# marvinquiet/SpaDOT

Measured on AMD Instinct MI355X. Metric: training steps/sec + Sinkhorn iters/sec, 50k spots x 3k genes x 5 timepoints, higher is better.
Workload: dtype bf16; 1 GPU; cfg3: 5 time points x 10000 spots x 3000 genes, batch 512, k=30, 1200 inducing points; parallelism=1 GPU, n_sub=9980, E_sub=308893, m_inducing=236, params=16136032, hip_graphs=True, staged_graphs=True, bucketed_grad_exchange=False, units_in_schedule=80

## Files before the change

### include/spadot_model.h

```cpp
#ifndef SPADOT_MODEL_H
#define SPADOT_MODEL_H

#ifdef __cplusplus
extern "C" {
#endif

enum { SPADOT_DT_F32 = 0, SPADOT_DT_BF16 = 1, SPADOT_DT_F64 = 2 };
enum { SPADOT_KERNEL_GAUSSIAN = 0, SPADOT_KERNEL_CAUCHY = 1, SPADOT_KERNEL_QUADRATIC = 2 };

const char *spadot_model_version(void);

int spadot_gat_forward(const void *h, int dtype, const float *s_src, const float *s_dst,
                       const int *rowptr, const int *col, const float *bias, int n, int H, int C,
                       int concat, int act, void *out, float *alpha_out, void *stream);

int spadot_gat_backward_target(const void *g_out, const void *out, const void *h, int dtype,
                               const float *s_src, const float *s_dst, const float *alpha,
                               const int *rowptr, const int *col, int n, int H, int C, int concat,
                               int act, void *g_pre, float *dz, float *ds_dst, void *stream);

int spadot_gat_backward_source(const void *g_pre, int dtype, const float *alpha, const float *dz,
                               const int *rowptr_t, const int *col_t, const int *eid_t, int n, int H,
                               int C, void *dh, float *ds_src, const float *ds_dst, const float *att_src,
                               const float *att_dst, void *stream);
// ... 33 lines not shown
                          void *stream);
int spadot_bn_act_backward(const float *dy, const float *y, const void *x, int x_dtype, const float *lin_bias,
                           const float *gamma, const float *save_mean, const float *save_invstd, int b, int F,
                           double slope, void *dx, float *dgamma, float *dbeta, void *stream);
int spadot_ln_act_forward(const float *x, const float *gamma, const float *beta, int b, int F, double eps, double slope,
                          float *y, float *save_mean, float *save_invstd, void *stream);
int spadot_ln_act_backward(const float *dy, const float *y, const float *x, const float *gamma, const float *save_mean,
                           const float *save_invstd, int b, int F, double slope, float *dx, float *dgamma, float *dbeta,
                           void *stream);

int spadot_svgp_post_forward(const double *raw, const double *rd, const double *r, const double *Mr, const double *ld,
                             const double *sm, const double *mu, const double *var, const double *ktilde, int b, int L,
                             int m, double c, double kl_const, double b_over_N, double *p_m, double *mv, double *p_v,
                             double *tr, double *out4, float *skl32 , void *stream);
int spadot_svgp_post_backward(const float *g_skl, const double *out4, const double *G_pm, const double *G_pv,
                              const double *mu, const double *var, const double *mv, const double *tr, const double *p_m,
                              const double *p_v, const double *ktilde, const double *Mr, const double *M, int b, int L,
                              int m, double c, double b_over_N, double *g_mu, double *g_var, double *G1, double *G2T,
                              double *g_kl, double *gMr, double *gM, void *stream);
int spadot_svgp_q1t(const double *Ta, const double *Tb, const double *G2T, const double *m0, const double *g_kl, int L, int nh,
                    int b, double *q1, void *stream);
int spadot_svgp_post_pm_pv(const double *raw, const double *rd_a, const double *ktilde, int b, int L, double c, double *p_m,
                           double *p_v, void *stream);
int spadot_svgp_grad_tail(const double *q1, const double *q2, const double *Kdt, const double *p_v, const double *ktilde,
                          const double *p_m, const double *mu, const double *w, const double *g_kl, const double *g_mu,
                          const double *g_var, int b, int L, double c, double *dmu, double *dvar, float *dz,
                          void *stream);
int spadot_svgp_pre(const float *z, int b, int L, double *mu, double *var, double *w, double *muw, void *stream);
int spadot_svgp_pre2(const float *z, const double *Kn, int b, int L, int m, double *mu, double *var, double *w, double *muw,
                     double *A, void *stream);
int spadot_svgp_mid(const double *S, const double *t, const double *M, const double *X2, int L, int m, int rows2,
                    double *r, double *Mr, double *raw, double *sm, double *smpart, int smpart_doubles, void *stream);

int spadot_latent_head_forward(const float *zg, const double *p_m, const double *p_v, float *eps, int b, int Ls,
                               int Lg, float *latent, float *scal2, double *partials, unsigned *counter,
                               unsigned long long *rng_state, void *stream);
int spadot_latent_head_backward(const float *zg, const double *p_v, const float *eps, const float *latent,
                                const float *g_latent, const float *g_kl, const float *g_align, int b, int Ls, int Lg,
                                float *d_zg, double *d_pm, double *d_pv, void *stream);
int spadot_cluster_losses_forward(const float *z, const long long *labels_all, const long long *seed_ids,
                                  const float *centres, const float *prev_centres, const float *gamma,
                                  const long long *cluster_list, int b, int D, int K, int Kp, int Kl, int do_km,
                                  int do_ot, float *out2, float *work, void *stream);
int spadot_cluster_losses_backward(const float *z, const float *centres, const float *prev_centres, const float *gamma,
                                   const long long *cluster_list, const float *work, const float *g_km,
                                   const float *g_ot, int b, int D, int K, int Kp, int Kl, int do_km, int do_ot,
                                   float *dz, void *stream);
int spadot_cluster_losses_fb(const float *z, const long long *labels_all, const long long *seed_ids, const float *centres,
                             const float *prev_centres, const float *gamma, const long long *cluster_list, int b, int D, int K,
                             int Kp, int Kl, int do_km, int do_ot, const float *g_km, const float *g_ot, float *out2,
                             float *work, float *dz, void *stream);
int spadot_mix_losses_forward(const float *const *terms6, const float *w6, float *out7, void *stream);
int spadot_mix_losses_backward(const float *g_elbo, const float *w6, float *g6, void *stream);

int spadot_sqerr_forward(const void *y, const void *yhat, long long count, double inv_scale, int dtype,
                         double *scratch, void *out1, void *stream);
int spadot_sqerr_backward(const void *g1, const void *y, const void *yhat, long long count,
                          double inv_scale, int dtype, void *g_yhat, void *stream);

int spadot_kmeans_assign(const void *x, const void *centers, int n, int k, int d, int dtype, int *labels,
                         void *stream);

int spadot_sgemm_small(int mode, const float *A, int lda, const float *B, int ldb, float *C, int ldc, int M, int N, int K,
                       const float *bias, int batch, long long strideA, long long strideB, long long strideC, void *stream);

int spadot_enc_fused_supported(int b, int F1, int F2, int Q);
long long spadot_enc_fused_workspace(int b, int F1, int F2, int Q);
int spadot_enc_bn_map(const float *h1, const float *lin_bias, const float *gamma, const float *beta, float *running_mean,
                      float *running_var, long long *num_batches_tracked, int b, int F1, double momentum, double eps, double slope,
                      float *y1, float *save_mean, float *save_invstd, const float *W2, int F2, float *part, void *stream);
int spadot_enc_bn_fc(const float *part, int nparts, const float *lin_bias, const float *gamma, const float *beta, float *running_mean,
                     float *running_var, long long *num_batches_tracked, int b, int F2, double momentum, double eps, double slope,
                     float *h2, float *y2, float *save_mean, float *save_invstd, const float *Wfc, int Q, float *pz, void *stream);
int spadot_enc_sum_z(const float *pz, int nparts, const float *bias, int b, int Q, float *z, void *stream);
int spadot_svgp_pre2_partials(const float *pz, int nparts, const float *bias, const double *Kn, int b, int L, int m, float *z,
                              double *mu, double *var, double *w, double *muw, double *A, void *stream);

int spadot_recon_fb_supported(int b, int K, int G);
long long spadot_recon_fb_workspace(int b, int K, int G);
int spadot_recon_fb(const void *h_bf16, const void *W_bf16, const void *WT_bf16, int ldt, const float *bias, const float *y, int b, int K,
                    int G, double inv_scale, const float *grad_weight, void *g_bf16, float *workspace, double *loss_parts, float *dh,
                    void *stream);
int spadot_sum_parts(const double *part, int n, double scale, float *out, void *stream);

int spadot_stamp(unsigned long long *buf, int slot, void *stream);

int spadot_lloyd_step(const double *X, double *C, const int *xoff, const int *npts, int n_max, int R, const int *rgroup,
                      const int *Kr, int K_max, int D, const double *tol, double *part, int *done, double *inertia, int skip_done,
                      void *stream);
int spadot_kmeanspp_seed(const double *X, const int *xoff, const int *npts, int D, int P, const int *pset, const int *pK,
                         const int *pfirst, const int *puoff, const double *U, int K_max, int n_max, double *closest, int *idx,
                         double *centers, void *stream);

int spadot_knn(const double *x, int n, int d, int kk, int *out, void *stream);

int spadot_gat_mfma_supported(int dtype, int H, int C, int max_cols);

int spadot_gat_tail_supported(int dtype, int H, int K);
int spadot_gat_tail_wvec(const float *W, int ldw, const float *att_src, const float *att_dst, int H, int C, int K, float *part,
                         int slices, float *wv, void *whi, void *wlo, void *stream);
int spadot_gat_tail_logits(const void *x, int dtype, int ldx, const float *wv, const void *whi, const void *wlo, int n, int H, int K,
                           float *s, void *stream);
int spadot_gat_tail_aggregate(const void *x, int dtype, int ldx, const float *s, const int *rowptr, const int *col, int n_tgt, int H,
                              int K, void *A, float *alpha, void *stream);
int spadot_gat_tail_headmean(const void *O, int dtype, const float *bias, int n_tgt, int H, int C, void *out, void *stream);
int spadot_gat_tail_colsum_rows(const void *g, int dtype, int rows, int C, float *out, void *stream);
int spadot_gat_tail_scale_colsum(const void *g, int dtype, int rows, int C, double scale, void *gs, float *out, void *stream);
int spadot_gat_tail_edge_backward(const void *x, int dtype, int ldx, const void *dA, const float *s, const float *alpha, const int *rowptr,
                                  const int *col, int n_tgt, int H, int K, float *dz, float *ds_dst, void *stream);
int spadot_gat_tail_source_backward(const void *dA, int dtype, const float *alpha, const float *dz, const float *ds_dst, const float *wv,
                                    const int *rowptr_t, const int *col_t, const int *eid_t, int n, int n_tgt, int rows_out, int H, int K,
                                    void *dx, int lddx, float *ds_src, const void *act_out, int ldm, double slope, void *stream);
int spadot_gat_tail_dwvec_rows(int n);
int spadot_gat_tail_dwvec(const void *x, int dtype, int ldx, const float *ds_src, const float *ds_dst, int n, int n_tgt, int H, int K,
                          float *part, void *stream);
int spadot_gat_tail_wvec_backward(const float *W, int ldw, const float *att_src, const float *att_dst, const float *dwv, int H, int C, int K,
                                  float *dW, int lddw, int accumulate, float *datt_src, float *datt_dst, void *stream);
int spadot_gat_alpha(const float *s_src, const float *s_dst, const int *rowptr, const int *col, const int *cellq, int n_tgt,
                     int H, float *alpha, void *acell, const int *cellq_s, void *acell_s, void *stream);
int spadot_gat_aggregate(const void *x, int dtype, const void *acell, const int *plan_rows, const int *plan_sptr,
                         const int *plan_cols, int nb, int max_cols, int H, int C, int mode, const float *vec_a,
                         const float *vec_b, int act, const float *ds_src, const float *ds_dst, void *out,
                         const void *h_rows, float *att_part, int part_width, int pad_from, int pad_to, const float *dz,
                         const int *rowptr_t, const int *eid_t, float *ds_src_out, void *stream);
int spadot_gat_edge_dot(const void *g_out, const void *out, const void *h, int dtype, const int *plan_rows,
                        const int *plan_sptr, const int *plan_cols, const int *plan_cell, int nb, int max_cols, int H,
                        int C, int act, void *g_pre, float *dz, float *bias_part, int part_width, int part_col, void *stream);
int spadot_gat_softmax_backward(const float *alpha, const float *s_src, const float *s_dst, const int *rowptr,
                                const int *col, const int *cellq_s, int n_tgt, int n_all, int H, float *dz, float *ds_dst,
                                void *acell_s, void *stream);
int spadot_gat_ds_src(const float *dz, const int *rowptr_t, const int *eid_t, int n, int H, float *ds_src, void *stream);

int spadot_gemm_tn_bf16(const void *A, int lda, const void *B, int ldb, void *C, int ldc, int M, int N, int K, void *stream);
int spadot_gemm_nn_bf16(const void *A, int lda, const void *B, int ldb, void *C, int ldc, int M, int N, int K, void *stream);
int spadot_gemm_nn_bf16_masked(const void *A, int lda, const void *B, int ldb, void *C, int ldc, int M, int N, int K,
                               const void *act_out, int ldm, double slope, void *stream);
long long spadot_gemm_bf16_split_workspace(int M, int N, int tail_row_tiles, int slices);
int spadot_gemm_tn_bf16_split(const void *A, int lda, const void *B, int ldb, void *C, int ldc, int M, int N, int K,
                              int tail_row_tiles, int slices, float *workspace, void *stream);


long long spadot_gemm_wgrad_bf16_workspace(int M, int N, int K, int slices);
int spadot_gemm_wgrad_bf16(const void *G, int ldg, const void *X, int ldx, float *dW, int ldw, int M, int N, int K,
                           int slices, float *workspace, const void *zero_row, void *stream);
long long spadot_gemm_wgrad_bf16_workspace_tiled(int M, int N, int K, int slices, int tile_k);
int spadot_gemm_wgrad_bf16_tiled(const void *G, int ldg, const void *X, int ldx, float *dW, int ldw, int M, int N, int K,
                                 int slices, int tile_k, float *workspace, const void *zero_row, void *stream);

int spadot_mlp_chain_supported(int n_layers, const int *dims);
int spadot_mlp_chain_workspace(int b, int n_layers, const int *dims, int *n_rows, int *width);
int spadot_mlp_chain_forward(const float *x, int b, int n_layers, const int *dims, const float *const *W,
                             const float *const *bias, const float *const *gamma, const float *const *beta, const double *eps,
                             const double *slope, float *const *a, float *const *y, float *const *mean, float *const *invstd,
                             void *stream);
int spadot_mlp_chain_forward_bf16(const float *x, int b, int n_layers, const int *dims, const float *const *W,
                                  const float *const *bias, const float *const *gamma, const float *const *beta,
                                  const double *eps, const double *slope, float *const *a, float *const *y, float *const *mean,
                                  float *const *invstd, void *y_last_bf16, void *stream);
int spadot_mlp_chain_backward(const float *dy, const float *x, int b, int n_layers, const int *dims, const float *const *W,
                              const float *const *gamma, const double *slope, float *const *a, float *const *y,
                              float *const *mean, float *const *invstd, float *dx, float *workspace, float *grads, void *stream);
int spadot_mlp_chain_backward_add(const float *dy, const float *x, int b, int n_layers, const int *dims, const float *const *W,
                                  const float *const *gamma, const double *slope, float *const *a, float *const *y,
                                  float *const *mean, float *const *invstd, float *dx, const float *dx_add, float *workspace,
                                  float *grads, void *stream);

int spadot_bias_sqerr_forward(const float *o, const float *bias, const float *y, int b, int G, double inv_scale, double *scratch,
                              float *out, void *stream);
int spadot_bias_sqerr_backward(const float *g1, const float *o, const float *bias, const float *y, int b, int G,
                               double inv_scale, void *g_bf16, float *dbias, void *stream);

int spadot_headfc_backward(const float *g, const void *h_bf16, const float *W, int b, int K, int N, void *dh_bf16,
                           float *workspace , float *grads ,
                           void *stream);

int spadot_cast_rows_multi(const float *const *src, void *const *dst, const int *rows, const int *K, const int *Kp, int n,
                           void *stream);

int spadot_grad_sumsq(const float *grad, long long count, double *scratch, float *sumsq, void *stream);
int spadot_clip_adamw_dev(float *param, const float *grad, float *exp_avg, float *exp_avg_sq, long long count, double lr,
                          double beta1, double beta2, double eps, double weight_decay, double max_norm, double *scratch,
                          float *sumsq, int *step_dev, unsigned *counter, const float *grad_scale_dev, void *stream);
typedef struct spadot_weight_image {
    long long offset;
    int rows, K, Kp, reserved;
    void *image;
} spadot_weight_image;
typedef struct spadot_weight_images {
    int n, reserved;
    spadot_weight_image w[8];
} spadot_weight_images;
int spadot_clip_adamw_images_dev(float *param, const float *grad, float *exp_avg, float *exp_avg_sq, long long count, double lr,
                                 double beta1, double beta2, double eps, double weight_decay, double max_norm, double *scratch,
                                 float *sumsq, int *step_dev, const float *grad_scale_dev, const spadot_weight_images *images,
                                 void *stream);
int spadot_grad_norm_step_dev(const float *grad, long long count, double *scratch, float *sumsq, int *step_dev, void *stream);
int spadot_adamw_range_dev(float *param, const float *grad, float *exp_avg, float *exp_avg_sq, long long offset, long long count,
                           double lr, double beta1, double beta2, double eps, double weight_decay, double max_norm,
                           const float *sumsq, const int *step_dev, const float *grad_scale_dev, const spadot_weight_images *images,
                           void *stream);

int spadot_adamw_step(float *param, const float *grad, float *exp_avg, float *exp_avg_sq,
                      const float *sumsq, long long count, double lr, double beta1, double beta2,
                      double eps, double weight_decay, double max_norm, int step, void *stream);

int spadot_adamw_step_dev(float *param, const float *grad, float *exp_avg, float *exp_avg_sq,
                          const float *sumsq, long long count, double lr, double beta1, double beta2,
                          double eps, double weight_decay, double max_norm, int *step_dev, void *stream);

int spadot_pre_gene_detect(const long long *colptr, const int *ridx, const float *val, const int *tp_off, int T, int G,
                           double thr, int *cnt, double *colsum, void *stream);
int spadot_pre_row_total(const long long *indptr, const int *cidx, const float *val, const int *tp_off, int T, int G,
                         const unsigned char *mask, int nrows, double *total, void *stream);
int spadot_sparkx_moments(const long long *colptr, const int *ridx, const float *val, const int *tp_off, int P,
                          const int *pair_t, const int *pair_g, const int *rowmap, const double *xt, double *mom, void *stream);
int spadot_sparkx_pvals(const double *mom, int P, const int *pair_t, const int *nkeep, const double *inv, const double *lam,
                        int nodes, double *stat, double *pval, double *comb, void *stream);
int spadot_pre_lognorm_stats(const long long *colptr, const int *ridx, const float *val, const int *tp_off, int T, int S,
                             const int *cols, const double *total, double target, double *mean, double *stdv, void *stream);
int spadot_pre_scale_write(const long long *indptr, const int *cidx, const float *val, const int *tp_off, int T, int S,
                           const int *colpos, const double *total, double target, const double *mean, const double *stdv,
                           double clip, int nrows, float *out, void *stream);

int spadot_sct_gene_stats(const long long *colptr, const int *ridx, const float *val, const int *tp_off, int t, int Gk,
                          const int *genes, int N, double *out, void *stream);
int spadot_sct_fit(const long long *colptr, const int *ridx, const float *val, const int *tp_off, int t, int G1,
                   const int *genes, const double *lur, const double *lu, int N, double tol, int maxit, int limit, double eps,
                   double *out, void *stream);
int spadot_sct_resid_stats(const long long *colptr, const int *ridx, const float *val, const int *tp_off, int t, int Gk,
                           const int *genes, const double *lur, const double *lu, int N, const double *pars, double clip_hi,
                           double clip_lo, double *out, void *stream);
int spadot_sct_resid_write(const long long *colptr, const int *ridx, const float *val, const int *tp_off, int t, int S,
                           const int *genes, const double *lur, const double *lu, const int *krow, const int *rowmap, int N,
                           const double *pars, const double *center, double clip_lo, double *out, void *stream);
int spadot_sct_polygamma(const double *x, int n, double *psi, double *psi1, void *stream);

#ifdef __cplusplus
}
#endif
#endif
```

### spadot_amd/_lib.py

```python
import ctypes
import os

_CSRC = os.path.join(os.path.dirname(os.path.abspath(__file__)), "csrc")
_CACHE = {}


class NativeLibraryMissing(RuntimeError):
    pass


def _load(name):
    if name in _CACHE:
        return _CACHE[name]
    import torch

    path = os.path.join(_CSRC, name)
    if not os.path.exists(path):
        raise NativeLibraryMissing(
            f"{path} is missing: build the HIP extension with `python -m spadot_amd.csrc.build` "
            "(needs hipcc; cross-compiles for gfx950 without a GPU). There is no CPU fallback.")
    lib = ctypes.CDLL(path)
    _CACHE[name] = lib
    return lib

# ... 70 lines not shown
    lib.spadot_ot_destroy.restype = None
    lib.spadot_ot_ld.argtypes = [vp]
    lib.spadot_ot_ld.restype = ci
    lib.spadot_ot_fused_geometry.argtypes = [vp, ctypes.POINTER(ci)]
    lib.spadot_ot_fused_geometry.restype = None
    lib.spadot_ot_matrix_dev.argtypes = [vp, ci]
    lib.spadot_ot_matrix_dev.restype = vp
    lib.spadot_ot_vector_dev.argtypes = [vp, ci]
    lib.spadot_ot_vector_dev.restype = vp
    lib.spadot_ot_vector_host.argtypes = [vp, ci, vp]
    lib.spadot_ot_vector_host.restype = ci
    lib.spadot_ot_matrix_host.argtypes = [vp, ci, vp]
    lib.spadot_ot_matrix_host.restype = ci
    lib.spadot_ot_set_cost_dev.argtypes = [vp, vp, ci, ci]
    lib.spadot_ot_set_cost_dev.restype = ci
    lib.spadot_ot_set_cost_host.argtypes = [vp, vp]
    lib.spadot_ot_set_cost_host.restype = ci
    lib.spadot_ot_set_cost_from_latents_dev.argtypes = [vp, vp, vp, ci, ci]
    lib.spadot_ot_set_cost_from_latents_dev.restype = ci
    lib.spadot_ot_solve.argtypes = [vp, vp, ctypes.POINTER(OTConfig), ctypes.POINTER(OTInfo)]
    lib.spadot_ot_solve.restype = ci
    lib.spadot_ot_plan_dev.argtypes = [vp, vp, ci, ci]
    lib.spadot_ot_plan_dev.restype = ci
    lib.spadot_ot_plan_group_sums_dev.argtypes = [vp, vp, ci, vp]
    lib.spadot_ot_plan_group_sums_dev.restype = ci
    lib.spadot_ot_plan_apply_dev.argtypes = [vp, ci, vp, ci, vp]
    lib.spadot_ot_plan_apply_dev.restype = ci
    lib.spadot_ot_plan_host.argtypes = [vp, vp]
    lib.spadot_ot_plan_host.restype = ci
    lib.spadot_ot_plan_rowsums_host.argtypes = [vp, vp]
    lib.spadot_ot_plan_rowsums_host.restype = ci
    lib.spadot_ot_run_iterations.argtypes = [vp, ctypes.POINTER(OTConfig), cd, ci, ctypes.POINTER(ctypes.c_float)]
    lib.spadot_ot_run_iterations.restype = ci
    lib.spadot_ot_run_tau_flag.argtypes = [vp, ci]
    lib.spadot_ot_run_tau_flag.restype = ci
    lib.spadot_ot_run_checked.argtypes = [vp, ctypes.POINTER(OTConfig), cd, ci, ci, ctypes.POINTER(ci), ctypes.POINTER(ctypes.c_float)]
    lib.spadot_ot_run_checked.restype = ci
    lib.spadot_ot_time_kernels.argtypes = [vp, ctypes.POINTER(OTConfig), cd, ci, ctypes.POINTER(ctypes.c_float)]
    lib.spadot_ot_time_kernels.restype = ci
    lib.spadot_ot_small_max.argtypes = []
    lib.spadot_ot_small_max.restype = ci
    lib.spadot_ot_small_solve.argtypes = [ci, ctypes.POINTER(OTSmallProblem), ci, ci, ctypes.POINTER(OTConfig), vp, vp]
    lib.spadot_ot_small_solve.restype = ci
    _seal(lib)
    lib._spadot_ready = True
    return lib


def model_lib():
    lib = _load("libspadot_model.so")
    if getattr(lib, "_spadot_ready", False):
        return lib
    vp, ci, cd, ll = ctypes.c_void_p, ctypes.c_int, ctypes.c_double, ctypes.c_longlong
    lib.spadot_model_version.restype = ctypes.c_char_p
    sig = {
        "spadot_gat_forward": [vp, ci, vp, vp, vp, vp, vp, ci, ci, ci, ci, ci, vp, vp, vp],
        "spadot_gat_backward_target": [vp, vp, vp, ci, vp, vp, vp, vp, vp, ci, ci, ci, ci, ci, vp, vp, vp, vp],
        "spadot_gat_backward_source": [vp, ci, vp, vp, vp, vp, vp, ci, ci, ci, vp, vp, vp, vp, vp, vp],
        "spadot_gat_logits": [vp, ci, vp, vp, ci, ci, ci, vp, vp, vp],
        "spadot_gat_att_grad": [vp, ci, vp, vp, ci, ci, ci, vp, ci, vp, vp, vp, ci, vp],
        "spadot_gat_alpha": [vp, vp, vp, vp, vp, ci, ci, vp, vp, vp, vp, vp],
        "spadot_gat_softmax_backward": [vp, vp, vp, vp, vp, vp, ci, ci, ci, vp, vp, vp, vp],
        "spadot_gat_ds_src": [vp, vp, vp, ci, ci, vp, vp],
        "spadot_gat_mfma_supported": [ci, ci, ci, ci],
        "spadot_gat_tail_supported": [ci, ci, ci],
        "spadot_gat_tail_wvec": [vp, ci, vp, vp, ci, ci, ci, vp, ci, vp, vp, vp, vp],
        "spadot_gat_tail_logits": [vp, ci, ci, vp, vp, vp, ci, ci, ci, vp, vp],
        "spadot_gat_tail_aggregate": [vp, ci, ci, vp, vp, vp, ci, ci, ci, vp, vp, vp],
        "spadot_gat_tail_headmean": [vp, ci, vp, ci, ci, ci, vp, vp],
        "spadot_gat_tail_colsum_rows": [vp, ci, ci, ci, vp, vp],
        "spadot_gat_tail_scale_colsum": [vp, ci, ci, ci, cd, vp, vp, vp],
        "spadot_gat_tail_edge_backward": [vp, ci, ci, vp, vp, vp, vp, vp, ci, ci, ci, vp, vp, vp],
        "spadot_gat_tail_source_backward": [vp, ci, vp, vp, vp, vp, vp, vp, vp, ci, ci, ci, ci, ci, vp, ci, vp, vp, ci, cd, vp],
        "spadot_gat_tail_dwvec_rows": [ci],
        "spadot_gat_tail_dwvec": [vp, ci, ci, vp, vp, ci, ci, ci, ci, vp, vp],
        "spadot_gat_tail_wvec_backward": [vp, ci, vp, vp, vp, ci, ci, ci, vp, ci, ci, vp, vp, vp],
        "spadot_gat_aggregate": [vp, ci, vp, vp, vp, vp, ci, ci, ci, ci, ci, vp, vp, ci, vp, vp, vp, vp, vp, ci, ci, ci, vp, vp, vp, vp, vp],
        "spadot_gat_edge_dot": [vp, vp, vp, ci, vp, vp, vp, vp, ci, ci, ci, ci, ci, vp, vp, vp, ci, ci, vp],
        "spadot_gemm_tn_bf16": [vp, ci, vp, ci, vp, ci, ci, ci, ci, vp],
        "spadot_gemm_nn_bf16": [vp, ci, vp, ci, vp, ci, ci, ci, ci, vp],
        "spadot_enc_fused_supported": [ci, ci, ci, ci],
        "spadot_recon_fb_supported": [ci, ci, ci],
        "spadot_recon_fb": [vp, vp, vp, ci, vp, vp, ci, ci, ci, cd, vp, vp, vp, vp, vp, vp],
        "spadot_sum_parts": [vp, ci, cd, vp, vp],
        "spadot_enc_bn_map": [vp, vp, vp, vp, vp, vp, vp, ci, ci, cd, cd, cd, vp, vp, vp, vp, ci, vp, vp],
        "spadot_enc_bn_fc": [vp, ci, vp, vp, vp, vp, vp, vp, ci, ci, cd, cd, cd, vp, vp, vp, vp, vp, ci, vp, vp],
        "spadot_enc_sum_z": [vp, ci, vp, ci, ci, vp, vp],
        "spadot_svgp_pre2_partials": [vp, ci, vp, vp, ci, ci, ci, vp, vp, vp, vp, vp, vp, vp],
        "spadot_gemm_nn_bf16_masked": [vp, ci, vp, ci, vp, ci, ci, ci, ci, vp, ci, cd, vp],
        "spadot_gemm_tn_bf16_split": [vp, ci, vp, ci, vp, ci, ci, ci, ci, ci, ci, vp, vp],
        "spadot_gemm_wgrad_bf16": [vp, ci, vp, ci, vp, ci, ci, ci, ci, ci, vp, vp, vp],
        "spadot_gemm_wgrad_bf16_tiled": [vp, ci, vp, ci, vp, ci, ci, ci, ci, ci, ci, vp, vp, vp],
        "spadot_mlp_chain_supported": [ci, vp],
        "spadot_headfc_backward": [vp, vp, vp, ci, ci, ci, vp, vp, vp, vp],
        "spadot_bias_sqerr_forward": [vp, vp, vp, ci, ci, cd, vp, vp, vp],
        "spadot_bias_sqerr_backward": [vp, vp, vp, vp, ci, ci, cd, vp, vp, vp],
        "spadot_mlp_chain_workspace": [ci, ci, vp, vp, vp],
        "spadot_mlp_chain_forward": [vp, ci, ci, vp, vp, vp, vp, vp, vp, vp, vp, vp, vp, vp, vp],
        "spadot_mlp_chain_forward_bf16": [vp, ci, ci, vp, vp, vp, vp, vp, vp, vp, vp, vp, vp, vp, vp, vp],
        "spadot_mlp_chain_backward": [vp, vp, ci, ci, vp, vp, vp, vp, vp, vp, vp, vp, vp, vp, vp, vp],
        "spadot_mlp_chain_backward_add": [vp, vp, ci, ci, vp, vp, vp, vp, vp, vp, vp, vp, vp, vp, vp, vp, vp],
        "spadot_kernel_matrix": [vp, vp, ci, ci, ci, cd, ci, ci, vp, vp],
        "spadot_spd_inverse_logdet": [vp, ci, ci, vp, vp, vp],
        "spadot_rowdot_forward": [vp, vp, ci, ci, ci, ci, vp, vp],
        "spadot_rowdot_backward": [vp, vp, ci, ci, ci, ci, vp, vp],
        "spadot_elbo_forward": [vp, vp, vp, vp, vp, vp, vp, ci, ci, ci, vp, vp],
        "spadot_elbo_backward": [vp, vp, vp, vp, vp, vp, vp, vp, ci, ci, ci, vp, vp, vp, vp, vp, vp, vp],
        "spadot_bn_act_forward": [vp, ci, vp, vp, vp, vp, vp, vp, ci, ci, cd, cd, cd, vp, vp, vp, vp],
        "spadot_bn_act_backward": [vp, vp, vp, ci, vp, vp, vp, vp, ci, ci, cd, vp, vp, vp, vp],
        "spadot_ln_act_forward": [vp, vp, vp, ci, ci, cd, cd, vp, vp, vp, vp],
        "spadot_ln_act_backward": [vp, vp, vp, vp, vp, vp, ci, ci, cd, vp, vp, vp, vp],
        "spadot_svgp_post_forward": [vp] * 9 + [ci, ci, ci, cd, cd, cd] + [vp] * 7,
        "spadot_svgp_post_backward": [vp] * 13 + [ci, ci, ci, cd, cd] + [vp] * 8,
        "spadot_svgp_grad_tail": [vp] * 11 + [ci, ci, cd] + [vp] * 4,
        "spadot_svgp_q1t": [vp, vp, vp, vp, vp, ci, ci, ci, vp, vp],
        "spadot_svgp_post_pm_pv": [vp, vp, vp, ci, ci, cd, vp, vp, vp],
        "spadot_svgp_pre": [vp, ci, ci, vp, vp, vp, vp, vp],
        "spadot_svgp_pre2": [vp, vp, ci, ci, ci, vp, vp, vp, vp, vp, vp],
        "spadot_svgp_mid": [vp, vp, vp, vp, ci, ci, ci, vp, vp, vp, vp, vp, ci, vp],
        "spadot_spd_inverse_logdet2": [vp, ci, ci, ci, vp, vp, vp, vp, vp],
        "spadot_latent_head_forward": [vp, vp, vp, vp, ci, ci, ci, vp, vp, vp, vp, vp, vp],
        "spadot_latent_head_backward": [vp, vp, vp, vp, vp, vp, vp, ci, ci, ci, vp, vp, vp, vp],
        "spadot_cluster_losses_forward": [vp, vp, vp, vp, vp, vp, vp, ci, ci, ci, ci, ci, ci, ci, vp, vp, vp],
        "spadot_cluster_losses_backward": [vp, vp, vp, vp, vp, vp, vp, vp, ci, ci, ci, ci, ci, ci, ci, vp, vp],
        "spadot_cluster_losses_fb": [vp, vp, vp, vp, vp, vp, vp, ci, ci, ci, ci, ci, ci, ci, vp, vp, vp, vp, vp, vp],
        "spadot_mix_losses_forward": [vp, vp, vp, vp],
        "spadot_mix_losses_backward": [vp, vp, vp, vp],
        "spadot_sqerr_forward": [vp, vp, ll, cd, ci, vp, vp, vp],
        "spadot_sqerr_backward": [vp, vp, vp, ll, cd, ci, vp, vp],
        "spadot_kmeans_assign": [vp, vp, ci, ci, ci, ci, vp, vp],
        "spadot_sgemm_small": [ci, vp, ci, vp, ci, vp, ci, ci, ci, ci, vp, ci, ll, ll, ll, vp],
        "spadot_lloyd_step": [vp, vp, vp, vp, ci, ci, vp, vp, ci, ci, vp, vp, vp, vp, ci, vp],
        "spadot_kmeanspp_seed": [vp, vp, vp, ci, ci, vp, vp, vp, vp, vp, ci, ci, vp, vp, vp, vp],
        "spadot_colsum": [vp, ci, ci, vp, vp],
        "spadot_cast_rows_multi": [vp, vp, vp, vp, vp, ci, vp],
        "spadot_knn": [vp, ci, ci, ci, vp, vp],
        "spadot_stamp": [vp, ci, vp],
        "spadot_grad_sumsq": [vp, ll, vp, vp, vp],
        "spadot_clip_adamw_dev": [vp, vp, vp, vp, ll, cd, cd, cd, cd, cd, cd, vp, vp, vp, vp, vp, vp],
        "spadot_clip_adamw_images_dev": [vp, vp, vp, vp, ll, cd, cd, cd, cd, cd, cd, vp, vp, vp, vp, ctypes.POINTER(WeightImages), vp],
        "spadot_grad_norm_step_dev": [vp, ll, vp, vp, vp, vp],
        "spadot_adamw_range_dev": [vp, vp, vp, vp, ll, ll, cd, cd, cd, cd, cd, cd, vp, vp, vp, ctypes.POINTER(WeightImages), vp],
        "spadot_adamw_step": [vp, vp, vp, vp, vp, ll, cd, cd, cd, cd, cd, cd, ci, vp],
        "spadot_adamw_step_dev": [vp, vp, vp, vp, vp, ll, cd, cd, cd, cd, cd, cd, vp, vp],
        "spadot_pre_gene_detect": [vp, vp, vp, vp, ci, ci, cd, vp, vp, vp],
        "spadot_pre_row_total": [vp, vp, vp, vp, ci, ci, vp, ci, vp, vp],
        "spadot_sparkx_moments": [vp, vp, vp, vp, ci, vp, vp, vp, vp, vp, vp],
        "spadot_sparkx_pvals": [vp, ci, vp, vp, vp, vp, ci, vp, vp, vp, vp],
        "spadot_pre_lognorm_stats": [vp, vp, vp, vp, ci, ci, vp, vp, cd, vp, vp, vp],
        "spadot_pre_scale_write": [vp, vp, vp, vp, ci, ci, vp, vp, cd, vp, vp, cd, ci, vp, vp],
        "spadot_sct_gene_stats": [vp, vp, vp, vp, ci, ci, vp, ci, vp, vp],
        "spadot_sct_fit": [vp, vp, vp, vp, ci, ci, vp, vp, vp, ci, cd, ci, ci, cd, vp, vp],
        "spadot_sct_resid_stats": [vp, vp, vp, vp, ci, ci, vp, vp, vp, ci, vp, cd, cd, vp, vp],
        "spadot_sct_resid_write": [vp, vp, vp, vp, ci, ci, vp, vp, vp, vp, vp, ci, vp, vp, cd, vp, vp],
        "spadot_sct_polygamma": [vp, ci, vp, vp, vp],
    }
    for name, args in sig.items():
        fn = getattr(lib, name)
        fn.argtypes = args
        fn.restype = ci
    lib.spadot_recon_fb_workspace.argtypes = [ci, ci, ci]
    lib.spadot_recon_fb_workspace.restype = ll
    lib.spadot_enc_fused_workspace.argtypes = [ci, ci, ci, ci]
    lib.spadot_enc_fused_workspace.restype = ll
    lib.spadot_gemm_bf16_split_workspace.argtypes = [ci, ci, ci, ci]
    lib.spadot_gemm_bf16_split_workspace.restype = ll
    lib.spadot_gemm_wgrad_bf16_workspace.argtypes = [ci, ci, ci, ci]
    lib.spadot_gemm_wgrad_bf16_workspace.restype = ll
    lib.spadot_gemm_wgrad_bf16_workspace_tiled.argtypes = [ci, ci, ci, ci, ci]
    lib.spadot_gemm_wgrad_bf16_workspace_tiled.restype = ll
    _seal(lib)
    lib._spadot_ready = True
    return lib
```

### spadot_amd/csrc/gemm_wgrad_bf16.hip

```cpp
#include <hip/hip_runtime.h>
#include <cstdint>

#include "../../include/spadot_model.h"
#include "per_device.h"

namespace {

typedef __bf16 bf8 __attribute__((ext_vector_type(8)));
typedef short s4v __attribute__((ext_vector_type(4)));
typedef float f16v __attribute__((ext_vector_type(16)));

constexpr int TN = 256, TK = 256, CH = 64, NT = 512;
constexpr int ROWB = 512;
constexpr int OPB = CH * ROWB;
constexpr int STAGEB = 2 * OPB;
constexpr int LDS_BYTES = 2 * STAGEB;
constexpr int PIECES = 8;

template <int WGN, int WGK, int TI, int TJ>
__global__ __launch_bounds__(NT, 1) void k_gemm_wgrad_bf16(const __bf16 *__restrict__ G, int ldg, const __bf16 *__restrict__ X,
                                                          int ldx, float *__restrict__ dW, int ldw, int M, int N, int K,
                                                          int ktiles, int S, int chunks_per_slice,
                                                          const __bf16 *__restrict__ zrow, float *__restrict__ part) {
    extern __shared__ __attribute__((aligned(16))) unsigned char smem[];
// ... 92 lines not shown
#pragma unroll
            for (int j = 0; j < TJ; j++) {
#ifdef WGRAD_PROBE_NO_MFMA
                asm volatile("" ::"v"(af), "v"(bf[j]));
#else
                acc[i][j] = __builtin_amdgcn_mfma_f32_32x32x16_bf16(af, bf[j], acc[i][j], 0, 0, 0);
#endif
            }
        }
        __builtin_amdgcn_s_setprio(0);
    };
    auto frags_ready = [&]() __attribute__((always_inline)) {
#ifdef WGRAD_PROBE_NO_READS
        return;
#endif
        asm volatile("s_waitcnt lgkmcnt(%0)" ::"n"(RD) : "memory");
        __builtin_amdgcn_sched_barrier(0);
    };

    if (nk > 0) {
        request(0);
        if (1 < nk) {
            request(1);
            asm volatile("s_waitcnt vmcnt(%0)" ::"n"(PIECES) : "memory");
        } else {
            asm volatile("s_waitcnt vmcnt(0)" ::: "memory");
        }
        __builtin_amdgcn_s_barrier();
        s4v a0[TI][2], b0[TJ][2], a1[TI][2], b1[TJ][2];
        read_frags(0u, 0, a0, b0);
        for (int P = 0; P < nk; P++) {
            const unsigned so = (unsigned)(P & 1) * STAGEB;
            read_frags(so, 1, a1, b1);
            frags_ready();
            mma(a0, b0);
            read_frags(so, 2, a0, b0);
            frags_ready();
            mma(a1, b1);
            read_frags(so, 3, a1, b1);
            frags_ready();
            mma(a0, b0);
            if (P + 1 < nk) {
                asm volatile("s_waitcnt vmcnt(0)" ::: "memory");
                asm volatile("s_waitcnt lgkmcnt(0)" ::: "memory");
                __builtin_amdgcn_sched_barrier(0);
                __builtin_amdgcn_s_barrier();
                if (P + 2 < nk) request(P + 2);
                read_frags((unsigned)((P + 1) & 1) * STAGEB, 0, a0, b0);
                asm volatile("s_waitcnt lgkmcnt(%0)" ::"n"(RD) : "memory");
            } else {
                asm volatile("s_waitcnt lgkmcnt(0)" ::: "memory");
            }
            __builtin_amdgcn_sched_barrier(0);
            mma(a1, b1);
        }
    }

    const int lk = (wk * TJ) * 32 + (lane & 31);
    if (S == 1) {
#pragma unroll
        for (int i = 0; i < TI; i++)
#pragma unroll
            for (int j = 0; j < TJ; j++)
#pragma unroll
                for (int e = 0; e < 16; e++) {
                    const int n = n0 + (wn * TI + i) * 32 + (e & 3) + 8 * (e >> 2) + 4 * hh, k = k0 + lk + 32 * j;
                    if (n < N && k < K) dW[(size_t)n * ldw + k] = acc[i][j][e];
                }
        return;
    }
    float *mine = part + ((size_t)slice * gridDim.x / S + tile) * (size_t)(TN * TKE);
#pragma unroll
    for (int i = 0; i < TI; i++)
#pragma unroll
        for (int j = 0; j < TJ; j++)
#pragma unroll
            for (int e = 0; e < 16; e++) {
                const int ln = (wn * TI + i) * 32 + (e & 3) + 8 * (e >> 2) + 4 * hh;
                mine[(size_t)ln * TKE + lk + 32 * j] = acc[i][j][e];
            }
}

template <int TKE>
__global__ __launch_bounds__(256) void k_wgrad_reduce(const float *__restrict__ part, int S, int tiles, int ktiles,
                                                      float *__restrict__ dW, int ldw, int N, int K) {
    constexpr int RP = TKE / 4;
    constexpr int BPT = RP / 4;
    constexpr int Q = 64 * RP;
    typedef float f32x4 __attribute__((ext_vector_type(4)));
    const int tile = blockIdx.x / BPT;
    const int p0 = (blockIdx.x - tile * BPT) * 256 + threadIdx.x;
    const int tn = tile / ktiles, tk = tile - tn * ktiles;
    f32x4 v[8][4];
#pragma unroll
    for (int s_ = 0; s_ < 8; s_++)
        if (s_ < S) {
            const f32x4 *src = reinterpret_cast<const f32x4 *>(part + ((size_t)s_ * tiles + tile) * (size_t)(TN * TKE));
#pragma unroll
            for (int j = 0; j < 4; j++) v[s_][j] = src[p0 + j * Q];
        }
#pragma unroll
    for (int j = 0; j < 4; j++) {
        f32x4 sum = v[0][j];
#pragma unroll
        for (int s_ = 1; s_ < 8; s_++)
            if (s_ < S) sum += v[s_][j];
        const int idx4 = p0 + j * Q, ln = idx4 / RP, c4 = idx4 - ln * RP;
        const int n = tn * TN + ln, k = tk * TKE + 4 * c4;
        if (n < N && k + 3 < K) *reinterpret_cast<f32x4 *>(dW + (size_t)n * ldw + k) = sum;
        else if (n < N) {
            for (int e = 0; e < 4; e++)
                if (k + e < K) dW[(size_t)n * ldw + k + e] = sum[e];
        }
    }
}

static int effective_slices(int M, int slices, int *cps_out) {
    const int nchunk = (M + CH - 1) / CH;
    int S = slices > 0 ? slices : 1;
    if (S > nchunk) S = nchunk;
    if (S > 8) S = 8;
    const int cps = (nchunk + S - 1) / S;
    S = (nchunk + cps - 1) / cps;
    if (cps_out) *cps_out = cps;
    return S;
}

}

extern "C" long long spadot_gemm_wgrad_bf16_workspace_tiled(int M, int N, int K, int slices, int tile_k) {
    if (M <= 0 || N <= 0 || K <= 0 || N % TN != 0 || (tile_k != 256 && tile_k != 192)) return -22;
    const int S = effective_slices(M, slices, nullptr);
    const long long tiles = (long long)(N / TN) * ((K + tile_k - 1) / tile_k);
    return S > 1 ? (long long)S * tiles * TN * tile_k : 0;
}

extern "C" long long spadot_gemm_wgrad_bf16_workspace(int M, int N, int K, int slices) {
    return spadot_gemm_wgrad_bf16_workspace_tiled(M, N, K, slices, 256);
}

template <int WGN, int WGK, int TI, int TJ>
static int launch_wgrad(const void *G, int ldg, const void *X, int ldx, float *dW, int ldw, int M, int N, int K, int ktiles, int ntiles,
                        int S, int cps, float *workspace, const void *zero_row, hipStream_t stream) {
    constexpr int TKE = 32 * WGK * TJ;
    static PerDeviceFlag attr_set;     
    auto kern = k_gemm_wgrad_bf16<WGN, WGK, TI, TJ>;
    if (!attr_set) {
        if (hipFuncSetAttribute((const void *)kern, hipFuncAttributeMaxDynamicSharedMemorySize, LDS_BYTES) != hipSuccess) return -5;
        attr_set = true;
    }
    const int tiles = ntiles * ktiles;
    hipLaunchKernelGGL(kern, dim3((unsigned)(tiles * S)), dim3(NT), LDS_BYTES, stream, (const __bf16 *)G, ldg, (const __bf16 *)X, ldx, dW,
                       ldw, M, N, K, ktiles, S, cps, (const __bf16 *)zero_row, workspace);
    if (S > 1)
        hipLaunchKernelGGL(k_wgrad_reduce<TKE>, dim3((unsigned)tiles * (unsigned)(TKE / 16)), dim3(256), 0, stream, (const float *)workspace, S,
                           tiles, ktiles, dW, ldw, N, K);
    return hipGetLastError() == hipSuccess ? 0 : -5;
}

extern "C" int spadot_gemm_wgrad_bf16_tiled(const void *G, int ldg, const void *X, int ldx, float *dW, int ldw, int M, int N, int K,
                                            int slices, int tile_k, float *workspace, const void *zero_row, void *stream) {
    if (M <= 0 || N <= 0 || K <= 0 || N % TN != 0 || ldg < N || ldx < K || ldw < K || ldg % 8 || ldx % 8) return -22;
    if (tile_k != 256 && tile_k != 192) return -22;
    if (((uintptr_t)G & 15) || ((uintptr_t)X & 15) || ((uintptr_t)dW & 15) || (ldw % 4)) return -22;
    if (!zero_row || ((uintptr_t)zero_row & 15)) return -22;
    const int ktiles = (K + tile_k - 1) / tile_k, ntiles = N / TN;
    if (ldx < ktiles * tile_k) return -22;
    if ((size_t)M * ldg * 2 >= ((size_t)1 << 32) || (size_t)M * ldx * 2 >= ((size_t)1 << 32)) return -22;
    int cps = 0;
    const int S = effective_slices(M, slices, &cps);
    if (ntiles * ktiles > 4096) return -22;
    if (S > 1 && (!workspace || ((uintptr_t)workspace & 15))) return -22;
    if (tile_k == 256)
        return launch_wgrad<2, 4, 4, 2>(G, ldg, X, ldx, dW, ldw, M, N, K, ktiles, ntiles, S, cps, workspace, zero_row, (hipStream_t)stream);
    return launch_wgrad<4, 2, 2, 3>(G, ldg, X, ldx, dW, ldw, M, N, K, ktiles, ntiles, S, cps, workspace, zero_row, (hipStream_t)stream);
}

extern "C" int spadot_gemm_wgrad_bf16(const void *G, int ldg, const void *X, int ldx, float *dW, int ldw, int M, int N, int K,
                                      int slices, float *workspace, const void *zero_row, void *stream) {
    return spadot_gemm_wgrad_bf16_tiled(G, ldg, X, ldx, dW, ldw, M, N, K, slices, 256, workspace, zero_row, stream);
}
```

### spadot_amd/csrc/mlp_chain.hip

```cpp
#include <hip/hip_runtime.h>
#include <cstdint>

#include "../../include/spadot_model.h"
#include "per_device.h"

namespace {

constexpr int MAXL = 4, MAXD = 256, WAVE = 64;
constexpr int RBF = 4;
constexpr int RBB = 8;
constexpr int LDW = MAXD + 4;

typedef float f32x4 __attribute__((ext_vector_type(4)));

struct Stage {
    const float *W, *bias, *gamma, *beta;
    float *a, *y, *mean, *invstd;
    int din, dout;
    float eps, slope;
    int ws_off;
};
struct Chain {
    Stage s[MAXL];
    int n;
    __bf16 *ybf;
};

__device__ __forceinline__ float wave_sum(float x) {
#pragma unroll
    for (int off = 32; off > 0; off >>= 1) x += __shfl_xor(x, off, WAVE);
    return x;
}

__global__ __launch_bounds__(256) void k_mlp_chain_fwd(const float *__restrict__ x, int b, Chain ch) {
    __shared__ __attribute__((aligned(16))) float act[2][RBF][LDW];
    __shared__ float par[3][MAXD];
    const int t = threadIdx.x, lane = t & 63, wave = t >> 6;
    const int r0 = blockIdx.x * RBF;
    int cur = 0;
    {
        const int d0 = ch.s[0].din;
        for (int e = t; e < RBF * d0; e += 256) {
            const int r = e / d0, k = e - r * d0;
            act[0][r][k] = (r0 + r < b) ? x[(size_t)(r0 + r) * d0 + k] : 0.f;
        }
    }
    __syncthreads();
    for (int l = 0; l < ch.n; l++) {
        const Stage &s = ch.s[l];
        const int din = s.din, dout = s.dout;
        if (t < dout) { par[0][t] = s.bias[t]; par[1][t] = s.gamma[t]; par[2][t] = s.beta[t]; }
        for (int j = t; j < dout; j += 256) {
            float acc[RBF];
            const float bj = s.bias[j];
#pragma unroll
            for (int r = 0; r < RBF; r++) acc[r] = bj;
            const float4 *w4 = reinterpret_cast<const float4 *>(s.W + (size_t)j * din);
            for (int kb = 0; kb < din / 4; kb += 16) {
                float4 w[16];
#pragma unroll
                for (int u = 0; u < 16; u++) w[u] = kb + u < din / 4 ? w4[kb + u] : make_float4(0.f, 0.f, 0.f, 0.f);
#pragma unroll
                for (int u = 0; u < 16; u++) {
                    if (kb + u < din / 4) {
#pragma unroll
                        for (int r = 0; r < RBF; r++) {
                            const float4 xv = *reinterpret_cast<const float4 *>(&act[cur][r][4 * (kb + u)]);
                            acc[r] += w[u].x * xv.x + w[u].y * xv.y + w[u].z * xv.z + w[u].w * xv.w;
                        }
                    }
                }
            }
#pragma unroll
            for (int r = 0; r < RBF; r++) act[cur ^ 1][r][j] = acc[r];
        }
        __syncthreads();
        {
            const int r = wave, row = r0 + r;
            float *ar = act[cur ^ 1][r];
            float sm = 0.f;
            for (int j = lane; j < dout; j += WAVE) sm += ar[j];
            const float mean = wave_sum(sm) / (float)dout;
            float ss = 0.f;
            for (int j = lane; j < dout; j += WAVE) { const float d = ar[j] - mean; ss += d * d; }
            const float invstd = rsqrtf(wave_sum(ss) / (float)dout + s.eps);
            for (int j = lane; j < dout; j += WAVE) {
                const float av = ar[j];
                const float v = (av - mean) * invstd * par[1][j] + par[2][j];
                const float yv = v > 0.f ? v : s.slope * v;
                ar[j] = yv;
                if (row < b) {
                    s.a[(size_t)row * dout + j] = av; s.y[(size_t)row * dout + j] = yv;
                    if (ch.ybf && l == ch.n - 1) ch.ybf[(size_t)row * dout + j] = (__bf16)yv;
                }
            }
            if (lane == 0 && row < b) { s.mean[row] = mean; s.invstd[row] = invstd; }
        }
        __syncthreads();
        cur ^= 1;
    }
}

constexpr int WST = 16384;
constexpr int LPR = 256 / RBB;
constexpr int LDS_BWD_FLOATS = 4 * RBB * LDW + 2 * RBB + MAXD + WST;
__global__ __launch_bounds__(256, 1) void k_mlp_chain_bwd(const float *__restrict__ dy_last, const float *__restrict__ x, int b,
                                                       Chain ch, float *__restrict__ dx_out, float *__restrict__ ws,
                                                       int ws_width, const float *__restrict__ dx_add) {
    extern __shared__ __attribute__((aligned(16))) float lds_dyn[];
    float (*gz)[LDW] = reinterpret_cast<float (*)[LDW]>(lds_dyn);
    float (*da)[LDW] = reinterpret_cast<float (*)[LDW]>(lds_dyn + RBB * LDW);
    float (*xs)[LDW] = reinterpret_cast<float (*)[LDW]>(lds_dyn + 2 * RBB * LDW);
    float (*xh)[LDW] = reinterpret_cast<float (*)[LDW]>(lds_dyn + 3 * RBB * LDW);
    float *rmean = lds_dyn + 4 * RBB * LDW, *rinv = rmean + RBB;
    float *gam = rinv + RBB;
    float *wst = gam + MAXD;
    const int t = threadIdx.x;
    const int r0 = blockIdx.x * RBB;
    float *wrow = ws + (size_t)blockIdx.x * ws_width;
    {
        const int d = ch.s[ch.n - 1].dout;
        float v[RBB * MAXD / 256];
#pragma unroll
        for (int u = 0; u < RBB * MAXD / 256; u++) {
            const int e = min(t + u * 256, RBB * d - 1), r = e / d, j = e - r * d;
            v[u] = dy_last[(size_t)min(r0 + r, b - 1) * d + j];
        }
#pragma unroll
        for (int u = 0; u < RBB * MAXD / 256; u++) {
            const int e = t + u * 256;
            if (!(e < RBB * d && r0 + e / d < b)) v[u] = 0.f;
        }
#pragma unroll
        for (int u = 0; u < RBB * MAXD / 256; u++) {
            const int e = t + u * 256, r = e / d, j = e - r * d;
            if (e < RBB * d) gz[r][j] = v[u];
        }
    }
    for (int l = ch.n - 1; l >= 0; l--) {
        const Stage &s = ch.s[l];
        const int din = s.din, dout = s.dout;
        const float *xin = l == 0 ? x : ch.s[l - 1].y;
        const int tk = din / 4;
        const int jc = min(dout, WST / din);
        const bool need_dx = l > 0 || dx_out != nullptr;
        {
            constexpr int NE = RBB * MAXD / 256, NW = WST / 4 / 256;
            float vx[NE], vy[NE], va[NE];
            f32x4 vw[NW];
#pragma unroll
            for (int u = 0; u < NE; u++) {
                const int e = min(t + u * 256, RBB * din - 1), r = e / din, k = e - r * din;
                vx[u] = xin[(size_t)min(r0 + r, b - 1) * din + k];
                const int e2 = min(t + u * 256, RBB * dout - 1), r2 = e2 / dout, j = e2 - r2 * dout;
                const size_t o2 = (size_t)min(r0 + r2, b - 1) * dout + j;
                vy[u] = s.y[o2];
                va[u] = s.a[o2];
            }
            {
                const f32x4 *src = reinterpret_cast<const f32x4 *>(s.W);
#pragma unroll
                for (int u = 0; u < NW; u++) vw[u] = src[min(t + u * 256, jc * tk - 1)];
            }
            const int rr = min(r0 + (t & (RBB - 1)), b - 1);
            const float mean_t = s.mean[rr], inv_t = s.invstd[rr], gam_t = s.gamma[min(t, dout - 1)];
#pragma unroll
            for (int u = 0; u < NE; u++) {
                const int e = t + u * 256;
                if (!(e < RBB * din && r0 + e / din < b)) vx[u] = 0.f;
                if (!(e < RBB * dout && r0 + e / dout < b)) { vy[u] = 0.f; va[u] = 0.f; }
            }
            if (t < RBB) {
                const bool live = r0 + t < b;
                rmean[t] = live ? mean_t : 0.f;
                rinv[t] = live ? inv_t : 0.f;
            }
            if (t < dout) gam[t] = gam_t;
            __syncthreads();
#pragma unroll
            for (int u = 0; u < NE; u++) {
                const int e = t + u * 256;
                if (e < RBB * din) { const int r = e / din; xs[r][e - r * din] = vx[u]; }
                if (e < RBB * dout) {
                    const int r = e / dout, j = e - r * dout;
                    const bool live = r0 + r < b;
                    gz[r][j] = live ? gz[r][j] * (vy[u] > 0.f ? 1.f : s.slope) : 0.f;
                    xh[r][j] = live ? (va[u] - rmean[r]) * rinv[r] : 0.f;
                }
            }
            if (need_dx) {
                f32x4 *dst = reinterpret_cast<f32x4 *>(wst);
#pragma unroll
                for (int u = 0; u < NW; u++) {
                    const int e = t + u * 256;
                    if (e < jc * tk) dst[e] = vw[u];
                }
            }
        }
        __syncthreads();
        {
            const int r = t / LPR, sl = t % LPR;
            const float inv = rinv[r];
            float s1 = 0.f, s2 = 0.f;
// ... 235 lines not shown
            for (int r = 0; r < 8; r++) {
                const float gv = gs[r][j];
#pragma unroll
                for (int e = 0; e < 8; e++) { acc[r][e] += gv * wv[e]; pw[e] += gv * hf[r][e]; }
            }
            *reinterpret_cast<float4 *>(wrow + (size_t)j * K + k0) = make_float4(pw[0], pw[1], pw[2], pw[3]);
            *reinterpret_cast<float4 *>(wrow + (size_t)j * K + k0 + 4) = make_float4(pw[4], pw[5], pw[6], pw[7]);
        }
#pragma unroll
        for (int r = 0; r < 8; r++)
            if (r0 + r < b) {
                bf16x8 o;
#pragma unroll
                for (int e = 0; e < 8; e++) o[e] = (__bf16)acc[r][e];
                *reinterpret_cast<bf16x8 *>(dh + (size_t)(r0 + r) * K + k0) = o;
            }
    }
    if ((int)threadIdx.x < N) {
        float sb = 0.f;
#pragma unroll
        for (int r = 0; r < 8; r++) sb += gs[r][threadIdx.x];
        wrow[(size_t)N * K + threadIdx.x] = sb;
    }
}

bool fill_chain(Chain &ch, int n_layers, const int *dims, const float *const *W, const float *const *bias,
                const float *const *gamma, const float *const *beta, const double *eps, const double *slope, float *const *a,
                float *const *y, float *const *mean, float *const *invstd) {
    if (n_layers < 1 || n_layers > MAXL) return false;
    int off = 0;
    for (int l = 0; l < n_layers; l++) {
        const int din = dims[l], dout = dims[l + 1];
        if (din <= 0 || dout <= 0 || din > MAXD || dout > MAXD || din % 4 || dout % 8) return false;
        Stage &s = ch.s[l];
        s.W = W[l]; s.bias = bias ? bias[l] : nullptr; s.gamma = gamma[l]; s.beta = beta ? beta[l] : nullptr;
        s.a = a[l]; s.y = y[l]; s.mean = mean[l]; s.invstd = invstd[l];
        s.din = din; s.dout = dout; s.eps = eps ? (float)eps[l] : 0.f; s.slope = (float)slope[l];
        s.ws_off = off;
        off += dout * din + 3 * dout;
    }
    ch.n = n_layers;
    ch.ybf = nullptr;
    return true;
}

}

extern "C" {

int spadot_mlp_chain_supported(int n_layers, const int *dims) {
    if (n_layers < 1 || n_layers > MAXL) return 0;
    for (int l = 0; l < n_layers; l++)
        if (dims[l] <= 0 || dims[l + 1] <= 0 || dims[l] > MAXD || dims[l + 1] > MAXD || dims[l] % 4 || dims[l + 1] % 8) return 0;
    return 1;
}

int spadot_mlp_chain_workspace(int b, int n_layers, const int *dims, int *n_rows, int *width) {
    if (!spadot_mlp_chain_supported(n_layers, dims) || b <= 0) return -22;
    int w = 0;
    for (int l = 0; l < n_layers; l++) w += dims[l + 1] * dims[l] + 3 * dims[l + 1];
    *n_rows = (b + RBB - 1) / RBB;
    *width = w;
    return 0;
}

int spadot_mlp_chain_forward_bf16(const float *x, int b, int n_layers, const int *dims, const float *const *W,
                                  const float *const *bias, const float *const *gamma, const float *const *beta,
                                  const double *eps, const double *slope, float *const *a, float *const *y, float *const *mean,
                                  float *const *invstd, void *y_last_bf16, void *stream) {
    Chain ch;
    if (b <= 0 || !fill_chain(ch, n_layers, dims, W, bias, gamma, beta, eps, slope, a, y, mean, invstd)) return -22;
    ch.ybf = (__bf16 *)y_last_bf16;
    hipLaunchKernelGGL(k_mlp_chain_fwd, dim3((b + RBF - 1) / RBF), dim3(256), 0, (hipStream_t)stream, x, b, ch);
    return hipGetLastError() == hipSuccess ? 0 : -5;
}

int spadot_mlp_chain_forward(const float *x, int b, int n_layers, const int *dims, const float *const *W,
                             const float *const *bias, const float *const *gamma, const float *const *beta, const double *eps,
                             const double *slope, float *const *a, float *const *y, float *const *mean, float *const *invstd,
                             void *stream) {
    return spadot_mlp_chain_forward_bf16(x, b, n_layers, dims, W, bias, gamma, beta, eps, slope, a, y, mean, invstd, nullptr, stream);
}

int spadot_mlp_chain_backward_add(const float *dy, const float *x, int b, int n_layers, const int *dims, const float *const *W,
                                  const float *const *gamma, const double *slope, float *const *a, float *const *y,
                                  float *const *mean, float *const *invstd, float *dx, const float *dx_add, float *workspace,
                                  float *grads, void *stream) {
    Chain ch;
    if (b <= 0 || !fill_chain(ch, n_layers, dims, W, nullptr, gamma, nullptr, nullptr, slope, a, y, mean, invstd)) return -22;
    if (dx_add && !dx) return -22;
    int rows, width;
    if (spadot_mlp_chain_workspace(b, n_layers, dims, &rows, &width)) return -22;
    constexpr int LDS_BWD = LDS_BWD_FLOATS * (int)sizeof(float);
    static PerDeviceFlag attr_set;     
    if (!attr_set) {
        if (hipFuncSetAttribute((const void *)k_mlp_chain_bwd, hipFuncAttributeMaxDynamicSharedMemorySize, LDS_BWD) != hipSuccess) return -5;
        attr_set = true;
    }
    hipLaunchKernelGGL(k_mlp_chain_bwd, dim3(rows), dim3(256), LDS_BWD, (hipStream_t)stream, dy, x, b, ch, dx, workspace, width, dx_add);
    if (hipGetLastError() != hipSuccess) return -5;
    if (!grads) return 0;
    return spadot_colsum(workspace, rows, width, grads, stream);
}

int spadot_mlp_chain_backward(const float *dy, const float *x, int b, int n_layers, const int *dims, const float *const *W,
                              const float *const *gamma, const double *slope, float *const *a, float *const *y,
                              float *const *mean, float *const *invstd, float *dx, float *workspace, float *grads, void *stream) {
    return spadot_mlp_chain_backward_add(dy, x, b, n_layers, dims, W, gamma, slope, a, y, mean, invstd, dx, nullptr, workspace, grads,
                                         stream);
}

int spadot_bias_sqerr_forward(const float *o, const float *bias, const float *y, int b, int G, double inv_scale, double *scratch,
                              float *out, void *stream) {
    const int nb = (b + SQ_ROWS - 1) / SQ_ROWS;
    if (b <= 0 || G <= 0 || !scratch || nb > 4096) return -22;
    hipLaunchKernelGGL(k_bias_sqerr_part, dim3(nb), dim3(256), 0, (hipStream_t)stream, o, bias, y, b, G, scratch);
    hipLaunchKernelGGL(k_sum_parts, dim3(1), dim3(1024), 0, (hipStream_t)stream, scratch, nb, inv_scale, out);
    return hipGetLastError() == hipSuccess ? 0 : -5;
}

int spadot_bias_sqerr_backward(const float *g1, const float *o, const float *bias, const float *y, int b, int G,
                               double inv_scale, void *g_bf16, float *dbias, void *stream) {
    if (b <= 0 || G <= 0) return -22;
    hipLaunchKernelGGL(k_bias_sqerr_bwd, dim3((G + SB_COLS - 1) / SB_COLS), dim3(SB_COLS * SB_GY), 0, (hipStream_t)stream, g1, o,
                       bias, y, b, G, inv_scale, (__bf16 *)g_bf16, dbias);
    return hipGetLastError() == hipSuccess ? 0 : -5;
}

int spadot_headfc_backward(const float *g, const void *h_bf16, const float *W, int b, int K, int N, void *dh_bf16,
                           float *workspace, float *grads, void *stream) {
    if (b <= 0 || K <= 0 || K % 8 || N <= 0 || N > FC_MAXN || !workspace) return -22;
    const int blocks = (b + 7) / 8;
    hipLaunchKernelGGL(k_headfc_bwd, dim3(blocks), dim3(256), 0, (hipStream_t)stream, g, (const __bf16 *)h_bf16, W, b, K, N,
                       (__bf16 *)dh_bf16, workspace);
    if (hipGetLastError() != hipSuccess) return -5;
    if (!grads) return 0;
    return spadot_colsum(workspace, blocks, N * K + N, grads, stream);
}

}
```

### spadot_amd/csrc/model_kernels.hip

```cpp
#include <hip/hip_runtime.h>
#include <cmath>
#include <climits>
#include <cstdint>
#include <cstdio>
#include <cstdlib>

#include "../../include/spadot_model.h"
#include "per_device.h"

namespace {

constexpr int WAVE = 64;
constexpr float ATT_SLOPE = 0.2f;
constexpr float ACT_SLOPE = 0.01f;

template <typename T> __device__ __forceinline__ float ld(const T *p);
template <> __device__ __forceinline__ float ld<float>(const float *p) { return *p; }
template <> __device__ __forceinline__ float ld<__bf16>(const __bf16 *p) { return (float)*p; }
template <typename T> __device__ __forceinline__ void st(T *p, float v);
template <> __device__ __forceinline__ void st<float>(float *p, float v) { *p = v; }
template <> __device__ __forceinline__ void st<__bf16>(__bf16 *p, float v) { *p = (__bf16)v; }

__device__ __forceinline__ unsigned bf16_pack2(float lo, float hi) {
    const unsigned short a = __builtin_bit_cast(unsigned short, (__bf16)lo), b = __builtin_bit_cast(unsigned short, (__bf16)hi);
// ... 1224 lines not shown
        }
        int best = 0;
        double bpot = 0.0;
#pragma unroll
        for (int j = 0; j < KPP_MAXTR; j++) {
            if (j < trials) {
                const double pj = block_sum_d(lp[j], s_red);
                if (j == 0 || pj < bpot) { bpot = pj; best = j; }
            }
        }
        pot = bpot;
        const double *cb = s_c + best * D;
        const double csqb = s_csq[best];
        for (int i = t; i < n; i += KPP_T) cl[i] = fmin(cl[i], kpp_d2(Xg + (size_t)i * D, cb, csqb, D));
        for (int e = t; e < D; e += KPP_T) cp[(size_t)c * D + e] = cb[e];
        if (t == 0) ip[c] = min(s_cand[best], n - 1);
        __syncthreads();
    }
}

__global__ __launch_bounds__(256) void k_sumsq_part(const float *__restrict__ g, long long count,
                                                    double *__restrict__ part) {
    __shared__ double sh[16];
    double acc = 0.0;
    const long long n4 = count / 4;
    const float4 *g4 = reinterpret_cast<const float4 *>(g);
    for (long long k = (long long)blockIdx.x * 256 + threadIdx.x; k < n4; k += (long long)gridDim.x * 256) {
        const float4 v = g4[k];
        acc += (double)v.x * v.x + (double)v.y * v.y + (double)v.z * v.z + (double)v.w * v.w;
    }
    if (blockIdx.x == 0)
        for (long long k = n4 * 4 + threadIdx.x; k < count; k += 256) acc += (double)g[k] * g[k];
    acc = block_sum_d(acc, sh);
    if (threadIdx.x == 0) part[blockIdx.x] = acc;
}

template <int U>
__global__ __launch_bounds__(256) void k_sumsq_last(const float *__restrict__ g, long long count, double *__restrict__ part,
                                                    float *__restrict__ sumsq, int *__restrict__ step_dev,
                                                    unsigned *__restrict__ counter) {
    __shared__ double sh[16];
    __shared__ bool last;
    double acc = 0.0;
    const long long n4 = count / 4;
    const float4 *g4 = reinterpret_cast<const float4 *>(g);
    const long long stride = (long long)gridDim.x * 256;
    for (long long k = (long long)blockIdx.x * 256 + threadIdx.x; k < n4; k += U * stride) {
        float4 v[U];
#pragma unroll
        for (int u = 0; u < U; u++)
            v[u] = (k + u * stride < n4) ? g4[k + u * stride] : make_float4(0.f, 0.f, 0.f, 0.f);
#pragma unroll
        for (int u = 0; u < U; u++)
            acc += ((double)v[u].x * v[u].x + (double)v[u].y * v[u].y) + ((double)v[u].z * v[u].z + (double)v[u].w * v[u].w);
    }
    if (blockIdx.x == 0)
        for (long long k = n4 * 4 + threadIdx.x; k < count; k += 256) acc += (double)g[k] * g[k];
    acc = block_sum_d(acc, sh);
    if (threadIdx.x == 0) {
        part[blockIdx.x] = acc;
        __threadfence();
        last = atomicAdd(counter, 1u) == gridDim.x - 1;
    }
    __syncthreads();
    if (!last) return;
    __threadfence();
    double t = 0.0;
    {
        double q[8];
#pragma unroll
        for (int u = 0; u < 8; u++) {
            const int b = threadIdx.x + u * 256;
            q[u] = b < (int)gridDim.x ? __builtin_nontemporal_load(part + b) : 0.0;
        }
        t = ((q[0] + q[1]) + (q[2] + q[3])) + ((q[4] + q[5]) + (q[6] + q[7]));
    }
    t = block_sum_d(t, sh);
    if (threadIdx.x == 0) { sumsq[0] = (float)t; if (step_dev) step_dev[0] += 1; *counter = 0u; }
}

__global__ void k_step_inc(int *step) { step[0] += 1; }

template <int U>
__global__ __launch_bounds__(256) void k_sumsq_part_u(const float *__restrict__ g, long long count, double *__restrict__ part) {
    __shared__ double sh[16];
    double acc = 0.0;
    const long long n4 = count / 4;
    const float4 *g4 = reinterpret_cast<const float4 *>(g);
    const long long stride = (long long)gridDim.x * 256;
    for (long long k = (long long)blockIdx.x * 256 + threadIdx.x; k < n4; k += U * stride) {
        float4 v[U];
#pragma unroll
        for (int u = 0; u < U; u++)
            v[u] = (k + u * stride < n4) ? g4[k + u * stride] : make_float4(0.f, 0.f, 0.f, 0.f);
#pragma unroll
        for (int u = 0; u < U; u++)
            acc += ((double)v[u].x * v[u].x + (double)v[u].y * v[u].y) + ((double)v[u].z * v[u].z + (double)v[u].w * v[u].w);
    }
    if (blockIdx.x == 0)
        for (long long k = n4 * 4 + threadIdx.x; k < count; k += 256) acc += (double)g[k] * g[k];
    acc = block_sum_d(acc, sh);
    if (threadIdx.x == 0) part[blockIdx.x] = acc;
}
__global__ __launch_bounds__(1024) void k_final_sum_step(const double *__restrict__ part, int nparts, float *__restrict__ out,
                                                         int *__restrict__ step_dev) {
    __shared__ double sh[16];
    double acc = 0.0;
    for (int k = threadIdx.x; k < nparts; k += 1024) acc += part[k];
    acc = block_sum_d(acc, sh);
    if (threadIdx.x == 0) { out[0] = (float)acc; if (step_dev) step_dev[0] += 1; }
}

__device__ __forceinline__ void adamw_element(float g_, float &pp, float &mm, float &vv, float coef, float lr, float wd,
                                              float b1, float b2, float eps, float bc1, float bc2_sqrt) {
#pragma clang fp contract(off)
    const float gg = g_ * coef;
    float pn = pp * (1.f - lr * wd);
    const float mn = mm + (gg - mm) * (1.f - b1);
    const float vn = vv * b2 + gg * gg * (1.f - b2);
    const float denom = sqrtf(vn) / bc2_sqrt + eps;
    pn -= (lr / bc1) * (mn / denom);
    pp = pn; mm = mn; vv = vn;
}

__device__ __forceinline__ float adamw_clip_coef(float sumsq, float gs, float max_norm) {
#pragma clang fp contract(off)
    const float total = sqrtf(sumsq) * gs;
    return fminf(1.f, max_norm / (total + 1e-6f)) * gs;
}

__global__ __launch_bounds__(256) void k_adamw(float *__restrict__ p, const float *__restrict__ g,
                                               float *__restrict__ m, float *__restrict__ v,
                                               const float *__restrict__ sumsq, long long count, float lr,
                                               float b1, float b2, float eps, float wd, float max_norm,
                                               float bc1, float bc2_sqrt, const int *__restrict__ step_dev,
                                               const float *__restrict__ grad_scale) {
    if (step_dev) {
        const double t = (double)step_dev[0];
        bc1 = (float)(1.0 - pow((double)b1, t));
        bc2_sqrt = (float)sqrt(1.0 - pow((double)b2, t));
    }
    const float gs = grad_scale ? grad_scale[0] : 1.f;
    const float coef = adamw_clip_coef(sumsq[0], gs, max_norm);
    for (long long k = (long long)blockIdx.x * 256 + threadIdx.x; k < count; k += (long long)gridDim.x * 256) {
        float pp = p[k], mm = m[k], vv = v[k];
        adamw_element(g[k], pp, mm, vv, coef, lr, wd, b1, b2, eps, bc1, bc2_sqrt);
        p[k] = pp; m[k] = mm; v[k] = vv;
    }
}

__global__ __launch_bounds__(256) void k_adamw_img(float *__restrict__ p, const float *__restrict__ g,
                                                   float *__restrict__ m, float *__restrict__ v,
                                                   const float *__restrict__ sumsq, long long count, float lr,
                                                   float b1, float b2, float eps, float wd, float max_norm,
                                                   const int *__restrict__ step_dev, const float *__restrict__ grad_scale,
                                                   spadot_weight_images imgs, long long base) {
    const double t = (double)step_dev[0];
    const float bc1 = (float)(1.0 - pow((double)b1, t));
    const float bc2_sqrt = (float)sqrt(1.0 - pow((double)b2, t));
    const float gs = grad_scale ? grad_scale[0] : 1.f;
    const float coef = adamw_clip_coef(sumsq[0], gs, max_norm);
    const long long n4 = count >> 2;
    for (long long q = (long long)blockIdx.x * 256 + threadIdx.x; q < n4; q += (long long)gridDim.x * 256) {
        const long long k = q << 2;
        const float4 g4 = *reinterpret_cast<const float4 *>(g + k);
        const float4 p4 = *reinterpret_cast<const float4 *>(p + k);
        const float4 m4 = *reinterpret_cast<const float4 *>(m + k);
        const float4 v4 = *reinterpret_cast<const float4 *>(v + k);
        const float gi[4] = {g4.x, g4.y, g4.z, g4.w}, pi[4] = {p4.x, p4.y, p4.z, p4.w};
        const float mi[4] = {m4.x, m4.y, m4.z, m4.w}, vi[4] = {v4.x, v4.y, v4.z, v4.w};
        float po[4], mo[4], vo[4];
#pragma unroll
        for (int e = 0; e < 4; e++) {
            po[e] = pi[e]; mo[e] = mi[e]; vo[e] = vi[e];
            adamw_element(gi[e], po[e], mo[e], vo[e], coef, lr, wd, b1, b2, eps, bc1, bc2_sqrt);
        }
        *reinterpret_cast<float4 *>(p + k) = make_float4(po[0], po[1], po[2], po[3]);
        *reinterpret_cast<float4 *>(m + k) = make_float4(mo[0], mo[1], mo[2], mo[3]);
        *reinterpret_cast<float4 *>(v + k) = make_float4(vo[0], vo[1], vo[2], vo[3]);
#pragma unroll
        for (int s_ = 0; s_ < 8; s_++) {
            if (s_ >= imgs.n) break;
            const spadot_weight_image W = imgs.w[s_];
            const unsigned long long d = (unsigned long long)(k + base - W.offset);
            if (d < (unsigned long long)W.rows * (unsigned long long)W.K) {
                const unsigned row = (unsigned)d / (unsigned)W.K;
                const unsigned col = (unsigned)d - row * (unsigned)W.K;
                __bf16 *dst = reinterpret_cast<__bf16 *>(W.image) + (size_t)row * W.Kp + col;
                const unsigned lo = (unsigned)__builtin_bit_cast(unsigned short, (__bf16)po[0]) |
                                    ((unsigned)__builtin_bit_cast(unsigned short, (__bf16)po[1]) << 16);
                const unsigned hi = (unsigned)__builtin_bit_cast(unsigned short, (__bf16)po[2]) |
                                    ((unsigned)__builtin_bit_cast(unsigned short, (__bf16)po[3]) << 16);
                *reinterpret_cast<uint2 *>(dst) = make_uint2(lo, hi);
                break;
            }
        }
    }
}

#ifndef BN_RG_DEF
#define BN_RG_DEF 16
#endif
constexpr int BN_RPT = 512 / BN_RG_DEF;
#ifndef BN_COLS_DEF
#define BN_COLS_DEF 16
#endif
constexpr int BN_COLS = BN_COLS_DEF, BN_RG = BN_RG_DEF, BN_NT = BN_COLS * BN_RG;
constexpr int LN_RG = 64, LN_NT = BN_COLS * LN_RG;

template <int RG = BN_RG>
__device__ __forceinline__ float bn_col_sum(float v, float (*sh)[BN_COLS + 1], int cl, int rg) {
    __syncthreads();
    sh[rg][cl] = v;
    __syncthreads();
    float t = 0.f;
#pragma unroll 8
    for (int g = 0; g < RG; g++) t += sh[g][cl];
    return t;
}

template <typename TX>
__global__ __launch_bounds__(BN_NT) void k_bn_act_fwd(const TX *__restrict__ x, const float *__restrict__ lb,
                                                    const float *__restrict__ gamma, const float *__restrict__ beta,
                                                    float *__restrict__ run_mean, float *__restrict__ run_var,
                                                    long long *__restrict__ nbt, int b, int F, float momentum, float eps,
                                                    float slope, float *__restrict__ y, float *__restrict__ save_mean,
                                                    float *__restrict__ save_invstd) {
    __shared__ float sh[BN_RG][BN_COLS + 1];
    const int cl = threadIdx.x & (BN_COLS - 1), rg = threadIdx.x / BN_COLS;
    const int c = blockIdx.x * BN_COLS + cl;
    const bool on = c < F;
    const int c1 = min(c, F - 1);
    const float add_r = (lb ? lb : gamma)[c1];
    const float add = (on && lb) ? add_r : 0.f;
    if (b <= BN_RG * BN_RPT) {
        float v[BN_RPT];
        const int cc = min(c, F - 1);
#pragma unroll
        for (int r = 0; r < BN_RPT; r++) v[r] = ld<TX>(x + (size_t)min(rg + r * BN_RG, b - 1) * F + cc);
        const float gam_r = gamma[cc], bet_r = beta[cc], rm_r = run_mean[cc], rv_r = run_var[cc];
#pragma unroll
        for (int r = 0; r < BN_RPT; r++) v[r] = (on && rg + r * BN_RG < b) ? v[r] + add : 0.f;
        float s = 0.f;
#pragma unroll
        for (int r = 0; r < BN_RPT; r++)
            if (rg + r * BN_RG < b) s += v[r];
        const float mean = bn_col_sum(s, sh, cl, rg) / (float)b;
        float ss = 0.f;
#pragma unroll
        for (int r = 0; r < BN_RPT; r++)
            if (rg + r * BN_RG < b) { const float d = v[r] - mean; ss += d * d; }
        const float var = bn_col_sum(ss, sh, cl, rg) / (float)b;
        const float invstd = rsqrtf(var + eps);
        if (on) {
            const float g = gam_r * invstd, o = bet_r;
#pragma unroll
            for (int r = 0; r < BN_RPT; r++) {
                const int i = rg + r * BN_RG;
                if (i < b) {
                    const float u = (v[r] - mean) * g + o;
                    y[(size_t)i * F + c] = u > 0.f ? u : slope * u;
                }
            }
            if (rg == 0) {
                save_mean[c] = mean; save_invstd[c] = invstd;
                run_mean[c] = (1.f - momentum) * rm_r + momentum * mean;
                run_var[c] = (1.f - momentum) * rv_r + momentum * var * ((float)b / (float)(b > 1 ? b - 1 : 1));
            }
        }
        if (nbt && blockIdx.x == 0 && threadIdx.x == 0) nbt[0] += 1;
        return;
    }
    float s = 0.f;
    if (on)
#pragma unroll 4
        for (int i = rg; i < b; i += BN_RG) s += ld<TX>(x + (size_t)i * F + c) + add;
    const float mean = bn_col_sum(s, sh, cl, rg) / (float)b;
    float ss = 0.f;
    if (on)
#pragma unroll 4
// ... 1041 lines not shown
    if (mode == 0) hipLaunchKernelGGL(k_sgemm_small<0>, grid, dim3(256), 0, st_, A, lda, B, ldb, C, ldc, M, N, K, bias, strideA, strideB, strideC);
    else if (mode == 1) hipLaunchKernelGGL(k_sgemm_small<1>, grid, dim3(256), 0, st_, A, lda, B, ldb, C, ldc, M, N, K, bias, strideA, strideB, strideC);
    else hipLaunchKernelGGL(k_sgemm_small<2>, grid, dim3(256), 0, st_, A, lda, B, ldb, C, ldc, M, N, K, bias, strideA, strideB, strideC);
    return hipGetLastError() == hipSuccess ? 0 : -5;
}

int spadot_stamp(unsigned long long *buf, int slot, void *stream) {
    if (!buf || slot < 0) return -22;
    hipLaunchKernelGGL(k_stamp, dim3(1), dim3(64), 0, (hipStream_t)stream, buf, slot);
    return hipGetLastError() == hipSuccess ? 0 : -5;
}

int spadot_knn(const double *x, int n, int d, int kk, int *out, void *stream) {
    if (n <= 0 || d <= 0 || d > KNN_MAXD || kk <= 0 || kk > n || kk > 128) return -22;
    const size_t lds = sizeof(double) * KNN_T * KNN_MAXD + (sizeof(double) + sizeof(int)) * (size_t)kk * KNN_T;
    static PerDeviceFlag attr_set;     
    if (!attr_set) { (void)hipFuncSetAttribute((const void *)k_knn, hipFuncAttributeMaxDynamicSharedMemorySize, 160 * 1024); attr_set = true; }
    hipLaunchKernelGGL(k_knn, dim3((n + KNN_T - 1) / KNN_T), dim3(KNN_T), lds, (hipStream_t)stream, x, n, d, kk, out);
    return hipGetLastError() == hipSuccess ? 0 : -5;
}

int spadot_lloyd_step(const double *X, double *C, const int *xoff, const int *npts, int n_max, int R, const int *rgroup,
                      const int *Kr, int K_max, int D, const double *tol, double *part, int *done, double *inertia, int skip_done,
                      void *stream) {
    if (n_max <= 0 || R <= 0 || R > 65535 || D <= 0 || D > LL_MAXD || K_max <= 0 || K_max > LL_MAXK) return -22;
    if (!X || !C || !xoff || !npts || !rgroup || !Kr || !tol || !part || !done || !inertia) return -22;
    if ((size_t)K_max * D + (size_t)LL_PTS * D > 7936) return -22;
    hipStream_t st_ = (hipStream_t)stream;
    const int nchunk = (n_max + LL_PTS - 1) / LL_PTS;
    const size_t lds = sizeof(double) * ((size_t)K_max * D + (size_t)LL_PTS * D);
    hipLaunchKernelGGL(k_lloyd_assign, dim3(nchunk, R), dim3(LL_PTS), lds, st_, X, (const double *)C, D, K_max, part, xoff, npts,
                       skip_done ? (const int *)done : (const int *)nullptr, Kr, rgroup);
    hipLaunchKernelGGL(k_lloyd_update, dim3(R), dim3(256), 0, st_, (const double *)part, nchunk, D, K_max, C, done, inertia, npts,
                       tol, skip_done, Kr, rgroup);
    return hipGetLastError() == hipSuccess ? 0 : -5;
}

int spadot_kmeanspp_seed(const double *X, const int *xoff, const int *npts, int D, int P, const int *pset, const int *pK,
                         const int *pfirst, const int *puoff, const double *U, int K_max, int n_max, double *closest, int *idx,
                         double *centers, void *stream) {
    if (P <= 0 || D <= 0 || D > LL_MAXD || K_max <= 0 || K_max > LL_MAXK || n_max <= 0) return -22;
    if (!X || !xoff || !npts || !pset || !pK || !pfirst || !puoff || !U || !closest || !idx || !centers) return -22;
    hipLaunchKernelGGL(k_kmeanspp_seed, dim3(P), dim3(KPP_T), 0, (hipStream_t)stream, X, xoff, npts, D, pset, pK, pfirst, puoff,
                       U, K_max, n_max, closest, idx, centers);
    return hipGetLastError() == hipSuccess ? 0 : -5;
}

int spadot_grad_sumsq(const float *grad, long long count, double *scratch, float *sumsq, void *stream) {
    if (count <= 0 || !scratch) return -22;
    if (((uintptr_t)grad & 15) != 0) return -22;
    hipStream_t st_ = (hipStream_t)stream;
    const long long want = (count / 4 + 255) / 256;
    const int nb = (int)(want < 1 ? 1 : (want < 2048 ? want : 2048));
    hipLaunchKernelGGL(k_sumsq_part, dim3(nb), dim3(256), 0, st_, grad, count, scratch);
    hipLaunchKernelGGL(k_final_sum<float>, dim3(1), dim3(1024), 0, st_, scratch, nb, 1.0, sumsq);
    return hipGetLastError() == hipSuccess ? 0 : -5;
}

int spadot_adamw_step_dev(float *param, const float *grad, float *exp_avg, float *exp_avg_sq, const float *sumsq,
                          long long count, double lr, double beta1, double beta2, double eps, double weight_decay,
                          double max_norm, int *step_dev, void *stream) {
    if (count <= 0 || !step_dev) return -22;
    hipStream_t st_ = (hipStream_t)stream;
    const long long want = (count + 255) / 256;
    const int nb = (int)(want < 4096 ? want : 4096);
    hipLaunchKernelGGL(k_step_inc, dim3(1), dim3(1), 0, st_, step_dev);
    hipLaunchKernelGGL(k_adamw, dim3(nb), dim3(256), 0, st_, param, grad, exp_avg, exp_avg_sq, sumsq, count,
                       (float)lr, (float)beta1, (float)beta2, (float)eps, (float)weight_decay, (float)max_norm,
                       1.f, 1.f, (const int *)step_dev, (const float *)nullptr);
    return hipGetLastError() == hipSuccess ? 0 : -5;
}

int spadot_clip_adamw_dev(float *param, const float *grad, float *exp_avg, float *exp_avg_sq, long long count, double lr,
                          double beta1, double beta2, double eps, double weight_decay, double max_norm, double *scratch,
                          float *sumsq, int *step_dev, unsigned *counter, const float *grad_scale_dev, void *stream) {
    if (count <= 0 || !step_dev || !scratch || !sumsq || !counter) return -22;
    if (((uintptr_t)grad & 15) != 0) return -22;
    hipStream_t st_ = (hipStream_t)stream;
    const long long want4 = (count / 4 + 255) / 256;
    const int nbs = (int)(want4 < 1 ? 1 : (want4 < 512 ? want4 : 512));
    constexpr int split = 2048;
    if (split > 0) {
        const int nb2 = (int)(want4 < 1 ? 1 : (want4 < split ? want4 : split));
        hipLaunchKernelGGL(k_sumsq_part_u<4>, dim3(nb2), dim3(256), 0, st_, grad, count, scratch);
        hipLaunchKernelGGL(k_final_sum_step, dim3(1), dim3(1024), 0, st_, (const double *)scratch, nb2, sumsq, step_dev);
    } else
        hipLaunchKernelGGL(k_sumsq_last<4>, dim3(nbs), dim3(256), 0, st_, grad, count, scratch, sumsq, step_dev, counter);
    const long long want = (count + 255) / 256;
    const int nb = (int)(want < 4096 ? want : 4096);
    hipLaunchKernelGGL(k_adamw, dim3(nb), dim3(256), 0, st_, param, grad, exp_avg, exp_avg_sq, (const float *)sumsq, count,
                       (float)lr, (float)beta1, (float)beta2, (float)eps, (float)weight_decay, (float)max_norm,
                       1.f, 1.f, (const int *)step_dev, grad_scale_dev);
    return hipGetLastError() == hipSuccess ? 0 : -5;
}

int spadot_clip_adamw_images_dev(float *param, const float *grad, float *exp_avg, float *exp_avg_sq, long long count, double lr,
                                 double beta1, double beta2, double eps, double weight_decay, double max_norm, double *scratch,
                                 float *sumsq, int *step_dev, const float *grad_scale_dev, const spadot_weight_images *images,
                                 void *stream) {
    if (count <= 0 || (count & 3) || !step_dev || !scratch || !sumsq || !images) return -22;
    if (((uintptr_t)grad & 15) || ((uintptr_t)param & 15) || ((uintptr_t)exp_avg & 15) || ((uintptr_t)exp_avg_sq & 15)) return -22;
    if (images->n < 0 || images->n > 8) return -22;
    for (int s_ = 0; s_ < images->n; s_++) {
        const spadot_weight_image &W = images->w[s_];
        if (!W.image || ((uintptr_t)W.image & 7) || W.rows <= 0 || W.K <= 0 || (W.K & 3) || W.Kp < W.K || (W.Kp & 3) || (W.offset & 3) ||
            W.offset < 0 || W.offset + (long long)W.rows * W.K > count || (long long)W.rows * W.K >= (1ll << 31))
            return -22;
    }
    hipStream_t st_ = (hipStream_t)stream;
    const long long want4 = (count / 4 + 255) / 256;
    const int nb2 = (int)(want4 < 1 ? 1 : (want4 < 2048 ? want4 : 2048));
    hipLaunchKernelGGL(k_sumsq_part_u<4>, dim3(nb2), dim3(256), 0, st_, grad, count, scratch);
    hipLaunchKernelGGL(k_final_sum_step, dim3(1), dim3(1024), 0, st_, (const double *)scratch, nb2, sumsq, step_dev);
    const int nb = (int)(want4 < 4096 ? want4 : 4096);
    hipLaunchKernelGGL(k_adamw_img, dim3(nb), dim3(256), 0, st_, param, grad, exp_avg, exp_avg_sq, (const float *)sumsq, count,
                       (float)lr, (float)beta1, (float)beta2, (float)eps, (float)weight_decay, (float)max_norm,
                       (const int *)step_dev, grad_scale_dev, *images, 0ll);
    return hipGetLastError() == hipSuccess ? 0 : -5;
}

int spadot_grad_norm_step_dev(const float *grad, long long count, double *scratch, float *sumsq, int *step_dev, void *stream) {
    if (count <= 0 || !scratch || !sumsq || !step_dev || ((uintptr_t)grad & 15)) return -22;
    hipStream_t st_ = (hipStream_t)stream;
    const long long want4 = (count / 4 + 255) / 256;
    const int nb2 = (int)(want4 < 1 ? 1 : (want4 < 2048 ? want4 : 2048));
    hipLaunchKernelGGL(k_sumsq_part_u<4>, dim3(nb2), dim3(256), 0, st_, grad, count, scratch);
    hipLaunchKernelGGL(k_final_sum_step, dim3(1), dim3(1024), 0, st_, (const double *)scratch, nb2, sumsq, step_dev);
    return hipGetLastError() == hipSuccess ? 0 : -5;
}

int spadot_adamw_range_dev(float *param, const float *grad, float *exp_avg, float *exp_avg_sq, long long offset, long long count,
                           double lr, double beta1, double beta2, double eps, double weight_decay, double max_norm,
                           const float *sumsq, const int *step_dev, const float *grad_scale_dev, const spadot_weight_images *images,
                           void *stream) {
    if (offset < 0 || count <= 0 || (offset & 3) || (count & 3) || !step_dev || !sumsq) return -22;
    if (((uintptr_t)grad & 15) || ((uintptr_t)param & 15) || ((uintptr_t)exp_avg & 15) || ((uintptr_t)exp_avg_sq & 15)) return -22;
    spadot_weight_images none;
    none.n = 0;
    const spadot_weight_images *tab = images ? images : &none;
    if (tab->n < 0 || tab->n > 8) return -22;
    for (int s_ = 0; s_ < tab->n; s_++) {
        const spadot_weight_image &W = tab->w[s_];
        if (!W.image || ((uintptr_t)W.image & 7) || W.rows <= 0 || W.K <= 0 || (W.K & 3) || W.Kp < W.K || (W.Kp & 3) || (W.offset & 3) ||
            W.offset < 0 || (long long)W.rows * W.K >= (1ll << 31))
            return -22;
    }
    hipStream_t st_ = (hipStream_t)stream;
    constexpr long long max_wgs = 512;
    const long long want4 = (count / 4 + 255) / 256;
    const int nb = (int)(want4 < max_wgs ? want4 : max_wgs);
    hipLaunchKernelGGL(k_adamw_img, dim3(nb), dim3(256), 0, st_, param + offset, grad + offset, exp_avg + offset, exp_avg_sq + offset,
                       sumsq, count, (float)lr, (float)beta1, (float)beta2, (float)eps, (float)weight_decay, (float)max_norm,
                       step_dev, grad_scale_dev, *tab, offset);
    return hipGetLastError() == hipSuccess ? 0 : -5;
}

int spadot_adamw_step(float *param, const float *grad, float *exp_avg, float *exp_avg_sq, const float *sumsq,
                      long long count, double lr, double beta1, double beta2, double eps, double weight_decay,
                      double max_norm, int step, void *stream) {
    if (count <= 0 || step < 1) return -22;
    hipStream_t st_ = (hipStream_t)stream;
    const long long want = (count + 255) / 256;
    const int nb = (int)(want < 4096 ? want : 4096);
    const double bc1 = 1.0 - pow(beta1, (double)step);
    const double bc2 = 1.0 - pow(beta2, (double)step);
    hipLaunchKernelGGL(k_adamw, dim3(nb), dim3(256), 0, st_, param, grad, exp_avg, exp_avg_sq, sumsq, count,
                       (float)lr, (float)beta1, (float)beta2, (float)eps, (float)weight_decay, (float)max_norm,
                       (float)bc1, (float)sqrt(bc2), (const int *)nullptr, (const float *)nullptr);
    return hipGetLastError() == hipSuccess ? 0 : -5;
}

}
```

### spadot_amd/csrc/recon_fb.hip

```cpp
#include <hip/hip_runtime.h>
#include <cmath>
#include <cstdint>

#include "../../include/spadot_model.h"

namespace {

constexpr int K = 256;
constexpr int BR = 64, BG = 128;
constexpr int NT = 256;
constexpr int DROW = 2 * BG + 16;
constexpr int LDS_D = BR * DROW;

typedef __bf16 bf8 __attribute__((ext_vector_type(8)));
typedef float f16v __attribute__((ext_vector_type(16)));

__device__ __forceinline__ unsigned short bf16_bits(float x) { return __builtin_bit_cast(unsigned short, (__bf16)x); }
__device__ __forceinline__ unsigned pack2(float lo, float hi) { return (unsigned)bf16_bits(lo) | ((unsigned)bf16_bits(hi) << 16); }

__global__ __launch_bounds__(NT, 1) void k_recon_fb(const __bf16 *__restrict__ hb, const __bf16 *__restrict__ W,
                                                    const __bf16 *__restrict__ WT, int ldt,
                                                    const float *__restrict__ bias, const float *__restrict__ y, int b, int G,
                                                    double inv_scale, const float *__restrict__ gw, __bf16 *__restrict__ gc,
                                                    float *__restrict__ dbp, double *__restrict__ lossp, float *__restrict__ dxp) {
// ... 64 lines not shown
                v[e] = (float)(coef * d);
            }
            *reinterpret_cast<uint2 *>(dl + (32 * rt + l31) * DROW + gl * 2) = make_uint2(pack2(v[0], v[1]), pack2(v[2], v[3]));
#pragma unroll
            for (int e = 0; e < 4; e++) {
                float s = v[e];
#pragma unroll
                for (int off = 16; off > 0; off >>= 1) s += __shfl_xor(s, off, 64);
                if (l31 == 0) dbl[rt * BG + gl + e] = s;
            }
        }
    }
#pragma unroll
    for (int off = 32; off > 0; off >>= 1) loss += __shfl_xor(loss, off, 64);
    if (lane == 0) lsh[wave] = loss;
    __syncthreads();
    if (tid == 0) lossp[rb * gridDim.x + gb] = ((lsh[0] + lsh[1]) + lsh[2]) + lsh[3];
    if (tid < BG && g0 + tid < G) dbp[(size_t)rb * G + g0 + tid] = dbl[tid] + dbl[BG + tid];
    {
        const int row = tid >> 2, quarter = tid & 3;
        if (r0 + row < b) {
#pragma unroll
            for (int p = 0; p < 4; p++) {
                const int gl = quarter * 32 + p * 8;
                if (g0 + gl < G)
                    *reinterpret_cast<uint4 *>(gc + (size_t)(r0 + row) * G + g0 + gl) = *reinterpret_cast<const uint4 *>(dl + row * DROW + gl * 2);
            }
        }
    }

    f16v acc2[4];
#pragma unroll
    for (int ct = 0; ct < 4; ct++)
#pragma unroll
        for (int i = 0; i < 16; i++) acc2[ct][i] = 0.f;
    const unsigned char *drow = dl + (32 * rt + l31) * DROW + 16 * hh;
#pragma unroll
    for (int gs = 0; gs < BG / 16; gs++) {
        const bf8 gf = *reinterpret_cast<const bf8 *>(drow + gs * 32);
#pragma unroll
        for (int ct = 0; ct < 4; ct++) acc2[ct] = __builtin_amdgcn_mfma_f32_32x32x16_bf16(w2[ct][gs], gf, acc2[ct], 0, 0, 0);
    }
    if (row_on) {
        float *dst = dxp + ((size_t)gb * b + r) * K + 128 * gh;
#pragma unroll
        for (int ct = 0; ct < 4; ct++)
#pragma unroll
            for (int q = 0; q < 4; q++)
                *reinterpret_cast<float4 *>(dst + 32 * ct + 8 * q + 4 * hh) =
                    make_float4(acc2[ct][4 * q], acc2[ct][4 * q + 1], acc2[ct][4 * q + 2], acc2[ct][4 * q + 3]);
    }
}

__global__ __launch_bounds__(256) void k_recon_fb_reduce(const float *__restrict__ dxp, int nblk, long long n4, float *__restrict__ dh) {
    const long long e = (long long)blockIdx.x * 256 + threadIdx.x;
    if (e >= n4) return;
    typedef float f32x4 __attribute__((ext_vector_type(4)));
    f32x4 acc = {0.f, 0.f, 0.f, 0.f};
    const f32x4 *src = reinterpret_cast<const f32x4 *>(dxp) + e;
    for (int k = 0; k < nblk; k += 8) {
        f32x4 v[8];
#pragma unroll
        for (int u = 0; u < 8; u++) v[u] = src[(long long)min(k + u, nblk - 1) * n4];
#pragma unroll
        for (int u = 0; u < 8; u++)
            if (k + u < nblk) acc += v[u];
    }
    reinterpret_cast<f32x4 *>(dh)[e] = acc;
}

}

extern "C" {

int spadot_recon_fb_supported(int b, int Kin, int G) {
    return b > 0 && b <= 4096 && Kin == K && G >= BG && G % 8 == 0;
}

long long spadot_recon_fb_workspace(int b, int Kin, int G) {
    if (!spadot_recon_fb_supported(b, Kin, G)) return -22;
    return (long long)((G + BG - 1) / BG) * b * K + (long long)((b + BR - 1) / BR) * G;
}

int spadot_recon_fb(const void *h_bf16, const void *W_bf16, const void *WT_bf16, int ldt, const float *bias, const float *y, int b, int Kin,
                    int G, double inv_scale, const float *grad_weight, void *g_bf16, float *workspace, double *loss_parts, float *dh,
                    void *stream) {
    if (!spadot_recon_fb_supported(b, Kin, G) || !h_bf16 || !W_bf16 || !WT_bf16 || !bias || !y || !grad_weight || !g_bf16 || !workspace ||
        !loss_parts || !dh || ldt < (G + BG - 1) / BG * BG || ldt % 8 || ((uintptr_t)WT_bf16 & 15))
        return -22;
    if (((uintptr_t)h_bf16 & 15) || ((uintptr_t)W_bf16 & 15) || ((uintptr_t)bias & 15) || ((uintptr_t)y & 15) || ((uintptr_t)g_bf16 & 15) ||
        ((uintptr_t)workspace & 15) || ((uintptr_t)dh & 15))
        return -22;
    const int GB = (G + BG - 1) / BG, RB = (b + BR - 1) / BR;
    float *dxp = workspace, *dbp = workspace + (size_t)GB * b * K;
    hipStream_t st = (hipStream_t)stream;
    hipLaunchKernelGGL(k_recon_fb, dim3(GB, RB), dim3(NT), 0, st, (const __bf16 *)h_bf16, (const __bf16 *)W_bf16, (const __bf16 *)WT_bf16, ldt,
                       bias, y, b, G,
                       inv_scale, grad_weight, (__bf16 *)g_bf16, dbp, loss_parts, dxp);
    const long long n4 = (long long)b * K / 4;
    hipLaunchKernelGGL(k_recon_fb_reduce, dim3((unsigned)((n4 + 255) / 256)), dim3(256), 0, st, (const float *)dxp, GB, n4, dh);
    return hipGetLastError() == hipSuccess ? 0 : -5;
}

}

namespace {
__global__ __launch_bounds__(256) void k_sum_parts_d(const double *__restrict__ part, int n, double scale, float *__restrict__ out) {
    __shared__ double sh[4];
    double acc = 0.0;
    for (int k = threadIdx.x; k < n; k += 256) acc += part[k];
#pragma unroll
    for (int off = 32; off > 0; off >>= 1) acc += __shfl_xor(acc, off, 64);
    if ((threadIdx.x & 63) == 0) sh[threadIdx.x >> 6] = acc;
    __syncthreads();
    if (threadIdx.x == 0) out[0] = (float)((((sh[0] + sh[1]) + sh[2]) + sh[3]) * scale);
}
}

extern "C" int spadot_sum_parts(const double *part, int n, double scale, float *out, void *stream) {
    if (!part || !out || n < 1) return -22;
    hipLaunchKernelGGL(k_sum_parts_d, dim3(1), dim3(256), 0, (hipStream_t)stream, part, n, scale, out);
    return hipGetLastError() == hipSuccess ? 0 : -5;
}
```

### spadot_amd/model/decoder.py

```python
import torch
import torch.nn as nn
import torch.nn.functional as F

from ..ops import (grad_bias, linear_bias, ln_act, mlp_chain, mlp_chain_ok, recon_fb_ok, recon_sqerr, recon_sqerr_fb, recon_sqerr_ok,
                   sqerr_sum, weight_image)


def _hidden_stage(fan_in, fan_out):
    dense = nn.Linear(fan_in, fan_out)
    nn.init.xavier_uniform_(dense.weight)
    return dense, nn.LayerNorm(fan_out), nn.LeakyReLU()


class Decoder(nn.Module):
    def __init__(self, input_dim, z_dim, decoder_layers, compute_dtype=torch.float32):
        super().__init__()
        self.compute_dtype = compute_dtype
        widths = [z_dim, *decoder_layers]
        stages = []
        for fan_in, fan_out in zip(widths[:-1], widths[1:]):
            stages.extend(_hidden_stage(fan_in, fan_out))
        stages.append(nn.Linear(widths[-1], input_dim))
        self.decoder_net = nn.Sequential(*stages)

    def forward(self, latent_sample):
        h, last, _ = self._hidden(latent_sample)
        return linear_bias(h, last.weight, last.bias, self.compute_dtype)

    def recon_loss(self, latent_sample, y, inv_scale, dz_extra=None, grad_weight=None):
        bf = self.compute_dtype == torch.bfloat16
        nocast = bf
        h, last, hb = self._hidden(latent_sample, bf16_out=nocast, dx_add=dz_extra)
        if bf and grad_weight is not None:
            wim = self._output_image(last.weight)
            wimT = self._output_image_T(wim) if wim is not None else None
            if recon_fb_ok(h, last.weight, last.bias, y, hb, wim, wimT, grad_weight):
                return recon_sqerr_fb(h, last.weight, last.bias, y, inv_scale, hb, wim, wimT, grad_weight)
        if bf and recon_sqerr_ok(h, last.weight, last.bias, y):
            return recon_sqerr(h, last.weight, last.bias, y, inv_scale, hb, self._output_image(last.weight) if nocast else None)
        return sqerr_sum(y, linear_bias(h, last.weight, last.bias, self.compute_dtype), inv_scale)

    def _output_image(self, W):
        opt = getattr(self, "_image_optimizer", None)
        if opt is None or not self.training or not W.is_cuda:
            return None
        if not opt.owns(W):
            object.__setattr__(self, "_image_optimizer", None)
            return None
        im = weight_image(W, W.shape[1], torch.bfloat16, self, tag="_wout")
        if not opt.maintain_image(W, im):
            return None
        opt.sync_images()
        return im

    def _output_image_T(self, wim, refresh=None):
        G, K = wim.shape
        Gp = (G + 127) // 128 * 128
        t = getattr(self, "_wout_T", None)
        if t is None or t.shape != (K, Gp) or t.device != wim.device:
            t = torch.zeros((K, Gp), dtype=torch.bfloat16, device=wim.device)
            object.__setattr__(self, "_wout_T", t)
            object.__setattr__(self, "_wout_T_fresh", False)
        if refresh is True or (refresh is None and not getattr(self, "_wout_T_fresh", False)):
            with torch.no_grad():
                t[:, :G].copy_(wim.t())
        object.__setattr__(self, "_wout_T_fresh", bool(refresh))
        return t

    def step_begin(self):
        if self.compute_dtype != torch.bfloat16 or not self.training:
            return
        wim = self._output_image(list(self.decoder_net)[-1].weight)
        if wim is not None:
            self._output_image_T(wim, refresh=True)

    def _hidden(self, latent_sample, bf16_out=False, dx_add=None):
        stages = list(self.decoder_net)
        h, hb = latent_sample, None
        hidden = [(stages[i], stages[i + 1], stages[i + 2].negative_slope) for i in range(0, len(stages) - 1, 3)]
        if hidden and mlp_chain_ok(h, hidden):
            if bf16_out:
                h, hb = mlp_chain(h, hidden, bf16_out=True, dx_add=dx_add)
            else:
                h = mlp_chain(h, hidden, dx_add=dx_add)
        else:
            if dx_add is not None:
                h = grad_bias(h, dx_add)
            for dense, norm, slope in hidden:
                h = ln_act(linear_bias(h, dense.weight, dense.bias), norm, slope)
        return h, stages[-1], hb
```

### spadot_amd/ops.py

```python
import ctypes

import torch

from ._lib import model_lib

DT_F32, DT_BF16, DT_F64 = 0, 1, 2
_DT = {torch.float32: DT_F32, torch.bfloat16: DT_BF16, torch.float64: DT_F64}
KERNEL_KINDS = {"Gaussian": 0, "Cauchy": 1, "Quadratic": 2}


def _p(t):
    return ctypes.c_void_p(t.data_ptr()) if t is not None else None


def _stream():
    return ctypes.c_void_p(torch.cuda.current_stream().cuda_stream)


def _need_cuda(*ts):
    for t in ts:
        if t is not None and not t.is_cuda:
            raise RuntimeError("spadot_amd ops run on the MI355X only (got a CPU tensor); there is no CPU path")


# ... 54 lines not shown
        return None
    return pt, ps


class _GATEdgeMFMA(torch.autograd.Function):

    @staticmethod
    def forward(ctx, h, att_src, att_dst, bias, graph, H, C, act, plans, defer=False, act_cell=None):
        _need_cuda(h, att_src, att_dst, bias)
        lib = model_lib()
        pt, ps = plans
        h = h.contiguous()
        a_s = att_src.reshape(H, C).contiguous().float()
        a_d = att_dst.reshape(H, C).contiguous().float()
        bias_f = bias.contiguous().float()
        n, nt = graph.n, graph.n_tgt
        assert h.shape[0] >= n and h.shape[1] == H * C, (h.shape, n, H, C)
        dev = h.device
        s_src = torch.empty((n, H), dtype=torch.float32, device=dev)
        s_dst = torch.empty((n, H), dtype=torch.float32, device=dev)
        _check(lib.spadot_gat_logits(_p(h), DT_BF16, _p(a_s), _p(a_d), n, H, C, _p(s_src), _p(s_dst), _stream()), "spadot_gat_logits")
        alpha = torch.empty((graph.E, H), dtype=torch.float32, device=dev)
        img = pt.weight_image(H)
        ctx.owner = att_src.data_ptr()
        img_s = ps.weight_image(H, owner=ctx.owner) if any(ctx.needs_input_grad[:4]) else None
        _check(lib.spadot_gat_alpha(_p(s_src), _p(s_dst), _p(graph.rowptr), _p(graph.col), _p(pt.cellq), nt, H, _p(alpha), _p(img),
                                    _p(ps.cellq) if img_s is not None else None, _p(img_s), _stream()), "spadot_gat_alpha")
        ctx.img_s = img_s
        out_rows = h.shape[0] if (nt == n and h.shape[0] - n <= 4096) else nt
        out = torch.empty((out_rows, H * C), dtype=h.dtype, device=dev)
        _check(lib.spadot_gat_aggregate(_p(h), DT_BF16, _p(img), _p(pt.rows), _p(pt.sptr), _p(pt.cols), pt.nb, pt.max_cols, H, C, 0,
                                        _p(bias_f), None, int(act), None, None, _p(out), None, None, 0, nt, out_rows,
                                        None, None, None, None, _stream()), "spadot_gat_aggregate")
        ctx.save_for_backward(h, s_src, s_dst, out, alpha, a_s, a_d)
        ctx.graph, ctx.H, ctx.C, ctx.act, ctx.plans = graph, H, C, act, plans
        ctx.bias_dtype, ctx.att_shape, ctx.att_dtype = bias.dtype, att_src.shape, att_src.dtype
        ctx.flat3, ctx.defer = _adjacent_flat_grads((att_src, att_dst, bias), H * C), bool(defer)
        ctx.cell = act_cell if (act and act_cell is not None) else None
        if ctx.cell is not None:
            ctx.cell["armed"], ctx.cell["rows"], ctx.cell["slope"] = True, out_rows, ACT_SLOPE
        return out

    @staticmethod
    def backward(ctx, g_out):
        lib = model_lib()
        h, s_src, s_dst, out, alpha, a_s, a_d = ctx.saved_tensors
        graph, H, C = ctx.graph, ctx.H, ctx.C
        pt, ps = ctx.plans
        n, nt = graph.n, graph.n_tgt
        dev = h.device
        g_out = g_out.contiguous().to(h.dtype)
        premasked = ctx.cell is not None and bool(ctx.cell.pop("premasked", False))
        act_here = 0 if premasked else int(ctx.act)
        g_pre = g_out if premasked else torch.empty((nt, H * C), dtype=h.dtype, device=dev)
        dz = torch.empty((graph.E, H), dtype=torch.float32, device=dev)
        ds_dst = torch.empty((n, H), dtype=torch.float32, device=dev)
        W3 = 3 * H * C
        R = max(pt.nb, ps.nb)
        bufs = graph.__dict__.setdefault("_bwd_bufs", {})
        part = bufs.get(("attpart", H, C, ctx.owner))
        if part is None or part.device != dev or part.shape != (R, W3):
            part = bufs[("attpart", H, C, ctx.owner)] = torch.zeros((R, W3), dtype=torch.float32, device=dev)
        _check(lib.spadot_gat_edge_dot(_p(g_out), _p(out), _p(h), DT_BF16, _p(pt.rows), _p(pt.sptr), _p(pt.cols), _p(pt.cell),
                                       pt.nb, pt.max_cols, H, C, act_here, None if premasked else _p(g_pre), _p(dz), _p(part), W3,
                                       2 * H * C, _stream()), "spadot_gat_edge_dot")
        img = ctx.img_s
        _check(lib.spadot_gat_softmax_backward(_p(alpha), _p(s_src), _p(s_dst), _p(graph.rowptr), _p(graph.col), None, nt, n,
                                               H, _p(dz), _p(ds_dst), None, _stream()), "spadot_gat_softmax_backward")
        dh = torch.empty_like(h)
        pad_ok = h.shape[0] - n <= 4096
        if not pad_ok:
            dh[n:].zero_()
        _check(lib.spadot_gat_aggregate(_p(g_pre), DT_BF16, _p(img), _p(ps.rows), _p(ps.sptr), _p(ps.cols), ps.nb, ps.max_cols, H, C, 1,
                                        _p(a_s), _p(a_d), 0, None, _p(ds_dst), _p(dh), _p(h), _p(part), W3, n,
                                        h.shape[0] if pad_ok else n, _p(dz), _p(graph.rowptr_t), _p(graph.eid_t), None, _stream()),
               "spadot_gat_aggregate")
        if ctx.flat3 is not None and _DIRECT_GRAD[0]:
            fa, fd, fb_ = ctx.flat3
            nrow = part.shape[0]
            job = lambda: _check(lib.spadot_colsum(_p(part), nrow, W3, _p(fa), _stream()), "spadot_colsum")
            if ctx.defer and _deferring():
                DEFERRED[0].append(job)
            elif POST_CHAIN[0] is not None:
                POST_CHAIN[0].append(job)
            else:
                job()
            return dh, fa, fd, fb_, None, None, None, None, None, None, None
        datt = torch.empty((3, H * C), dtype=torch.float32, device=dev)
        _check(lib.spadot_colsum(_p(part), part.shape[0], W3, _p(datt), _stream()), "spadot_colsum")
        return (dh, datt[0].view(ctx.att_shape).to(ctx.att_dtype), datt[1].view(ctx.att_shape).to(ctx.att_dtype),
                datt[2].to(ctx.bias_dtype), None, None, None, None, None, None, None)


ACT_SLOPE = 0.01


def _adjacent_flat_grads(params, width):
    gs = [getattr(p, "grad", None) for p in params]
    if any(g is None or g.dtype != torch.float32 or not g.is_contiguous() or g.numel() != width or g.shape != p.shape
           for g, p in zip(gs, params)):
        return None
    base = gs[0].data_ptr()
    if any(g.data_ptr() != base + 4 * width * k for k, g in enumerate(gs)):
        return None
    return tuple(gs)


class _GATEdge(torch.autograd.Function):

    @staticmethod
    def forward(ctx, h, att_src, att_dst, bias, graph, H, C, concat, act):
        _need_cuda(h, att_src, att_dst, bias)
        lib = model_lib()
        h = h.contiguous()
        a_s = att_src.reshape(H, C).contiguous().float()
        a_d = att_dst.reshape(H, C).contiguous().float()
        bias_f = bias.contiguous().float()
        n, nt = graph.n, graph.n_tgt
        assert h.shape[0] >= n and h.shape[1] == H * C, (h.shape, n, H, C)
        s_src = torch.empty((n, H), dtype=torch.float32, device=h.device)
        s_dst = torch.empty((n, H), dtype=torch.float32, device=h.device)
        _check(lib.spadot_gat_logits(_p(h), _DT[h.dtype], _p(a_s), _p(a_d), n, H, C, _p(s_src), _p(s_dst), _stream()),
               "spadot_gat_logits")
        out = torch.empty((nt, H * C if concat else C), dtype=h.dtype, device=h.device)
        alpha = torch.empty((graph.E, H), dtype=torch.float32, device=h.device)
        _check(lib.spadot_gat_forward(_p(h), _DT[h.dtype], _p(s_src), _p(s_dst), _p(graph.rowptr), _p(graph.col),
                                      _p(bias_f), nt, H, C, int(concat), int(act), _p(out), _p(alpha), _stream()),
               "spadot_gat_forward")
        ctx.save_for_backward(h, s_src, s_dst, out, alpha, a_s, a_d)
        ctx.graph, ctx.H, ctx.C, ctx.concat, ctx.act = graph, H, C, concat, act
        ctx.bias_dtype, ctx.att_shape, ctx.att_dtype = bias.dtype, att_src.shape, att_src.dtype
        return out

    @staticmethod
    def backward(ctx, g_out):
        lib = model_lib()
        h, s_src, s_dst, out, alpha, a_s, a_d = ctx.saved_tensors
        graph, H, C = ctx.graph, ctx.H, ctx.C
        n, nt = graph.n, graph.n_tgt
        g_out = g_out.contiguous().to(h.dtype)
        g_pre = torch.empty((nt, H * C), dtype=h.dtype, device=h.device)
        dz = torch.empty((graph.E, H), dtype=torch.float32, device=h.device)
        if nt == n:
            ds_dst = torch.empty((n, H), dtype=torch.float32, device=h.device)
        else:
            key = ("ds_dst", H)
            bufs = graph.__dict__.setdefault("_bwd_bufs", {})
            ds_dst = bufs.get(key)
            if ds_dst is None or ds_dst.device != h.device:
                ds_dst = bufs[key] = torch.zeros((n, H), dtype=torch.float32, device=h.device)
        _check(lib.spadot_gat_backward_target(_p(g_out), _p(out), _p(h), _DT[h.dtype], _p(s_src), _p(s_dst), _p(alpha),
                                              _p(graph.rowptr), _p(graph.col), nt, H, C, int(ctx.concat), int(ctx.act),
                                              _p(g_pre), _p(dz), _p(ds_dst), _stream()), "spadot_gat_backward_target")
        dh = torch.empty_like(h)
        if h.shape[0] > n:
            dh[n:].zero_()
        ds_src = torch.empty((n, H), dtype=torch.float32, device=h.device)
        _check(lib.spadot_gat_backward_source(_p(g_pre), _DT[h.dtype], _p(alpha), _p(dz), _p(graph.rowptr_t),
                                              _p(graph.col_t), _p(graph.eid_t), n, H, C, _p(dh), _p(ds_src),
                                              _p(ds_dst), _p(a_s), _p(a_d), _stream()), "spadot_gat_backward_source")
        datt = torch.empty((3, H * C), dtype=torch.float32, device=h.device)
        floats = 3 * H * C * max(1, min((n + 15) // 16, 1024))
        scratch = _gat_att_scratch(h.device, floats)
        _check(lib.spadot_gat_att_grad(_p(h), _DT[h.dtype], _p(ds_src), _p(ds_dst), n, H, C, _p(scratch), floats,
                                       _p(datt), ctypes.c_void_p(datt.data_ptr() + 4 * H * C), _p(g_pre), nt, _stream()),
               "spadot_gat_att_grad")
        dbias = datt[2] if ctx.concat else datt[2].view(H, C).sum(dim=0)
# ... 181 lines not shown
        K = (ctypes.c_int * n)(*(s_.shape[1] for s_, _ in grp))
        Kp = (ctypes.c_int * n)(*(d_.shape[1] for _, d_ in grp))
        _check(lib.spadot_cast_rows_multi(src, dst, rows, K, Kp, n, _stream()), "spadot_cast_rows_multi")


GEMM_DGRAD_MIN_WGS = 240
GEMM_MAX_WGS = 256
GEMM_OWN = [True]
GEMM_BUSY_CUS = 40
GEMM_FWD_SHAPES = ((2048, 9000),)


def _own_forward(M, Kp):
    return any(t[0] == Kp and M >= t[1] for t in GEMM_FWD_SHAPES)


def gemm_tn(x, w):
    M, K = x.shape
    N = w.shape[0]
    if (GEMM_OWN[0] and x.is_cuda and x.dtype == torch.bfloat16 and w.dtype == torch.bfloat16 and x.is_contiguous()
            and w.is_contiguous() and N % 256 == 0 and K % 64 == 0 and w.shape[1] == K and M >= 2560 and N >= 1024
            and ((M + 319) // 320) * (N // 256) <= GEMM_MAX_WGS):
        out = torch.empty((M, N), dtype=torch.bfloat16, device=x.device)
        lib = model_lib()
        mt, nt_ = (M + 319) // 320, N // 256
        tail = mt - (256 - GEMM_BUSY_CUS) // nt_ if GEMM_BUSY_CUS > 0 else 0
        if 0 < tail < mt and mt * nt_ > 256 - GEMM_BUSY_CUS and K >= 4 * 64:
            need = int(lib.spadot_gemm_bf16_split_workspace(M, N, tail, 4))
            if need > 0:
                ws = torch.empty(need, dtype=torch.float32, device=x.device)
                rc = lib.spadot_gemm_tn_bf16_split(x.data_ptr(), K, w.data_ptr(), K, out.data_ptr(), N, M, N, K, tail, 4,
                                                   ws.data_ptr(), _stream())
                if rc == 0:
                    return out
                if rc != -22:
                    _check(rc, "spadot_gemm_tn_bf16_split")
        rc = lib.spadot_gemm_tn_bf16(x.data_ptr(), K, w.data_ptr(), K, out.data_ptr(), N, M, N, K, _stream())
        if rc == 0:
            return out
        if rc != -22:
            _check(rc, "spadot_gemm_tn_bf16")
    return torch.nn.functional.linear(x, w)


WGRAD_MIN_WGS = 200


_ZERO_ROWS = {}


def _zero_row(device):
    key = (device.type, device.index)
    z = _ZERO_ROWS.get(key)
    if z is None:
        z = torch.zeros(256, dtype=torch.bfloat16, device=device)
        if not torch.cuda.is_current_stream_capturing():
            _ZERO_ROWS[key] = z
    return z




def wgrad_plan(N, K, Kp):
    best = None
    for tk in (256, 192):
        kt = (K + tk - 1) // tk
        if Kp < kt * tk:
            continue
        tiles = (N // 256) * kt
        if tiles == 0 or tiles > 256:
            wgs, slices = tiles, 1
        else:
            slices = min(8, max(1, 256 // tiles))
            wgs = tiles * slices
        fill = wgs / (256.0 * ((wgs + 255) // 256)) if wgs else 0.0
        score = fill * (1.0 if tk == 256 else 0.85)
        if best is None or score > best[0]:
            best = (score, tk, slices, wgs)
    if best is None or best[3] < WGRAD_MIN_WGS:
        return None
    return best[1], best[2], best[3]


def wgrad_bf16(g, x, K, out=None):
    M, N = g.shape
    Kp = x.shape[1]
    if (g.is_cuda and g.dtype == torch.bfloat16 and x.dtype == torch.bfloat16 and g.is_contiguous()
            and x.is_contiguous() and N % 256 == 0 and Kp % 8 == 0 and M >= 1024 and N >= 1024 and K >= 1024):
        if out is None:
            out = torch.empty((N, K), dtype=torch.float32, device=g.device)
        plan = wgrad_plan(N, K, Kp) if (out.is_contiguous() and out.dtype == torch.float32 and out.shape == (N, K)) else None
        if plan is not None:
            tile_k, slices, _ = plan
            lib = model_lib()
            need = int(lib.spadot_gemm_wgrad_bf16_workspace_tiled(M, N, K, slices, tile_k))
            ws = torch.empty(max(need, 4), dtype=torch.float32, device=g.device) if need >= 0 else None
            rc = -22 if ws is None else lib.spadot_gemm_wgrad_bf16_tiled(g.data_ptr(), N, x.data_ptr(), Kp, out.data_ptr(), K, M, N, K,
                                                                        slices, tile_k, ws.data_ptr(), _zero_row(g.device).data_ptr(),
                                                                        _stream())
            if rc == 0:
                return out
            if rc != -22:
                _check(rc, "spadot_gemm_wgrad_bf16_tiled")
    if out is not None:
        return torch.mm(g.t(), x[:, :K], out_dtype=torch.float32, out=out)
    return torch.mm(g.t(), x[:, :K], out_dtype=torch.float32)


class _DenseCD(torch.autograd.Function):

    @staticmethod
    def forward(ctx, x, W, wbuf, fresh, defer=False, in_cell=None):
        N, K = W.shape
        Kp = x.shape[1]
        ctx.defer = bool(defer)
        ctx.in_cell = in_cell if (in_cell is not None and in_cell.get("armed") and in_cell.get("rows") == x.shape[0]
                                  and x.dtype == torch.bfloat16 and x.is_contiguous()) else None
        assert Kp >= K and wbuf.shape == (N, Kp) and wbuf.dtype == x.dtype
        if not fresh:
            wbuf[:, :K].copy_(W)
        ctx.save_for_backward(x, wbuf)
        ctx.K = K
        g = W.grad
        ctx.wgrad = g if (g is not None and g.dtype == torch.float32 and g.is_contiguous() and g.shape == W.shape) else None
        return gemm_tn(x, wbuf) if _own_forward(x.shape[0], Kp) else torch.nn.functional.linear(x, wbuf)

    @staticmethod
    def backward(ctx, g):
        x, wbuf = ctx.saved_tensors
        g_final = g.is_contiguous() and g.dtype == x.dtype
        g = g.contiguous()
        dx = None
        if ctx.needs_input_grad[0]:
            dx = None
            M_, Kp_ = g.shape[0], wbuf.shape[1]
            if (GEMM_OWN[0] and g.is_cuda and g.dtype == torch.bfloat16 and M_ >= 2560 and Kp_ % 256 == 0
                    and wbuf.shape[0] % 64 == 0 and wbuf.is_contiguous() and ((M_ + 319) // 320) * (Kp_ // 256) >= GEMM_DGRAD_MIN_WGS):
                dx = torch.empty((M_, Kp_), dtype=torch.bfloat16, device=g.device)
                if ctx.in_cell is not None and x.shape == (M_, Kp_):
                    rc = model_lib().spadot_gemm_nn_bf16_masked(g.data_ptr(), g.shape[1], wbuf.data_ptr(), Kp_, dx.data_ptr(), Kp_, M_,
                                                                Kp_, g.shape[1], x.data_ptr(), Kp_, float(ctx.in_cell["slope"]), _stream())
                    if rc == 0:
                        ctx.in_cell["premasked"] = True
                else:
                    rc = model_lib().spadot_gemm_nn_bf16(g.data_ptr(), g.shape[1], wbuf.data_ptr(), Kp_, dx.data_ptr(), Kp_, M_, Kp_,
                                                         g.shape[1], _stream())
                if rc == -22:
                    dx = None
                elif rc != 0:
                    _check(rc, "spadot_gemm_nn_bf16")
            if dx is None:
                dx = g @ wbuf
        dW = None
        if ctx.needs_input_grad[1]:
            if ctx.defer and ctx.wgrad is not None and _deferring() and g_final:
                DEFERRED[0].append(lambda g=g, x=x, K=ctx.K, out=ctx.wgrad: wgrad_bf16(g, x, K, out))
                dW = ctx.wgrad
            else:
                dW = wgrad_bf16(g, x, ctx.K, ctx.wgrad if (ctx.wgrad is not None and _DIRECT_GRAD[0]) else None)
        return dx, dW, None, None, None, None


class _FirstMapSeeds(torch.autograd.Function):

    @staticmethod
    def forward(ctx, x32, W, xbf):
        K = W.shape[1]
        ctx.save_for_backward(x32, xbf)
        ctx.K = K
        g = W.grad
        ctx.wgrad = g if (g is not None and g.dtype == torch.float32 and g.is_contiguous() and g.shape == W.shape) else None
        return torch.nn.functional.linear(x32[:, :K], W)

    @staticmethod
    def backward(ctx, g):
        x32, xbf = ctx.saved_tensors
        K = ctx.K
        M, N = g.shape
        lib = model_lib()
        gb = g.contiguous().to(torch.bfloat16)
        out = ctx.wgrad if (ctx.wgrad is not None and _DIRECT_GRAD[0]) else torch.empty((N, K), dtype=torch.float32, device=g.device)
        S_ = 1
        need = int(lib.spadot_gemm_wgrad_bf16_workspace(M, N, K, S_))
        rc = -22
        if need >= 0:
            ws = torch.empty(max(need, 4), dtype=torch.float32, device=g.device)
            rc = lib.spadot_gemm_wgrad_bf16(gb.data_ptr(), N, xbf.data_ptr(), xbf.shape[1], out.data_ptr(), K, M, N, K, S_,
                                            ws.data_ptr(), _zero_row(g.device).data_ptr(), _stream())
        if rc == -22:
            return None, torch.mm(g.t(), x32[:, :K]), None
        _check(rc, "spadot_gemm_wgrad_bf16")
        return None, out, None


def first_map_seeds_ok(x32, W, xbf):
    if xbf is None or not (x32.is_cuda and x32.dtype == torch.float32 and xbf.dtype == torch.bfloat16 and xbf.is_contiguous()):
        return False
    N, K = W.shape
    return (N % 256 == 0 and K % 4 == 0 and xbf.shape[0] == x32.shape[0] and xbf.shape[1] >= (K + 255) // 256 * 256
            and xbf.shape[1] % 8 == 0 and xbf.data_ptr() % 16 == 0 and x32.shape[0] >= 64 and not x32.requires_grad)


def first_map_seeds(x32, W, xbf):
    return _FirstMapSeeds.apply(x32, W, xbf)


def _small_weight_grad(g, x):
    M, N = g.shape
    K = x.shape[1]
    if M >= 256 and M % 8 == 0 and min(N, K) >= 64 and N * K <= 65536:
        return torch.bmm(g.view(8, M // 8, N).transpose(1, 2), x.view(8, M // 8, K)).sum(0)
    return g.t() @ x


def sgemm_small_ok(*ts):
    return all(t.is_cuda and t.dtype == torch.float32 and t.dim() == 2 and t.is_contiguous() for t in ts)


def sgemm_small(mode, A, B, bias=None):
    _need_cuda(A, B, bias)
    if mode == 0:
        (M, K), N = A.shape, B.shape[1]
    elif mode == 1:
        (M, K), N = A.shape, B.shape[0]
    else:
        (K, M), N = A.shape, B.shape[1]
    C = torch.empty((M, N), dtype=torch.float32, device=A.device)
    _check(model_lib().spadot_sgemm_small(mode, _p(A), A.shape[1], _p(B), B.shape[1], _p(C), N, M, N, K,
                                          _p(bias) if bias is not None else None, 1, 0, 0, 0, _stream()), "spadot_sgemm_small")
    return C


def wgrad_small(g, x, slices=8):
    _need_cuda(g, x)
    M, N = g.shape
    K = x.shape[1]
    S = slices if (M % slices == 0 and M // slices >= 32) else 1
    Ms = M // S
    part = torch.empty((S, N, K), dtype=torch.float32, device=g.device)
    _check(model_lib().spadot_sgemm_small(2, _p(g), N, _p(x), K, _p(part), K, N, K, Ms, None, S, Ms * N, Ms * K, N * K, _stream()),
           "spadot_sgemm_small")
    return part.sum(0) if S > 1 else part[0]
# ... 181 lines not shown
        np1, np2 = F1 // 16, F2 // 4
        ws = torch.empty(int(lib.spadot_enc_fused_workspace(b, F1, F2, Q)), dtype=torch.float32, device=dev)
        part, pz = ws[:np1 * b * F2], ws[np1 * b * F2:]
        y1 = torch.empty((b, F1), dtype=torch.float32, device=dev)
        h2 = torch.empty((b, F2), dtype=torch.float32, device=dev)
        y2 = torch.empty((b, F2), dtype=torch.float32, device=dev)
        st = torch.empty(2 * F1 + 2 * F2, dtype=torch.float32, device=dev)
        sm1, si1, sm2, si2 = st[:F1], st[F1:2 * F1], st[2 * F1:2 * F1 + F2], st[2 * F1 + F2:]
        mom = lambda bn: 0.1 if bn.momentum is None else float(bn.momentum)
        _check(lib.spadot_enc_bn_map(_p(h1), _p(b1), _p(g1), _p(be1), _p(bn1.running_mean), _p(bn1.running_var),
                                     _p(bn1.num_batches_tracked), b, F1, mom(bn1), float(bn1.eps), float(slope1), _p(y1), _p(sm1), _p(si1),
                                     _p(W2), F2, _p(part), _stream()), "spadot_enc_bn_map")
        _check(lib.spadot_enc_bn_fc(_p(part), np1, _p(b2), _p(g2), _p(be2), _p(bn2.running_mean), _p(bn2.running_var),
                                    _p(bn2.num_batches_tracked), b, F2, mom(bn2), float(bn2.eps), float(slope2), _p(h2), _p(y2), _p(sm2),
                                    _p(si2), _p(Wfc), Q, _p(pz), _stream()), "spadot_enc_bn_fc")
        z = torch.empty((b, Q), dtype=torch.float32, device=dev)
        if fill:
            _check(lib.spadot_enc_sum_z(_p(pz), np2, _p(bfc), b, Q, _p(z), _stream()), "spadot_enc_sum_z")
        ctx.save_for_backward(h1, b1, g1, y1, sm1, si1, W2, b2, g2, h2, y2, sm2, si2, Wfc)
        ctx.slopes = (float(slope1), float(slope2))
        ctx.mark_non_differentiable(pz)
        return z, pz

    @staticmethod
    def backward(ctx, dz, _unused):
        h1, b1, g1, y1, sm1, si1, W2, b2, g2, h2, y2, sm2, si2, Wfc = ctx.saved_tensors
        lib = model_lib()
        b, F1 = h1.shape
        F2, Q = W2.shape[0], Wfc.shape[0]
        dev = h1.device
        dz = dz.contiguous().float()
        dbfc = torch.empty(Q, dtype=torch.float32, device=dev)
        _check(lib.spadot_colsum(_p(dz), b, Q, _p(dbfc), _stream()), "spadot_colsum")
        dy2 = dz @ Wfc
        dWfc = _small_weight_grad(dz, y2)
        dh2 = torch.empty_like(h2)
        dg2 = torch.empty(F2, dtype=torch.float32, device=dev)
        dbe2 = torch.empty(F2, dtype=torch.float32, device=dev)
        _check(lib.spadot_bn_act_backward(_p(dy2), _p(y2), _p(h2), DT_F32, None if b2 is None else _p(b2), _p(g2), _p(sm2), _p(si2), b, F2,
                                          ctx.slopes[1], _p(dh2), _p(dg2), _p(dbe2), _stream()), "spadot_bn_act_backward")
        small = sgemm_small_ok(dh2, W2) and b * F2 * F1 <= _SMALL_WORK
        dy1 = sgemm_small(0, dh2, W2) if small else dh2 @ W2
        small = sgemm_small_ok(dh2, y1) and b * F2 * F1 <= _SMALL_WORK
        dW2 = wgrad_small(dh2, y1) if small else dh2.t() @ y1
        dh1 = torch.empty_like(h1)
        dg1 = torch.empty(F1, dtype=torch.float32, device=dev)
        dbe1 = torch.empty(F1, dtype=torch.float32, device=dev)
        _check(lib.spadot_bn_act_backward(_p(dy1.contiguous()), _p(y1), _p(h1), DT_F32, None if b1 is None else _p(b1), _p(g1), _p(sm1),
                                          _p(si1), b, F1, ctx.slopes[0], _p(dh1), _p(dg1), _p(dbe1), _stream()), "spadot_bn_act_backward")
        return (dh1, None if b1 is None else _const_zeros(b1), dg1, dbe1, None, None, dW2, None if b2 is None else _const_zeros(b2),
                dg2, dbe2, None, None, dWfc, dbfc, None)


def encoder_mid(h1, lin1_bias, bn1, slope1, W2, lin2_bias, bn2, slope2, Wfc, bfc, fill=True):
    assert bn1.training and bn2.training and bn1.track_running_stats and bn2.track_running_stats and bn1.affine and bn2.affine
    z, pz = _EncoderMid.apply(h1, lin1_bias, bn1.weight, bn1.bias, bn1, slope1, W2, lin2_bias, bn2.weight, bn2.bias, bn2, slope2,
                               Wfc, bfc, fill)
    return z, pz, W2.shape[0] // 4



MLP_CHAIN = [True]


def _ptr_array(tensors):
    return (ctypes.c_void_p * len(tensors))(*(t_.data_ptr() for t_ in tensors))


def _contiguous_grad_block(params):
    gs_ = [p.grad for p in params]
    if any(g is None or g.dtype != torch.float32 or not g.is_contiguous() for g in gs_):
        return None
    st0, off = gs_[0].untyped_storage(), gs_[0].storage_offset()
    pos = off
    for g in gs_:
        if g.untyped_storage().data_ptr() != st0.data_ptr() or g.storage_offset() != pos:
            return None
        pos += g.numel()
    return torch.empty(0, dtype=torch.float32, device=gs_[0].device).set_(st0, off, (pos - off,))


CHAIN_BF16_OUT = [False]
CHAIN_DX_ADD = [None]
_LAST_CHAIN_BF16 = []


class _MLPChain(torch.autograd.Function):

    @staticmethod
    def forward(ctx, x, eps, slope, *params):
        n = len(params) // 4
        Ws, bs, gs, betas = params[0::4], params[1::4], params[2::4], params[3::4]
        b = x.shape[0]
        dims = [x.shape[1]] + [W.shape[0] for W in Ws]
        dev = x.device
        a = [torch.empty((b, d), dtype=torch.float32, device=dev) for d in dims[1:]]
        y = [torch.empty((b, d), dtype=torch.float32, device=dev) for d in dims[1:]]
        stats = torch.empty((2 * n, b), dtype=torch.float32, device=dev)
        mean, inv = [stats[2 * l] for l in range(n)], [stats[2 * l + 1] for l in range(n)]
        cd = (ctypes.c_int * (n + 1))(*dims)
        ce = (ctypes.c_double * n)(*[float(e) for e in eps])
        cs = (ctypes.c_double * n)(*[float(v) for v in slope])
        ybf = torch.empty((b, dims[-1]), dtype=torch.bfloat16, device=dev) if CHAIN_BF16_OUT[0] else None
        _check(model_lib().spadot_mlp_chain_forward_bf16(_p(x), b, n, cd, _ptr_array(Ws), _ptr_array(bs), _ptr_array(gs),
                                                         _ptr_array(betas), ce, cs, _ptr_array(a), _ptr_array(y), _ptr_array(mean),
                                                         _ptr_array(inv), None if ybf is None else _p(ybf), _stream()),
               "spadot_mlp_chain_forward_bf16")
        if ybf is not None:
            _LAST_CHAIN_BF16.append(ybf)
        ctx.dx_add = CHAIN_DX_ADD[0]
        ctx.save_for_backward(x, stats, *Ws, *gs, *a, *y)
        ctx.n, ctx.dims, ctx.slope = n, dims, [float(v) for v in slope]
        ctx.flat_out = _contiguous_grad_block(params)
        return y[-1]

    @staticmethod
    def backward(ctx, dy):
        n, dims = ctx.n, ctx.dims
        sv = ctx.saved_tensors
        x, stats = sv[0], sv[1]
        Ws, gs, a, y = sv[2:2 + n], sv[2 + n:2 + 2 * n], sv[2 + 2 * n:2 + 3 * n], sv[2 + 3 * n:2 + 4 * n]
        b = x.shape[0]
        dev = x.device
        cd = (ctypes.c_int * (n + 1))(*dims)
        rows, width = ctypes.c_int(0), ctypes.c_int(0)
        lib = model_lib()
        _check(lib.spadot_mlp_chain_workspace(b, n, cd, ctypes.byref(rows), ctypes.byref(width)), "spadot_mlp_chain_workspace")
        ws = torch.empty((rows.value, width.value), dtype=torch.float32, device=dev)
        direct = ctx.flat_out is not None and _DIRECT_GRAD[0] and ctx.flat_out.numel() == width.value
        grads = ctx.flat_out if direct else torch.empty(width.value, dtype=torch.float32, device=dev)
        dx = torch.empty_like(x) if ctx.needs_input_grad[0] else None
        mean, inv = [stats[2 * l] for l in range(n)], [stats[2 * l + 1] for l in range(n)]
        cs = (ctypes.c_double * n)(*ctx.slope)
        late = direct and _deferring()
        add = ctx.dx_add
        assert add is None or (dx is not None and add.shape == x.shape and add.dtype == torch.float32 and add.is_contiguous())
        _check(lib.spadot_mlp_chain_backward_add(_p(dy.contiguous().float()), _p(x), b, n, cd, _ptr_array(Ws), _ptr_array(gs), cs,
                                                 _ptr_array(a), _ptr_array(y), _ptr_array(mean), _ptr_array(inv),
                                                 None if dx is None else _p(dx), None if add is None else _p(add), _p(ws),
                                                 None if late else _p(grads), _stream()),
               "spadot_mlp_chain_backward_add")
        if late:
            DEFERRED[0].append(lambda ws=ws, grads=grads: _check(
                lib.spadot_colsum(_p(ws), ws.shape[0], ws.shape[1], _p(grads), _stream()), "spadot_colsum"))
        out = []
        off = 0
        for l in range(n):
            din, dout = dims[l], dims[l + 1]
            out += [grads[off:off + dout * din].view(dout, din), grads[off + dout * din:off + dout * din + dout],
                    grads[off + dout * din + dout:off + dout * din + 2 * dout],
                    grads[off + dout * din + 2 * dout:off + dout * din + 3 * dout]]
            off += dout * din + 3 * dout
        return (dx, None, None, *out)


def mlp_chain_ok(x, stages):
    if not (MLP_CHAIN[0] and x.is_cuda and x.dtype == torch.float32 and x.dim() == 2 and 1 <= len(stages) <= 4):
        return False
    dims = [x.shape[1]] + [lin.out_features for lin, _, _ in stages]
    if any(lin.in_features != d for (lin, _, _), d in zip(stages, dims[:-1])):
        return False
    ts = [t_ for lin, ln, _ in stages for t_ in (lin.weight, lin.bias, ln.weight, ln.bias)]
    if any(t_ is None or t_.dtype != torch.float32 or not t_.is_contiguous() or t_.data_ptr() % 16 for t_ in ts):
        return False
    return bool(model_lib().spadot_mlp_chain_supported(len(stages), (ctypes.c_int * len(dims))(*dims)))


def mlp_chain(x, stages, bf16_out=False, dx_add=None):
    params = [t_ for lin, ln, _ in stages for t_ in (lin.weight, lin.bias, ln.weight, ln.bias)]
    CHAIN_BF16_OUT[0], CHAIN_DX_ADD[0] = bool(bf16_out), dx_add
    try:
        out = _MLPChain.apply(x.contiguous(), [ln.eps for _, ln, _ in stages], [sl for _, _, sl in stages], *params)
    finally:
        CHAIN_BF16_OUT[0], CHAIN_DX_ADD[0] = False, None
    return (out, _LAST_CHAIN_BF16.pop()) if bf16_out else out


class _GradBias(torch.autograd.Function):

    @staticmethod
    def forward(ctx, x, extra):
        ctx.extra = extra
        return x.view_as(x)

    @staticmethod
    def backward(ctx, g):
        return (ctx.extra if g is None else g + ctx.extra), None


def grad_bias(x, extra):
    return _GradBias.apply(x, extra)




class _HeadFC(torch.autograd.Function):

    @staticmethod
    def forward(ctx, h, W, bias):
        b, K = h.shape
        N = W.shape[0]
        out = torch.addmm(bias, h.float(), W.t())
        ctx.save_for_backward(h, W)
        ctx.flat_out = _contiguous_grad_block((W, bias))
        return out

    @staticmethod
    def backward(ctx, g):
        h, W = ctx.saved_tensors
        b, K = h.shape
        N = W.shape[0]
        dev = h.device
        dh = torch.empty_like(h)
        ws = torch.empty(((b + 7) // 8, N * K + N), dtype=torch.float32, device=dev)
        direct = ctx.flat_out is not None and _DIRECT_GRAD[0] and ctx.flat_out.numel() == N * K + N
        grads = ctx.flat_out if direct else torch.empty(N * K + N, dtype=torch.float32, device=dev)
        late = direct and _deferring()
        _check(model_lib().spadot_headfc_backward(_p(g.contiguous().float()), _p(h), _p(W), b, K, N, _p(dh), _p(ws),
                                                  None if late else _p(grads), _stream()), "spadot_headfc_backward")
        if late:
            DEFERRED[0].append(lambda ws=ws, grads=grads: _check(
                model_lib().spadot_colsum(_p(ws), ws.shape[0], ws.shape[1], _p(grads), _stream()), "spadot_colsum"))
        return dh, grads[:N * K].view(N, K), grads[N * K:]


def head_fc_ok(h, W, bias):
    return bool(h.is_cuda and h.dtype == torch.bfloat16 and h.dim() == 2 and h.is_contiguous()
                and W.dtype == torch.float32 and W.is_contiguous() and bias is not None and W.shape[0] <= 32
                and h.shape[1] % 8 == 0 and W.shape[1] == h.shape[1] and W.data_ptr() % 16 == 0 and h.data_ptr() % 16 == 0
                and W.numel() * 4 <= 65536)


def head_fc(h, W, bias):
    return _HeadFC.apply(h, W, bias)



_counters = {}


def _zero_counter(device):
    key = str(device)
    if key not in _counters:
        _counters[key] = torch.zeros(1, dtype=torch.int32, device=device)
    return _counters[key]


class _LatentHead(torch.autograd.Function):
    @staticmethod
    def forward(ctx, zg, p_m, p_v, eps, Ls, Lg, rng_state=None):
        _need_cuda(zg, p_m, p_v)
        zg = zg.contiguous().float()
        p_m, p_v = p_m.contiguous().double(), p_v.contiguous().double()
        b = zg.shape[0]
        if eps is None:
            assert rng_state is not None and rng_state.dtype == torch.int64 and rng_state.numel() == 2
            eps = torch.empty((b, Ls + Lg), dtype=torch.float32, device=zg.device)
# ... 304 lines not shown
        _need_cuda(y, yhat)
        y, yhat = y.contiguous(), yhat.contiguous()
        assert y.shape == yhat.shape and y.dtype == yhat.dtype
        out = torch.empty(1, dtype=y.dtype, device=y.device)
        _check(model_lib().spadot_sqerr_forward(_p(y), _p(yhat), y.numel(), float(inv_scale), _DT[y.dtype],
                                                _p(_get_scratch(y.device)), _p(out), _stream()), "spadot_sqerr_forward")
        ctx.save_for_backward(y, yhat)
        ctx.inv_scale = float(inv_scale)
        return out[0]

    @staticmethod
    def backward(ctx, g):
        y, yhat = ctx.saved_tensors
        g1 = g.reshape(1).contiguous().to(y.dtype)
        gy = torch.empty_like(yhat)
        _check(model_lib().spadot_sqerr_backward(_p(g1), _p(y), _p(yhat), y.numel(), ctx.inv_scale, _DT[y.dtype],
                                                 _p(gy), _stream()), "spadot_sqerr_backward")
        return None, gy, None


def sqerr_sum(y, yhat, inv_scale):
    return _SqErr.apply(y, yhat, inv_scale)




class _LinearSqErr(torch.autograd.Function):

    @staticmethod
    def forward(ctx, h, W, bias, y, inv_scale, hc=None, Wc=None):
        b, G = y.shape
        pairs = []
        if hc is None:
            hc = torch.empty(h.shape, dtype=torch.bfloat16, device=h.device)
            pairs.append((h, hc))
        if Wc is None:
            Wc = torch.empty(W.shape, dtype=torch.bfloat16, device=W.device)
            pairs.append((W.detach().contiguous(), Wc))
        if pairs:
            cast_rows(pairs)
        o = torch.mm(hc, Wc.t(), out_dtype=torch.float32)
        out = torch.empty(1, dtype=torch.float32, device=h.device)

        scratch = _get_scratch(h.device) if DEFERRED[0] is None else torch.empty_like(_get_scratch(h.device))

        def value(o=o, bias=bias, y=y, out=out, scratch=scratch):
            _check(model_lib().spadot_bias_sqerr_forward(_p(o), _p(bias), _p(y), b, G, float(inv_scale), _p(scratch), _p(out), _stream()),
                   "spadot_bias_sqerr_forward")

        if DEFERRED[0] is not None:
            DEFERRED[0].append(value)
        else:
            value()
        ctx.save_for_backward(hc, Wc, o, bias, y)
        ctx.inv_scale = float(inv_scale)
        ok = lambda g_, p_: g_ if (g_ is not None and g_.dtype == torch.float32 and g_.is_contiguous() and g_.shape == p_.shape) else None
        ctx.wgrad, ctx.bgrad = ok(W.grad, W), ok(bias.grad, bias)
        return out[0]

    @staticmethod
    def backward(ctx, g):
        hc, Wc, o, bias, y = ctx.saved_tensors
        b, G = y.shape
        g1 = g.reshape(1).contiguous().float()
        gc = torch.empty((b, G), dtype=torch.bfloat16, device=y.device)
        direct = _DIRECT_GRAD[0]
        db = ctx.bgrad if (direct and ctx.bgrad is not None) else torch.empty(G, dtype=torch.float32, device=y.device)
        _check(model_lib().spadot_bias_sqerr_backward(_p(g1), _p(o), _p(bias), _p(y), b, G, ctx.inv_scale, _p(gc), _p(db),
                                                      _stream()), "spadot_bias_sqerr_backward")
        dh = torch.mm(gc, Wc, out_dtype=torch.float32) if ctx.needs_input_grad[0] else None
        if direct and ctx.wgrad is not None and _deferring():
            DEFERRED[0].append(lambda gc=gc, hc=hc, out=ctx.wgrad: torch.mm(gc.t(), hc, out_dtype=torch.float32, out=out))
            dW = ctx.wgrad
        elif direct and ctx.wgrad is not None:
            dW = torch.mm(gc.t(), hc, out_dtype=torch.float32, out=ctx.wgrad)
        else:
            dW = torch.mm(gc.t(), hc, out_dtype=torch.float32)
        return dh, dW, db, None, None, None, None


class _ReconFB(torch.autograd.Function):

    @staticmethod
    def forward(ctx, h, W, bias, y, inv_scale, hc, Wc, WcT, gw):
        lib = model_lib()
        b, K = h.shape
        G = W.shape[0]
        dev = h.device
        nfl = int(lib.spadot_recon_fb_workspace(b, K, G))
        GB, RB = (G + 127) // 128, (b + 63) // 64
        ws = torch.empty(nfl, dtype=torch.float32, device=dev)
        lossp = torch.empty(GB * RB, dtype=torch.float64, device=dev)
        gc = torch.empty((b, G), dtype=torch.bfloat16, device=dev)
        dh = torch.empty((b, K), dtype=torch.float32, device=dev)
        _check(lib.spadot_recon_fb(_p(hc), _p(Wc), _p(WcT), WcT.shape[1], _p(bias), _p(y), b, K, G, float(inv_scale), _p(gw), _p(gc), _p(ws),
                                   _p(lossp), _p(dh), _stream()), "spadot_recon_fb")
        out = torch.empty(1, dtype=torch.float32, device=dev)

        def value(lossp=lossp, out=out):
            _check(lib.spadot_sum_parts(_p(lossp), GB * RB, float(inv_scale), _p(out), _stream()), "spadot_sum_parts")

        if DEFERRED[0] is not None:
            DEFERRED[0].append(value)
        else:
            value()
        ctx.save_for_backward(hc, gc, dh)
        ctx.dbp = ws[GB * b * K:].view(RB, G)
        ctx.seed = gw.data_ptr()
        ok = lambda g_, p_: g_ if (g_ is not None and g_.dtype == torch.float32 and g_.is_contiguous() and g_.shape == p_.shape) else None
        ctx.wgrad, ctx.bgrad = ok(W.grad, W), ok(bias.grad, bias)
        return out[0]

    @staticmethod
    def backward(ctx, g):
        if g is None or g.data_ptr() != ctx.seed:
            raise RuntimeError("recon_sqerr_fb: backward seeded with something other than the weight its gradient was formed for "
                               "(the forward launch already holds d loss / d h for THAT seed)")
        hc, gc, dh = ctx.saved_tensors
        lib = model_lib()
        dbp = ctx.dbp
        direct = _DIRECT_GRAD[0]
        db = ctx.bgrad if (direct and ctx.bgrad is not None) else torch.empty(dbp.shape[1], dtype=torch.float32, device=dh.device)
        dW = ctx.wgrad if (direct and ctx.wgrad is not None) else torch.empty((gc.shape[1], hc.shape[1]), dtype=torch.float32, device=dh.device)

        def rest(dbp=dbp, db=db, dW=dW, gc=gc, hc=hc):
            _check(lib.spadot_colsum(_p(dbp), dbp.shape[0], dbp.shape[1], _p(db), _stream()), "spadot_colsum")
            torch.mm(gc.t(), hc, out_dtype=torch.float32, out=dW)

        if direct and ctx.wgrad is not None and ctx.bgrad is not None and _deferring():
            DEFERRED[0].append(rest)
        else:
            with torch.no_grad():
                rest()
        return dh, dW, db, None, None, None, None, None, None


def recon_fb_ok(h, W, bias, y, hc, Wc, WcT, gw):
    ok = lambda t_, like: (t_ is not None and t_.dtype == torch.bfloat16 and t_.is_contiguous() and t_.shape == like.shape)
    okT = (WcT is not None and WcT.dtype == torch.bfloat16 and WcT.is_contiguous() and WcT.dim() == 2 and WcT.shape[0] == W.shape[1]
           and WcT.shape[1] >= (W.shape[0] + 127) // 128 * 128 and WcT.shape[1] % 8 == 0 and WcT.data_ptr() % 16 == 0)
    return bool(okT and gw is not None and gw.is_cuda and gw.dtype == torch.float32 and h.is_cuda and h.dtype == torch.float32 and h.dim() == 2
                and y.dtype == torch.float32 and y.is_contiguous() and y.shape == (h.shape[0], W.shape[0]) and bias is not None
                and bias.dtype == torch.float32 and bias.is_contiguous() and bias.data_ptr() % 16 == 0 and y.data_ptr() % 16 == 0
                and ok(hc, h) and ok(Wc, W) and model_lib().spadot_recon_fb_supported(h.shape[0], h.shape[1], W.shape[0]))


def recon_sqerr_fb(h, W, bias, y, inv_scale, h_bf16, W_image, W_image_T, grad_weight):
    return _ReconFB.apply(h, W, bias, y, inv_scale, h_bf16, W_image, W_image_T, grad_weight)


def recon_sqerr_ok(h, W, bias, y):
    return bool(h.is_cuda and h.dtype == torch.float32 and y.dtype == torch.float32 and h.dim() == 2
                and y.dim() == 2 and h.shape[1] % 4 == 0 and W.shape[1] % 4 == 0 and y.shape == (h.shape[0], W.shape[0])
                and h.shape[0] <= 4096
                and bias is not None)


def recon_sqerr(h, W, bias, y, inv_scale, h_bf16=None, W_image=None):
    ok = lambda t_, like: (t_ is not None and t_.dtype == torch.bfloat16 and t_.is_contiguous() and t_.shape == like.shape)
    return _LinearSqErr.apply(h.contiguous(), W, bias, y.contiguous(), inv_scale, h_bf16 if ok(h_bf16, h) else None,
                              W_image if ok(W_image, W) else None)


def kmeans_assign(x, centers):
    _need_cuda(x, centers)
    x = x.contiguous()
    centers = centers.contiguous().to(x.dtype)
    labels = torch.empty(x.shape[0], dtype=torch.int32, device=x.device)
    _check(model_lib().spadot_kmeans_assign(_p(x), _p(centers), x.shape[0], centers.shape[0], x.shape[1],
                                            _DT[x.dtype], _p(labels), _stream()), "spadot_kmeans_assign")
    return labels



def lloyd_steps(X, C, xoff, npts, n_max, rgroup, Kr, tol, done, inertia, part, steps, skip_done=False):
    D = X.shape[1]
    R, K_max = C.shape[0], C.shape[1]
    lib = model_lib()
    for _ in range(steps):
        _check(lib.spadot_lloyd_step(_p(X), _p(C), _p(xoff), _p(npts), int(n_max), R, _p(rgroup), _p(Kr), K_max, D, _p(tol),
                                     _p(part), _p(done), _p(inertia), 1 if skip_done else 0, _stream()), "spadot_lloyd_step")


def kmeanspp_seed(X, xoff, npts, n_max, pset, pK, pfirst, puoff, U, K_max, out=None):
    _need_cuda(X)
    P, D = int(pset.shape[0]), int(X.shape[1])
    dev = X.device
    idx, centers, closest = out if out is not None else (
        torch.empty((P, K_max), dtype=torch.int32, device=dev), torch.empty((P, K_max, D), dtype=torch.float64, device=dev),
        torch.empty((P, int(n_max)), dtype=torch.float64, device=dev))
    _check(model_lib().spadot_kmeanspp_seed(_p(X), _p(xoff), _p(npts), D, P, _p(pset), _p(pK), _p(pfirst), _p(puoff), _p(U),
                                            int(K_max), int(n_max), _p(closest), _p(idx), _p(centers), _stream()),
           "spadot_kmeanspp_seed")
    return idx, centers


def knn(coords, kk):
    _need_cuda(coords)
    x = coords.contiguous().double()
    n, d = x.shape
    out = torch.empty((n, kk), dtype=torch.int32, device=x.device)
    _check(model_lib().spadot_knn(_p(x), n, d, int(kk), _p(out), _stream()), "spadot_knn")
    return out


STAMP_BUF = [None]


def stamp_if(slot):
    if STAMP_BUF[0] is not None:
        stamp(STAMP_BUF[0], slot)


def stamp(buf, slot):
    _check(model_lib().spadot_stamp(_p(buf), int(slot), _stream()), "spadot_stamp")


class FlatAdamW:

    def __init__(self, params, lr=3e-4, betas=(0.9, 0.999), eps=1e-8, weight_decay=1e-2, max_norm=0.3, last=None, first=None):
        params = [p for p in params if p.requires_grad]
        tail_ids = {id(p) for p in (last or [])}
        head_ids = {id(p) for p in (first or [])} - tail_ids
        params = ([p for p in params if id(p) in head_ids] + [p for p in params if id(p) not in tail_ids and id(p) not in head_ids]
                  + [p for p in params if id(p) in tail_ids])
        n_tail = sum(1 for p in params if id(p) in tail_ids)
        n_head = sum(1 for p in params if id(p) in head_ids)
        assert params and all(p.is_cuda and p.dtype == torch.float32 for p in params), \
            "FlatAdamW needs fp32 parameters on the MI355X"
        dev = params[0].device
        sizes = [p.numel() for p in params]
# ... 10 lines not shown
        for p, o, s in zip(params, offs, sizes):
            self.flat_param[o:o + s].copy_(p.data.reshape(-1))
            p.data = self.flat_param[o:o + s].view_as(p.data)
            p.grad = self.flat_grad[o:o + s].view_as(p.data)
        self.params, self.count = params, tot
        self.tail_offset = offs[len(params) - n_tail] if n_tail else None
        self.tail_params = params[len(params) - n_tail:] if n_tail else []
        self.head_count = (offs[n_head] if n_head < len(params) else tot) if n_head else 0
        self.lr, self.betas, self.eps, self.weight_decay, self.max_norm = lr, betas, eps, weight_decay, max_norm
        self.t = 0
        self.step_dev = torch.zeros(1, dtype=torch.int32, device=dev)
        self.grad_scale = torch.ones(1, dtype=torch.float32, device=dev)
        self._counter = torch.zeros(1, dtype=torch.int32, device=dev)
        self._images, self._image_table, self.images_version = [], None, 0
        self._image_stamps = {}

    def owns(self, param):
        lo = self.flat_param.data_ptr()
        return param.is_cuda and lo <= param.data_ptr() < lo + 4 * self.count

    def _stamp(self, param):
        return (self.flat_param._version, param._version)

    def maintain_image(self, param, image):
        if not self.owns(param):
            return False
        if any(im.data_ptr() == image.data_ptr() and p is param for p, im in self._images):
            return True
        idx = next((i for i, p in enumerate(self.params) if p is param), None)
        rows, K = (int(param.shape[0]), int(param.shape[1])) if param.dim() == 2 else (0, 0)
        ok = (idx is not None and param.dim() == 2 and image.dtype == torch.bfloat16 and image.is_contiguous()
              and image.dim() == 2 and image.shape[0] == rows and image.shape[1] >= K and K % 4 == 0 and image.shape[1] % 4 == 0
              and rows * K < 2 ** 31 and image.data_ptr() % 8 == 0 and len(self._images) < 8 and self.count % 4 == 0
              and not any(im.data_ptr() == image.data_ptr() for _, im in self._images))
        if not ok:
            return False
        self._images.append((param, image))
        self._image_table = None
        self.images_version += 1
        self.refresh_images([image])
        return True

    def maintains(self, image):
        return any(im.data_ptr() == image.data_ptr() for _, im in self._images)

    def refresh_images(self, only=None):
        pairs = [(p.detach(), im) for p, im in self._images if only is None or any(im is o for o in only)]
        if pairs:
            with torch.no_grad():
                cast_rows(pairs)
        for p, im in self._images:
            if only is None or any(im is o for o in only):
                self._image_stamps[im.data_ptr()] = self._stamp(p)

    def sync_images(self):
        stale = [im for p, im in self._images if self._image_stamps.get(im.data_ptr()) != self._stamp(p)]
        if stale:
            self.refresh_images(stale)
        return len(stale)

    def _images_struct(self):
        if self._image_table is None:
            from ._lib import WeightImages
            tab = WeightImages()
            tab.n = len(self._images)
            for k, (p, im) in enumerate(self._images):
                off = (p.data_ptr() - self.flat_param.data_ptr()) // 4
                tab.w[k].offset, tab.w[k].rows, tab.w[k].K, tab.w[k].Kp = off, p.shape[0], p.shape[1], im.shape[1]
                tab.w[k].image = im.data_ptr()
            self._image_table = tab
        return self._image_table

    def zero_grad(self):
        self.flat_grad.zero_()

    def backward(self, loss):
        _DIRECT_GRAD[0] = True
        post = POST_CHAIN[0] = []
        try:
            grads = torch.autograd.grad(loss, self.params, allow_unused=True)
        finally:
            _DIRECT_GRAD[0] = False
            POST_CHAIN[0] = None
        with torch.no_grad():
            for job in post:
                job()
        pairs = [(p.grad, g) for p, g in zip(self.params, grads) if g is not None and g.data_ptr() != p.grad.data_ptr()]
        dst = [d for d, _ in pairs]
        src = [s for _, s in pairs]
        self._zero_unreached(self.params, grads)
        torch._foreach_copy_(dst, src)

    def backward_partial(self, outputs, grad_outputs, params, extra_inputs=()):
        ins = list(params) + list(extra_inputs)
        if grad_outputs is None and torch.is_tensor(outputs) and outputs.dim() == 0 and outputs.dtype == torch.float32:
            grad_outputs = unit_seed(outputs.device)
        _DIRECT_GRAD[0] = True
        post = POST_CHAIN[0] = []
        try:
            grads = torch.autograd.grad(outputs, ins, grad_outputs=grad_outputs, allow_unused=True)
        finally:
            _DIRECT_GRAD[0] = False
            POST_CHAIN[0] = None
        with torch.no_grad():
            for job in post:
                job()
        pg = grads[:len(params)]
        pairs = [(p.grad, g) for p, g in zip(params, pg) if g is not None and g.data_ptr() != p.grad.data_ptr()]
        self._zero_unreached(params, pg)
        if pairs:
            try:
                torch._foreach_copy_([d for d, _ in pairs], [s for _, s in pairs])
            except RuntimeError as ex:
                bad = [(tuple(d.shape), d.requires_grad, d.is_leaf, d.data_ptr() - self.flat_grad.data_ptr()) for d, _ in pairs
                       if d.requires_grad or not (0 <= d.data_ptr() - self.flat_grad.data_ptr() < 4 * self.count)]
                raise RuntimeError(f"{ex}; offending gradient slots (shape, requires_grad, is_leaf, byte offset in flat_grad): {bad}") from ex
        return grads[len(params):]

    def _zero_unreached(self, params, grads):
        for p, g in zip(params, grads):
            if g is None:
                p.grad.zero_()

    def grad_norm_sq(self):
        _check(model_lib().spadot_grad_sumsq(_p(self.flat_grad), self.count, _p(self.scratch), _p(self.sumsq),
                                             _stream()), "spadot_grad_sumsq")
        return self.sumsq

    def step(self):
        self.t += 1
        if self._images:
            _check(model_lib().spadot_clip_adamw_images_dev(_p(self.flat_param), _p(self.flat_grad), _p(self.exp_avg),
                                                            _p(self.exp_avg_sq), self.count, self.lr, self.betas[0], self.betas[1],
                                                            self.eps, self.weight_decay, self.max_norm, _p(self.scratch),
                                                            _p(self.sumsq), _p(self.step_dev), _p(self.grad_scale),
                                                            ctypes.byref(self._images_struct()), _stream()),
                   "spadot_clip_adamw_images_dev")
            return
        _check(model_lib().spadot_clip_adamw_dev(_p(self.flat_param), _p(self.flat_grad), _p(self.exp_avg),
                                                 _p(self.exp_avg_sq), self.count, self.lr, self.betas[0], self.betas[1],
                                                 self.eps, self.weight_decay, self.max_norm, _p(self.scratch), _p(self.sumsq),
                                                 _p(self.step_dev), _p(self._counter), _p(self.grad_scale), _stream()),
               "spadot_clip_adamw_dev")

    def _update_range(self, lo, hi):
        tab = ctypes.byref(self._images_struct()) if self._images else None
        _check(model_lib().spadot_adamw_range_dev(_p(self.flat_param), _p(self.flat_grad), _p(self.exp_avg), _p(self.exp_avg_sq),
                                                  lo, hi - lo, self.lr, self.betas[0], self.betas[1], self.eps, self.weight_decay,
                                                  self.max_norm, _p(self.sumsq), _p(self.step_dev), _p(self.grad_scale), tab,
                                                  _stream()), "spadot_adamw_range_dev")

    def step_sharded(self, group=None):
        from . import parallel as _par
        assert self.count % 4 == 0
        self.t += 1

        def local_sumsq(lo, hi):
            if hi <= lo:
                self.sumsq.zero_()
                self.step_dev += 1
                return self.sumsq
            _check(model_lib().spadot_grad_norm_step_dev(self.flat_grad[lo:hi].data_ptr(), hi - lo, _p(self.scratch), _p(self.sumsq),
                                                         _p(self.step_dev), _stream()), "spadot_grad_norm_step_dev")
            return self.sumsq

        def update_range(lo, hi, sumsq):
            if sumsq.data_ptr() != self.sumsq.data_ptr():
                self.sumsq.copy_(sumsq)
            self._update_range(lo, hi)

        _par.sharded_update(self.flat_grad, self.flat_param, local_sumsq, update_range, group=group)
        if self._images:
            self.refresh_images()

    def step_head(self):
        assert self.head_count > 0 and self.count % 4 == 0
        self.t += 1
        _check(model_lib().spadot_grad_norm_step_dev(_p(self.flat_grad), self.count, _p(self.scratch), _p(self.sumsq),
                                                     _p(self.step_dev), _stream()), "spadot_grad_norm_step_dev")
        self._update_range(0, self.head_count)

    def step_rest(self):
        if self.head_count < self.count:
            self._update_range(self.head_count, self.count)
```

Before: 672.0 training steps/s.

## Fold recon dh slab reduction, bias colsum, and grad-norm into downstream kernels

The recon forward/backward now leaves per-slab partial dh instead of reducing it, and the MLP-chain backward sums those slabs while loading its input gradient. A bias column-sum is folded into the wgrad reduce kernel as extra blocks, and the grad-norm computation is fused with the head AdamW update. The aim is fewer kernel launches and fewer intermediate passes over memory in the backward and optimizer steps. The cost is more complex cross-function state through slab cells, and the chain backward now reads every slab.

Result: no change. 671.2 training steps/s (-0.1%).

```diff
diff --git a/include/spadot_model.h b/include/spadot_model.h
--- a/include/spadot_model.h
+++ b/include/spadot_model.h
@@ -139,6 +139,9 @@
                     int G, double inv_scale, const float *grad_weight, void *g_bf16, float *workspace, double *loss_parts, float *dh,
                     void *stream);
 int spadot_sum_parts(const double *part, int n, double scale, float *out, void *stream);
+int spadot_recon_fb_slabs(const void *h_bf16, const void *W_bf16, const void *WT_bf16, int ldt, const float *bias, const float *y, int b,
+                          int K, int G, double inv_scale, const float *grad_weight, void *g_bf16, float *workspace, double *loss_parts,
+                          void *stream);
 
 int spadot_stamp(unsigned long long *buf, int slot, void *stream);
 
@@ -203,6 +206,9 @@
 long long spadot_gemm_wgrad_bf16_workspace_tiled(int M, int N, int K, int slices, int tile_k);
 int spadot_gemm_wgrad_bf16_tiled(const void *G, int ldg, const void *X, int ldx, float *dW, int ldw, int M, int N, int K,
                                  int slices, int tile_k, float *workspace, const void *zero_row, void *stream);
+int spadot_gemm_wgrad_bf16_tiled_colsum(const void *G, int ldg, const void *X, int ldx, float *dW, int ldw, int M, int N, int K,
+                                        int slices, int tile_k, float *workspace, const void *zero_row, const float *cs_part,
+                                        int cs_nslab, int cs_width, float *cs_out, void *stream);
 
 int spadot_mlp_chain_supported(int n_layers, const int *dims);
 int spadot_mlp_chain_workspace(int b, int n_layers, const int *dims, int *n_rows, int *width);
@@ -221,6 +227,10 @@
                                   const float *const *gamma, const double *slope, float *const *a, float *const *y,
                                   float *const *mean, float *const *invstd, float *dx, const float *dx_add, float *workspace,
                                   float *grads, void *stream);
+int spadot_mlp_chain_backward_slabs(const float *dy_slabs, int nslab, const float *x, int b, int n_layers, const int *dims,
+                                    const float *const *W, const float *const *gamma, const double *slope, float *const *a,
+                                    float *const *y, float *const *mean, float *const *invstd, float *dx, const float *dx_add,
+                                    float *workspace, float *grads, void *stream);
 
 int spadot_bias_sqerr_forward(const float *o, const float *bias, const float *y, int b, int G, double inv_scale, double *scratch,
                               float *out, void *stream);
@@ -256,6 +266,10 @@
                            double lr, double beta1, double beta2, double eps, double weight_decay, double max_norm,
                            const float *sumsq, const int *step_dev, const float *grad_scale_dev, const spadot_weight_images *images,
                            void *stream);
+int spadot_norm_adamw_head_dev(float *param, const float *grad, float *exp_avg, float *exp_avg_sq, long long count, long long head_count,
+                               double lr, double beta1, double beta2, double eps, double weight_decay, double max_norm, double *scratch,
+                               float *sumsq, int *step_dev, const float *grad_scale_dev, const spadot_weight_images *images,
+                               void *stream);
 
 int spadot_adamw_step(float *param, const float *grad, float *exp_avg, float *exp_avg_sq,
                       const float *sumsq, long long count, double lr, double beta1, double beta2,
diff --git a/spadot_amd/_lib.py b/spadot_amd/_lib.py
--- a/spadot_amd/_lib.py
+++ b/spadot_amd/_lib.py
@@ -176,6 +176,7 @@
         "spadot_enc_fused_supported": [ci, ci, ci, ci],
         "spadot_recon_fb_supported": [ci, ci, ci],
         "spadot_recon_fb": [vp, vp, vp, ci, vp, vp, ci, ci, ci, cd, vp, vp, vp, vp, vp, vp],
+        "spadot_recon_fb_slabs": [vp, vp, vp, ci, vp, vp, ci, ci, ci, cd, vp, vp, vp, vp, vp],
         "spadot_sum_parts": [vp, ci, cd, vp, vp],
         "spadot_enc_bn_map": [vp, vp, vp, vp, vp, vp, vp, ci, ci, cd, cd, cd, vp, vp, vp, vp, ci, vp, vp],
         "spadot_enc_bn_fc": [vp, ci, vp, vp, vp, vp, vp, vp, ci, ci, cd, cd, cd, vp, vp, vp, vp, vp, ci, vp, vp],
@@ -185,6 +186,7 @@
         "spadot_gemm_tn_bf16_split": [vp, ci, vp, ci, vp, ci, ci, ci, ci, ci, ci, vp, vp],
         "spadot_gemm_wgrad_bf16": [vp, ci, vp, ci, vp, ci, ci, ci, ci, ci, vp, vp, vp],
         "spadot_gemm_wgrad_bf16_tiled": [vp, ci, vp, ci, vp, ci, ci, ci, ci, ci, ci, vp, vp, vp],
+        "spadot_gemm_wgrad_bf16_tiled_colsum": [vp, ci, vp, ci, vp, ci, ci, ci, ci, ci, ci, vp, vp, vp, ci, ci, vp, vp],
         "spadot_mlp_chain_supported": [ci, vp],
         "spadot_headfc_backward": [vp, vp, vp, ci, ci, ci, vp, vp, vp, vp],
         "spadot_bias_sqerr_forward": [vp, vp, vp, ci, ci, cd, vp, vp, vp],
@@ -194,6 +196,7 @@
         "spadot_mlp_chain_forward_bf16": [vp, ci, ci, vp, vp, vp, vp, vp, vp, vp, vp, vp, vp, vp, vp, vp],
         "spadot_mlp_chain_backward": [vp, vp, ci, ci, vp, vp, vp, vp, vp, vp, vp, vp, vp, vp, vp, vp],
         "spadot_mlp_chain_backward_add": [vp, vp, ci, ci, vp, vp, vp, vp, vp, vp, vp, vp, vp, vp, vp, vp, vp],
+        "spadot_mlp_chain_backward_slabs": [vp, ci, vp, ci, ci, vp, vp, vp, vp, vp, vp, vp, vp, vp, vp, vp, vp, vp],
         "spadot_kernel_matrix": [vp, vp, ci, ci, ci, cd, ci, ci, vp, vp],
         "spadot_spd_inverse_logdet": [vp, ci, ci, vp, vp, vp],
         "spadot_rowdot_forward": [vp, vp, ci, ci, ci, ci, vp, vp],
@@ -235,6 +238,7 @@
         "spadot_clip_adamw_images_dev": [vp, vp, vp, vp, ll, cd, cd, cd, cd, cd, cd, vp, vp, vp, vp, ctypes.POINTER(WeightImages), vp],
         "spadot_grad_norm_step_dev": [vp, ll, vp, vp, vp, vp],
         "spadot_adamw_range_dev": [vp, vp, vp, vp, ll, ll, cd, cd, cd, cd, cd, cd, vp, vp, vp, ctypes.POINTER(WeightImages), vp],
+        "spadot_norm_adamw_head_dev": [vp, vp, vp, vp, ll, ll, cd, cd, cd, cd, cd, cd, vp, vp, vp, vp, ctypes.POINTER(WeightImages), vp],
         "spadot_adamw_step": [vp, vp, vp, vp, vp, ll, cd, cd, cd, cd, cd, cd, ci, vp],
         "spadot_adamw_step_dev": [vp, vp, vp, vp, vp, ll, cd, cd, cd, cd, cd, cd, vp, vp],
         "spadot_pre_gene_detect": [vp, vp, vp, vp, ci, ci, cd, vp, vp, vp],
diff --git a/spadot_amd/csrc/gemm_wgrad_bf16.hip b/spadot_amd/csrc/gemm_wgrad_bf16.hip
--- a/spadot_amd/csrc/gemm_wgrad_bf16.hip
+++ b/spadot_amd/csrc/gemm_wgrad_bf16.hip
@@ -198,8 +198,8 @@
 }
 
 template <int TKE>
-__global__ __launch_bounds__(256) void k_wgrad_reduce(const float *__restrict__ part, int S, int tiles, int ktiles,
-                                                      float *__restrict__ dW, int ldw, int N, int K) {
+__device__ __forceinline__ void wgrad_reduce_block(const float *__restrict__ part, int S, int tiles, int ktiles,
+                                                   float *__restrict__ dW, int ldw, int N, int K) {
     constexpr int RP = TKE / 4;
     constexpr int BPT = RP / 4;
     constexpr int Q = 64 * RP;
@@ -229,6 +229,48 @@
                 if (k + e < K) dW[(size_t)n * ldw + k + e] = sum[e];
         }
     }
+}
+
+template <int TKE>
+__global__ __launch_bounds__(256) void k_wgrad_reduce(const float *__restrict__ part, int S, int tiles, int ktiles,
+                                                      float *__restrict__ dW, int ldw, int N, int K) {
+    wgrad_reduce_block<TKE>(part, S, tiles, ktiles, dW, ldw, N, K);
+}
+
+template <int TKE>
+__global__ __launch_bounds__(256) void k_wgrad_reduce_colsum(const float *__restrict__ part, int S, int tiles, int ktiles,
+                                                             float *__restrict__ dW, int ldw, int N, int K,
+                                                             const float *__restrict__ cpart, int nslab, int width,
+                                                             float *__restrict__ cout) {
+    const int nred = tiles * (TKE / 16);
+    if ((int)blockIdx.x < nred) {
+        wgrad_reduce_block<TKE>(part, S, tiles, ktiles, dW, ldw, N, K);
+        return;
+    }
+    constexpr int GY = 16;
+    __shared__ float sh[GY][17];
+    const int cx = threadIdx.x & 15, gy = threadIdx.x >> 4;
+    const int c = ((int)blockIdx.x - nred) * 16 + cx;
+    float acc = 0.f;
+    {
+        const int cc = min(c, width - 1);
+        const int per = (nslab + GY - 1) / GY;
+        const int s0 = gy * per, s1 = min(nslab, s0 + per);
+        for (int sb = s0; sb < s1; sb += 16) {
+            float q[16];
+#pragma unroll
+            for (int u = 0; u < 16; u++) q[u] = cpart[(size_t)min(sb + u, nslab - 1) * width + cc];
+#pragma unroll
+            for (int u = 0; u < 16; u++) acc += (sb + u < s1) ? q[u] : 0.f;
+        }
+    }
+    sh[gy][cx] = acc;
+    __syncthreads();
+    if (gy != 0 || c >= width) return;
+    acc = 0.f;
+#pragma unroll
+    for (int g = 0; g < GY; g++) acc += sh[g][cx];
+    cout[c] = acc;
 }
 
 static int effective_slices(int M, int slices, int *cps_out) {
@@ -257,7 +299,8 @@
 
 template <int WGN, int WGK, int TI, int TJ>
 static int launch_wgrad(const void *G, int ldg, const void *X, int ldx, float *dW, int ldw, int M, int N, int K, int ktiles, int ntiles,
-                        int S, int cps, float *workspace, const void *zero_row, hipStream_t stream) {
+                        int S, int cps, float *workspace, const void *zero_row, hipStream_t stream, const float *cpart = nullptr,
+                        int nslab = 0, int width = 0, float *cout = nullptr) {
     constexpr int TKE = 32 * WGK * TJ;
     static PerDeviceFlag attr_set;     
     auto kern = k_gemm_wgrad_bf16<WGN, WGK, TI, TJ>;
@@ -268,14 +311,17 @@
     const int tiles = ntiles * ktiles;
     hipLaunchKernelGGL(kern, dim3((unsigned)(tiles * S)), dim3(NT), LDS_BYTES, stream, (const __bf16 *)G, ldg, (const __bf16 *)X, ldx, dW,
                        ldw, M, N, K, ktiles, S, cps, (const __bf16 *)zero_row, workspace);
-    if (S > 1)
+    if (S > 1 && cpart)
+        hipLaunchKernelGGL(k_wgrad_reduce_colsum<TKE>, dim3((unsigned)tiles * (unsigned)(TKE / 16) + (unsigned)((width + 15) / 16)), dim3(256), 0,
+                           stream, (const float *)workspace, S, tiles, ktiles, dW, ldw, N, K, cpart, nslab, width, cout);
+    else if (S > 1)
         hipLaunchKernelGGL(k_wgrad_reduce<TKE>, dim3((unsigned)tiles * (unsigned)(TKE / 16)), dim3(256), 0, stream, (const float *)workspace, S,
                            tiles, ktiles, dW, ldw, N, K);
     return hipGetLastError() == hipSuccess ? 0 : -5;
 }
 
-extern "C" int spadot_gemm_wgrad_bf16_tiled(const void *G, int ldg, const void *X, int ldx, float *dW, int ldw, int M, int N, int K,
-                                            int slices, int tile_k, float *workspace, const void *zero_row, void *stream) {
+static int wgrad_tiled(const void *G, int ldg, const void *X, int ldx, float *dW, int ldw, int M, int N, int K, int slices, int tile_k,
+                       float *workspace, const void *zero_row, void *stream, const float *cpart, int nslab, int width, float *cout) {
     if (M <= 0 || N <= 0 || K <= 0 || N % TN != 0 || ldg < N || ldx < K || ldw < K || ldg % 8 || ldx % 8) return -22;
     if (tile_k != 256 && tile_k != 192) return -22;
     if (((uintptr_t)G & 15) || ((uintptr_t)X & 15) || ((uintptr_t)dW & 15) || (ldw % 4)) return -22;
@@ -287,9 +333,24 @@
     const int S = effective_slices(M, slices, &cps);
     if (ntiles * ktiles > 4096) return -22;
     if (S > 1 && (!workspace || ((uintptr_t)workspace & 15))) return -22;
+    if (cpart && S < 2) return -22;
     if (tile_k == 256)
-        return launch_wgrad<2, 4, 4, 2>(G, ldg, X, ldx, dW, ldw, M, N, K, ktiles, ntiles, S, cps, workspace, zero_row, (hipStream_t)stream);
-    return launch_wgrad<4, 2, 2, 3>(G, ldg, X, ldx, dW, ldw, M, N, K, ktiles, ntiles, S, cps, workspace, zero_row, (hipStream_t)stream);
+        return launch_wgrad<2, 4, 4, 2>(G, ldg, X, ldx, dW, ldw, M, N, K, ktiles, ntiles, S, cps, workspace, zero_row, (hipStream_t)stream,
+                                        cpart, nslab, width, cout);
+    return launch_wgrad<4, 2, 2, 3>(G, ldg, X, ldx, dW, ldw, M, N, K, ktiles, ntiles, S, cps, workspace, zero_row, (hipStream_t)stream, cpart,
+                                    nslab, width, cout);
+}
+
+extern "C" int spadot_gemm_wgrad_bf16_tiled(const void *G, int ldg, const void *X, int ldx, float *dW, int ldw, int M, int N, int K,
+                                            int slices, int tile_k, float *workspace, const void *zero_row, void *stream) {
+    return wgrad_tiled(G, ldg, X, ldx, dW, ldw, M, N, K, slices, tile_k, workspace, zero_row, stream, nullptr, 0, 0, nullptr);
+}
+
+extern "C" int spadot_gemm_wgrad_bf16_tiled_colsum(const void *G, int ldg, const void *X, int ldx, float *dW, int ldw, int M, int N, int K,
+                                                   int slices, int tile_k, float *workspace, const void *zero_row, const float *cs_part,
+                                                   int cs_nslab, int cs_width, float *cs_out, void *stream) {
+    if (!cs_part || !cs_out || cs_nslab < 1 || cs_width < 1) return -22;
+    return wgrad_tiled(G, ldg, X, ldx, dW, ldw, M, N, K, slices, tile_k, workspace, zero_row, stream, cs_part, cs_nslab, cs_width, cs_out);
 }
 
 extern "C" int spadot_gemm_wgrad_bf16(const void *G, int ldg, const void *X, int ldx, float *dW, int ldw, int M, int N, int K,
diff --git a/spadot_amd/csrc/mlp_chain.hip b/spadot_amd/csrc/mlp_chain.hip
--- a/spadot_amd/csrc/mlp_chain.hip
+++ b/spadot_amd/csrc/mlp_chain.hip
@@ -104,9 +104,11 @@
 constexpr int WST = 16384;
 constexpr int LPR = 256 / RBB;
 constexpr int LDS_BWD_FLOATS = 4 * RBB * LDW + 2 * RBB + MAXD + WST;
+constexpr int SG = 24;
+template <bool SLABS>
 __global__ __launch_bounds__(256, 1) void k_mlp_chain_bwd(const float *__restrict__ dy_last, const float *__restrict__ x, int b,
                                                        Chain ch, float *__restrict__ dx_out, float *__restrict__ ws,
-                                                       int ws_width, const float *__restrict__ dx_add) {
+                                                       int ws_width, const float *__restrict__ dx_add, int nslab) {
     extern __shared__ __attribute__((aligned(16))) float lds_dyn[];
     float (*gz)[LDW] = reinterpret_cast<float (*)[LDW]>(lds_dyn);
     float (*da)[LDW] = reinterpret_cast<float (*)[LDW]>(lds_dyn + RBB * LDW);
@@ -118,7 +120,43 @@
     const int t = threadIdx.x;
     const int r0 = blockIdx.x * RBB;
     float *wrow = ws + (size_t)blockIdx.x * ws_width;
-    {
+    if constexpr (SLABS) {
+        constexpr int NV = RBB * MAXD / 4 / 256;
+        const int d4 = ch.s[ch.n - 1].dout / 4;
+        const size_t n4 = (size_t)b * d4;
+        const f32x4 *src = reinterpret_cast<const f32x4 *>(dy_last);
+        size_t pos[NV];
+#pragma unroll
+        for (int u = 0; u < NV; u++) {
+            const int e = min(t + u * 256, RBB * d4 - 1), r = e / d4;
+            pos[u] = (size_t)min(r0 + r, b - 1) * d4 + (e - r * d4);
+        }
+        f32x4 acc[NV];
+#pragma unroll
+        for (int u = 0; u < NV; u++) acc[u] = f32x4{0.f, 0.f, 0.f, 0.f};
+        for (int k = 0; k < nslab; k += SG) {
+            f32x4 v[SG][NV];
+#pragma unroll
+            for (int q = 0; q < SG; q++)
+#pragma unroll
+                for (int u = 0; u < NV; u++) v[q][u] = src[(size_t)min(k + q, nslab - 1) * n4 + pos[u]];
+#pragma unroll
+            for (int q = 0; q < SG; q++)
+                if (k + q < nslab) {
+#pragma unroll
+                    for (int u = 0; u < NV; u++) acc[u] += v[q][u];
+                }
+        }
+#pragma unroll
+        for (int u = 0; u < NV; u++) {
+            const int e = t + u * 256;
+            if (e < RBB * d4) {
+                const int r = e / d4;
+                if (!(r0 + r < b)) acc[u] = f32x4{0.f, 0.f, 0.f, 0.f};
+                *reinterpret_cast<f32x4 *>(&gz[r][4 * (e - r * d4)]) = acc[u];
+            }
+        }
+    } else {
         const int d = ch.s[ch.n - 1].dout;
         float v[RBB * MAXD / 256];
 #pragma unroll
@@ -520,25 +558,48 @@
     return spadot_mlp_chain_forward_bf16(x, b, n_layers, dims, W, bias, gamma, beta, eps, slope, a, y, mean, invstd, nullptr, stream);
 }
 
-int spadot_mlp_chain_backward_add(const float *dy, const float *x, int b, int n_layers, const int *dims, const float *const *W,
-                                  const float *const *gamma, const double *slope, float *const *a, float *const *y,
-                                  float *const *mean, float *const *invstd, float *dx, const float *dx_add, float *workspace,
-                                  float *grads, void *stream) {
+}
+
+namespace {
+template <bool SLABS>
+int launch_chain_bwd(const float *dy, int nslab, const float *x, int b, int n_layers, const int *dims, const float *const *W,
+                     const float *const *gamma, const double *slope, float *const *a, float *const *y, float *const *mean,
+                     float *const *invstd, float *dx, const float *dx_add, float *workspace, float *grads, void *stream) {
     Chain ch;
     if (b <= 0 || !fill_chain(ch, n_layers, dims, W, nullptr, gamma, nullptr, nullptr, slope, a, y, mean, invstd)) return -22;
     if (dx_add && !dx) return -22;
     int rows, width;
     if (spadot_mlp_chain_workspace(b, n_layers, dims, &rows, &width)) return -22;
     constexpr int LDS_BWD = LDS_BWD_FLOATS * (int)sizeof(float);
-    static PerDeviceFlag attr_set;     
+    static PerDeviceFlag attr_set;
     if (!attr_set) {
-        if (hipFuncSetAttribute((const void *)k_mlp_chain_bwd, hipFuncAttributeMaxDynamicSharedMemorySize, LDS_BWD) != hipSuccess) return -5;
+        if (hipFuncSetAttribute((const void *)k_mlp_chain_bwd<SLABS>, hipFuncAttributeMaxDynamicSharedMemorySize, LDS_BWD) != hipSuccess) return -5;
         attr_set = true;
     }
-    hipLaunchKernelGGL(k_mlp_chain_bwd, dim3(rows), dim3(256), LDS_BWD, (hipStream_t)stream, dy, x, b, ch, dx, workspace, width, dx_add);
+    hipLaunchKernelGGL(k_mlp_chain_bwd<SLABS>, dim3(rows), dim3(256), LDS_BWD, (hipStream_t)stream, dy, x, b, ch, dx, workspace, width,
+                       dx_add, nslab);
     if (hipGetLastError() != hipSuccess) return -5;
     if (!grads) return 0;
     return spadot_colsum(workspace, rows, width, grads, stream);
+}
+}
+
+extern "C" {
+
+int spadot_mlp_chain_backward_add(const float *dy, const float *x, int b, int n_layers, const int *dims, const float *const *W,
+                                  const float *const *gamma, const double *slope, float *const *a, float *const *y,
+                                  float *const *mean, float *const *invstd, float *dx, const float *dx_add, float *workspace,
+                                  float *grads, void *stream) {
+    return launch_chain_bwd<false>(dy, 0, x, b, n_layers, dims, W, gamma, slope, a, y, mean, invstd, dx, dx_add, workspace, grads, stream);
+}
+
+int spadot_mlp_chain_backward_slabs(const float *dy_slabs, int nslab, const float *x, int b, int n_layers, const int *dims,
+                                    const float *const *W, const float *const *gamma, const double *slope, float *const *a,
+                                    float *const *y, float *const *mean, float *const *invstd, float *dx, const float *dx_add,
+                                    float *workspace, float *grads, void *stream) {
+    if (nslab < 1 || !dy_slabs || ((uintptr_t)dy_slabs & 15)) return -22;
+    return launch_chain_bwd<true>(dy_slabs, nslab, x, b, n_layers, dims, W, gamma, slope, a, y, mean, invstd, dx, dx_add, workspace, grads,
+                                  stream);
 }
 
 int spadot_mlp_chain_backward(const float *dy, const float *x, int b, int n_layers, const int *dims, const float *const *W,
diff --git a/spadot_amd/csrc/model_kernels.hip b/spadot_amd/csrc/model_kernels.hip
--- a/spadot_amd/csrc/model_kernels.hip
+++ b/spadot_amd/csrc/model_kernels.hip
@@ -1330,8 +1330,10 @@
 __global__ void k_step_inc(int *step) { step[0] += 1; }
 
 template <int U>
-__global__ __launch_bounds__(256) void k_sumsq_part_u(const float *__restrict__ g, long long count, double *__restrict__ part) {
+__global__ __launch_bounds__(256) void k_sumsq_part_u(const float *__restrict__ g, long long count, double *__restrict__ part,
+                                                      int *__restrict__ step_dev) {
     __shared__ double sh[16];
+    if (step_dev && blockIdx.x == 0 && threadIdx.x == 0) step_dev[0] += 1;
     double acc = 0.0;
     const long long n4 = count / 4;
     const float4 *g4 = reinterpret_cast<const float4 *>(g);
@@ -1397,17 +1399,15 @@
     }
 }
 
-__global__ __launch_bounds__(256) void k_adamw_img(float *__restrict__ p, const float *__restrict__ g,
-                                                   float *__restrict__ m, float *__restrict__ v,
-                                                   const float *__restrict__ sumsq, long long count, float lr,
-                                                   float b1, float b2, float eps, float wd, float max_norm,
-                                                   const int *__restrict__ step_dev, const float *__restrict__ grad_scale,
-                                                   spadot_weight_images imgs, long long base) {
+__device__ __forceinline__ void adamw_img_body(float *__restrict__ p, const float *__restrict__ g, float *__restrict__ m,
+                                               float *__restrict__ v, float sumsq, long long count, float lr, float b1, float b2,
+                                               float eps, float wd, float max_norm, const int *__restrict__ step_dev,
+                                               const float *__restrict__ grad_scale, const spadot_weight_images &imgs, long long base) {
     const double t = (double)step_dev[0];
     const float bc1 = (float)(1.0 - pow((double)b1, t));
     const float bc2_sqrt = (float)sqrt(1.0 - pow((double)b2, t));
     const float gs = grad_scale ? grad_scale[0] : 1.f;
-    const float coef = adamw_clip_coef(sumsq[0], gs, max_norm);
+    const float coef = adamw_clip_coef(sumsq, gs, max_norm);
     const long long n4 = count >> 2;
     for (long long q = (long long)blockIdx.x * 256 + threadIdx.x; q < n4; q += (long long)gridDim.x * 256) {
         const long long k = q << 2;
@@ -1444,6 +1444,48 @@
             }
         }
     }
+}
+
+__global__ __launch_bounds__(256) void k_adamw_img(float *__restrict__ p, const float *__restrict__ g,
+                                                   float *__restrict__ m, float *__restrict__ v,
+                                                   const float *__restrict__ sumsq, long long count, float lr,
+                                                   float b1, float b2, float eps, float wd, float max_norm,
+                                                   const int *__restrict__ step_dev, const float *__restrict__ grad_scale,
+                                                   spadot_weight_images imgs, long long base) {
+    adamw_img_body(p, g, m, v, sumsq[0], count, lr, b1, b2, eps, wd, max_norm, step_dev, grad_scale, imgs, base);
+}
+
+__global__ __launch_bounds__(256) void k_adamw_img_sum(float *__restrict__ p, const float *__restrict__ g,
+                                                       float *__restrict__ m, float *__restrict__ v,
+                                                       const double *__restrict__ part, int nparts, float *__restrict__ sumsq_out,
+                                                       long long count, float lr, float b1, float b2, float eps, float wd,
+                                                       float max_norm, const int *__restrict__ step_dev,
+                                                       const float *__restrict__ grad_scale, spadot_weight_images imgs, long long base) {
+    __shared__ double sh[16];
+    double pv[8];
+#pragma unroll
+    for (int u = 0; u < 8; u++) pv[u] = part[min((int)threadIdx.x + u * 256, nparts - 1)];
+    double a[4];
+#pragma unroll
+    for (int j = 0; j < 4; j++) {
+        const int v = (int)threadIdx.x + 256 * j;
+        a[j] = 0.0;
+        if (v < nparts) a[j] += pv[j];
+        if (v + 1024 < nparts) a[j] += pv[j + 4];
+#pragma unroll
+        for (int off = 32; off > 0; off >>= 1) a[j] += __shfl_xor(a[j], off, WAVE);
+    }
+    if ((threadIdx.x & 63) == 0) {
+#pragma unroll
+        for (int j = 0; j < 4; j++) sh[(threadIdx.x >> 6) + 4 * j] = a[j];
+    }
+    __syncthreads();
+    double acc = 0.0;
+#pragma unroll
+    for (int k = 0; k < 16; k++) acc += sh[k];
+    const float sumsq = (float)acc;
+    if (blockIdx.x == 0 && threadIdx.x == 0) sumsq_out[0] = sumsq;
+    adamw_img_body(p, g, m, v, sumsq, count, lr, b1, b2, eps, wd, max_norm, step_dev, grad_scale, imgs, base);
 }
 
 #ifndef BN_RG_DEF
@@ -2651,7 +2693,7 @@
     constexpr int split = 2048;
     if (split > 0) {
         const int nb2 = (int)(want4 < 1 ? 1 : (want4 < split ? want4 : split));
-        hipLaunchKernelGGL(k_sumsq_part_u<4>, dim3(nb2), dim3(256), 0, st_, grad, count, scratch);
+        hipLaunchKernelGGL(k_sumsq_part_u<4>, dim3(nb2), dim3(256), 0, st_, grad, count, scratch, (int *)nullptr);
         hipLaunchKernelGGL(k_final_sum_step, dim3(1), dim3(1024), 0, st_, (const double *)scratch, nb2, sumsq, step_dev);
     } else
         hipLaunchKernelGGL(k_sumsq_last<4>, dim3(nbs), dim3(256), 0, st_, grad, count, scratch, sumsq, step_dev, counter);
@@ -2679,7 +2721,7 @@
     hipStream_t st_ = (hipStream_t)stream;
     const long long want4 = (count / 4 + 255) / 256;
     const int nb2 = (int)(want4 < 1 ? 1 : (want4 < 2048 ? want4 : 2048));
-    hipLaunchKernelGGL(k_sumsq_part_u<4>, dim3(nb2), dim3(256), 0, st_, grad, count, scratch);
+    hipLaunchKernelGGL(k_sumsq_part_u<4>, dim3(nb2), dim3(256), 0, st_, grad, count, scratch, (int *)nullptr);
     hipLaunchKernelGGL(k_final_sum_step, dim3(1), dim3(1024), 0, st_, (const double *)scratch, nb2, sumsq, step_dev);
     const int nb = (int)(want4 < 4096 ? want4 : 4096);
     hipLaunchKernelGGL(k_adamw_img, dim3(nb), dim3(256), 0, st_, param, grad, exp_avg, exp_avg_sq, (const float *)sumsq, count,
@@ -2693,7 +2735,7 @@
     hipStream_t st_ = (hipStream_t)stream;
     const long long want4 = (count / 4 + 255) / 256;
     const int nb2 = (int)(want4 < 1 ? 1 : (want4 < 2048 ? want4 : 2048));
-    hipLaunchKernelGGL(k_sumsq_part_u<4>, dim3(nb2), dim3(256), 0, st_, grad, count, scratch);
+    hipLaunchKernelGGL(k_sumsq_part_u<4>, dim3(nb2), dim3(256), 0, st_, grad, count, scratch, (int *)nullptr);
     hipLaunchKernelGGL(k_final_sum_step, dim3(1), dim3(1024), 0, st_, (const double *)scratch, nb2, sumsq, step_dev);
     return hipGetLastError() == hipSuccess ? 0 : -5;
 }
@@ -2724,6 +2766,35 @@
     return hipGetLastError() == hipSuccess ? 0 : -5;
 }
 
+int spadot_norm_adamw_head_dev(float *param, const float *grad, float *exp_avg, float *exp_avg_sq, long long count, long long head_count,
+                               double lr, double beta1, double beta2, double eps, double weight_decay, double max_norm, double *scratch,
+                               float *sumsq, int *step_dev, const float *grad_scale_dev, const spadot_weight_images *images,
+                               void *stream) {
+    if (count <= 0 || head_count <= 0 || head_count > count || (head_count & 3) || !scratch || !step_dev || !sumsq) return -22;
+    if (((uintptr_t)grad & 15) || ((uintptr_t)param & 15) || ((uintptr_t)exp_avg & 15) || ((uintptr_t)exp_avg_sq & 15)) return -22;
+    spadot_weight_images none;
+    none.n = 0;
+    const spadot_weight_images *tab = images ? images : &none;
+    if (tab->n < 0 || tab->n > 8) return -22;
+    for (int s_ = 0; s_ < tab->n; s_++) {
+        const spadot_weight_image &W = tab->w[s_];
+        if (!W.image || ((uintptr_t)W.image & 7) || W.rows <= 0 || W.K <= 0 || (W.K & 3) || W.Kp < W.K || (W.Kp & 3) || (W.offset & 3) ||
+            W.offset < 0 || (long long)W.rows * W.K >= (1ll << 31))
+            return -22;
+    }
+    hipStream_t st_ = (hipStream_t)stream;
+    const long long want4 = (count / 4 + 255) / 256;
+    const int nb2 = (int)(want4 < 1 ? 1 : (want4 < 2048 ? want4 : 2048));
+    hipLaunchKernelGGL(k_sumsq_part_u<4>, dim3(nb2), dim3(256), 0, st_, grad, count, scratch, step_dev);
+    constexpr long long max_wgs = 512;
+    const long long hw4 = (head_count / 4 + 255) / 256;
+    const int nb = (int)(hw4 < max_wgs ? hw4 : max_wgs);
+    hipLaunchKernelGGL(k_adamw_img_sum, dim3(nb), dim3(256), 0, st_, param, grad, exp_avg, exp_avg_sq, (const double *)scratch, nb2, sumsq,
+                       head_count, (float)lr, (float)beta1, (float)beta2, (float)eps, (float)weight_decay, (float)max_norm,
+                       (const int *)step_dev, grad_scale_dev, *tab, 0ll);
+    return hipGetLastError() == hipSuccess ? 0 : -5;
+}
+
 int spadot_adamw_step(float *param, const float *grad, float *exp_avg, float *exp_avg_sq, const float *sumsq,
                       long long count, double lr, double beta1, double beta2, double eps, double weight_decay,
                       double max_norm, int step, void *stream) {
diff --git a/spadot_amd/csrc/recon_fb.hip b/spadot_amd/csrc/recon_fb.hip
--- a/spadot_amd/csrc/recon_fb.hip
+++ b/spadot_amd/csrc/recon_fb.hip
@@ -170,11 +170,12 @@
     return (long long)((G + BG - 1) / BG) * b * K + (long long)((b + BR - 1) / BR) * G;
 }
 
-int spadot_recon_fb(const void *h_bf16, const void *W_bf16, const void *WT_bf16, int ldt, const float *bias, const float *y, int b, int Kin,
+namespace {
+int recon_fb_launch(const void *h_bf16, const void *W_bf16, const void *WT_bf16, int ldt, const float *bias, const float *y, int b, int Kin,
                     int G, double inv_scale, const float *grad_weight, void *g_bf16, float *workspace, double *loss_parts, float *dh,
-                    void *stream) {
+                    bool reduce, void *stream) {
     if (!spadot_recon_fb_supported(b, Kin, G) || !h_bf16 || !W_bf16 || !WT_bf16 || !bias || !y || !grad_weight || !g_bf16 || !workspace ||
-        !loss_parts || !dh || ldt < (G + BG - 1) / BG * BG || ldt % 8 || ((uintptr_t)WT_bf16 & 15))
+        !loss_parts || (reduce && !dh) || ldt < (G + BG - 1) / BG * BG || ldt % 8 || ((uintptr_t)WT_bf16 & 15))
         return -22;
     if (((uintptr_t)h_bf16 & 15) || ((uintptr_t)W_bf16 & 15) || ((uintptr_t)bias & 15) || ((uintptr_t)y & 15) || ((uintptr_t)g_bf16 & 15) ||
         ((uintptr_t)workspace & 15) || ((uintptr_t)dh & 15))
@@ -185,9 +186,26 @@
     hipLaunchKernelGGL(k_recon_fb, dim3(GB, RB), dim3(NT), 0, st, (const __bf16 *)h_bf16, (const __bf16 *)W_bf16, (const __bf16 *)WT_bf16, ldt,
                        bias, y, b, G,
                        inv_scale, grad_weight, (__bf16 *)g_bf16, dbp, loss_parts, dxp);
-    const long long n4 = (long long)b * K / 4;
-    hipLaunchKernelGGL(k_recon_fb_reduce, dim3((unsigned)((n4 + 255) / 256)), dim3(256), 0, st, (const float *)dxp, GB, n4, dh);
+    if (reduce) {
+        const long long n4 = (long long)b * K / 4;
+        hipLaunchKernelGGL(k_recon_fb_reduce, dim3((unsigned)((n4 + 255) / 256)), dim3(256), 0, st, (const float *)dxp, GB, n4, dh);
+    }
     return hipGetLastError() == hipSuccess ? 0 : -5;
+}
+}
+
+int spadot_recon_fb(const void *h_bf16, const void *W_bf16, const void *WT_bf16, int ldt, const float *bias, const float *y, int b, int Kin,
+                    int G, double inv_scale, const float *grad_weight, void *g_bf16, float *workspace, double *loss_parts, float *dh,
+                    void *stream) {
+    return recon_fb_launch(h_bf16, W_bf16, WT_bf16, ldt, bias, y, b, Kin, G, inv_scale, grad_weight, g_bf16, workspace, loss_parts, dh, true,
+                           stream);
+}
+
+int spadot_recon_fb_slabs(const void *h_bf16, const void *W_bf16, const void *WT_bf16, int ldt, const float *bias, const float *y, int b,
+                          int Kin, int G, double inv_scale, const float *grad_weight, void *g_bf16, float *workspace, double *loss_parts,
+                          void *stream) {
+    return recon_fb_launch(h_bf16, W_bf16, WT_bf16, ldt, bias, y, b, Kin, G, inv_scale, grad_weight, g_bf16, workspace, loss_parts, nullptr,
+                           false, stream);
 }
 
 }
diff --git a/spadot_amd/model/decoder.py b/spadot_amd/model/decoder.py
--- a/spadot_amd/model/decoder.py
+++ b/spadot_amd/model/decoder.py
@@ -2,7 +2,7 @@
 import torch.nn as nn
 import torch.nn.functional as F
 
-from ..ops import (grad_bias, linear_bias, ln_act, mlp_chain, mlp_chain_ok, recon_fb_ok, recon_sqerr, recon_sqerr_fb, recon_sqerr_ok,
+from ..ops import (FOLD_SLABS, grad_bias, linear_bias, ln_act, mlp_chain, mlp_chain_ok, recon_fb_ok, recon_sqerr, recon_sqerr_fb, recon_sqerr_ok,
                    sqerr_sum, weight_image)
 
 
@@ -30,12 +30,14 @@
     def recon_loss(self, latent_sample, y, inv_scale, dz_extra=None, grad_weight=None):
         bf = self.compute_dtype == torch.bfloat16
         nocast = bf
-        h, last, hb = self._hidden(latent_sample, bf16_out=nocast, dx_add=dz_extra)
+        cell = {} if (FOLD_SLABS[0] and bf and grad_weight is not None and self.training and latent_sample.shape[0] <= 512) else None
+        h, last, hb = self._hidden(latent_sample, bf16_out=nocast, dx_add=dz_extra, slab_cell=cell)
         if bf and grad_weight is not None:
             wim = self._output_image(last.weight)
             wimT = self._output_image_T(wim) if wim is not None else None
             if recon_fb_ok(h, last.weight, last.bias, y, hb, wim, wimT, grad_weight):
-                return recon_sqerr_fb(h, last.weight, last.bias, y, inv_scale, hb, wim, wimT, grad_weight)
+                return recon_sqerr_fb(h, last.weight, last.bias, y, inv_scale, hb, wim, wimT, grad_weight,
+                                      slab_cell=cell if (cell is not None and cell.get("armed")) else None)
         if bf and recon_sqerr_ok(h, last.weight, last.bias, y):
             return recon_sqerr(h, last.weight, last.bias, y, inv_scale, hb, self._output_image(last.weight) if nocast else None)
         return sqerr_sum(y, linear_bias(h, last.weight, last.bias, self.compute_dtype), inv_scale)
@@ -74,13 +76,13 @@
         if wim is not None:
             self._output_image_T(wim, refresh=True)
 
-    def _hidden(self, latent_sample, bf16_out=False, dx_add=None):
+    def _hidden(self, latent_sample, bf16_out=False, dx_add=None, slab_cell=None):
         stages = list(self.decoder_net)
         h, hb = latent_sample, None
         hidden = [(stages[i], stages[i + 1], stages[i + 2].negative_slope) for i in range(0, len(stages) - 1, 3)]
         if hidden and mlp_chain_ok(h, hidden):
             if bf16_out:
-                h, hb = mlp_chain(h, hidden, bf16_out=True, dx_add=dx_add)
+                h, hb = mlp_chain(h, hidden, bf16_out=True, dx_add=dx_add, slab_cell=slab_cell)
             else:
                 h = mlp_chain(h, hidden, dx_add=dx_add)
         else:
diff --git a/spadot_amd/ops.py b/spadot_amd/ops.py
--- a/spadot_amd/ops.py
+++ b/spadot_amd/ops.py
@@ -160,7 +160,11 @@
             if ctx.defer and _deferring():
                 DEFERRED[0].append(job)
             elif POST_CHAIN[0] is not None:
-                POST_CHAIN[0].append(job)
+                if FOLD_COLSUM[0]:
+                    req = PENDING_COLSUM[0] = {"args": (part, nrow, W3, fa), "done": False}
+                    POST_CHAIN[0].append(lambda: None if req["done"] else job())
+                else:
+                    POST_CHAIN[0].append(job)
             else:
                 job()
             return dh, fa, fd, fb_, None, None, None, None, None, None, None
@@ -508,7 +512,7 @@
     return best[1], best[2], best[3]
 
 
-def wgrad_bf16(g, x, K, out=None):
+def wgrad_bf16(g, x, K, out=None, take_colsum=False):
     M, N = g.shape
     Kp = x.shape[1]
     if (g.is_cuda and g.dtype == torch.bfloat16 and x.dtype == torch.bfloat16 and g.is_contiguous()
@@ -521,6 +525,18 @@
             lib = model_lib()
             need = int(lib.spadot_gemm_wgrad_bf16_workspace_tiled(M, N, K, slices, tile_k))
             ws = torch.empty(max(need, 4), dtype=torch.float32, device=g.device) if need >= 0 else None
+            req = PENDING_COLSUM[0] if take_colsum else None
+            if req is not None and not req["done"] and ws is not None and need > 0:
+                cpart, nrow, width, cout = req["args"]
+                rc = lib.spadot_gemm_wgrad_bf16_tiled_colsum(g.data_ptr(), N, x.data_ptr(), Kp, out.data_ptr(), K, M, N, K, slices, tile_k,
+                                                             ws.data_ptr(), _zero_row(g.device).data_ptr(), _p(cpart), nrow, width, _p(cout),
+                                                             _stream())
+                if rc == 0:
+                    req["done"] = True
+                    PENDING_COLSUM[0] = None
+                    return out
+                if rc != -22:
+                    _check(rc, "spadot_gemm_wgrad_bf16_tiled_colsum")
             rc = -22 if ws is None else lib.spadot_gemm_wgrad_bf16_tiled(g.data_ptr(), N, x.data_ptr(), Kp, out.data_ptr(), K, M, N, K,
                                                                         slices, tile_k, ws.data_ptr(), _zero_row(g.device).data_ptr(),
                                                                         _stream())
@@ -583,7 +599,7 @@
                 DEFERRED[0].append(lambda g=g, x=x, K=ctx.K, out=ctx.wgrad: wgrad_bf16(g, x, K, out))
                 dW = ctx.wgrad
             else:
-                dW = wgrad_bf16(g, x, ctx.K, ctx.wgrad if (ctx.wgrad is not None and _DIRECT_GRAD[0]) else None)
+                dW = wgrad_bf16(g, x, ctx.K, ctx.wgrad if (ctx.wgrad is not None and _DIRECT_GRAD[0]) else None, take_colsum=True)
         return dx, dW, None, None, None, None
 
 
@@ -931,6 +947,11 @@
 
 CHAIN_BF16_OUT = [False]
 CHAIN_DX_ADD = [None]
+CHAIN_SLAB_CELL = [None]
+FOLD_SLABS = [True]
+FOLD_COLSUM = [True]
+FOLD_NORM = [True]
+PENDING_COLSUM = [None]
 _LAST_CHAIN_BF16 = []
 
 
@@ -958,6 +979,9 @@
         if ybf is not None:
             _LAST_CHAIN_BF16.append(ybf)
         ctx.dx_add = CHAIN_DX_ADD[0]
+        ctx.slab_cell = CHAIN_SLAB_CELL[0]
+        if ctx.slab_cell is not None:
+            ctx.slab_cell["armed"] = True
         ctx.save_for_backward(x, stats, *Ws, *gs, *a, *y)
         ctx.n, ctx.dims, ctx.slope = n, dims, [float(v) for v in slope]
         ctx.flat_out = _contiguous_grad_block(params)
@@ -984,11 +1008,23 @@
         late = direct and _deferring()
         add = ctx.dx_add
         assert add is None or (dx is not None and add.shape == x.shape and add.dtype == torch.float32 and add.is_contiguous())
-        _check(lib.spadot_mlp_chain_backward_add(_p(dy.contiguous().float()), _p(x), b, n, cd, _ptr_array(Ws), _ptr_array(gs), cs,
-                                                 _ptr_array(a), _ptr_array(y), _ptr_array(mean), _ptr_array(inv),
-                                                 None if dx is None else _p(dx), None if add is None else _p(add), _p(ws),
-                                                 None if late else _p(grads), _stream()),
-               "spadot_mlp_chain_backward_add")
+        slabs = ctx.slab_cell.pop("slabs", None) if ctx.slab_cell is not None else None
+        if slabs is not None:
+            dxp, nslab = slabs
+            if dy.data_ptr() != dxp.data_ptr() or dy.shape != (b, dims[-1]):
+                raise RuntimeError("mlp_chain: gradient slabs were left for this chain, but the gradient that arrived is not their "
+                                   "placeholder (the chain's output has another consumer)")
+            _check(lib.spadot_mlp_chain_backward_slabs(_p(dxp), nslab, _p(x), b, n, cd, _ptr_array(Ws), _ptr_array(gs), cs,
+                                                       _ptr_array(a), _ptr_array(y), _ptr_array(mean), _ptr_array(inv),
+                                                       None if dx is None else _p(dx), None if add is None else _p(add), _p(ws),
+                                                       None if late else _p(grads), _stream()),
+                   "spadot_mlp_chain_backward_slabs")
+        else:
+            _check(lib.spadot_mlp_chain_backward_add(_p(dy.contiguous().float()), _p(x), b, n, cd, _ptr_array(Ws), _ptr_array(gs), cs,
+                                                     _ptr_array(a), _ptr_array(y), _ptr_array(mean), _ptr_array(inv),
+                                                     None if dx is None else _p(dx), None if add is None else _p(add), _p(ws),
+                                                     None if late else _p(grads), _stream()),
+                   "spadot_mlp_chain_backward_add")
         if late:
             DEFERRED[0].append(lambda ws=ws, grads=grads: _check(
                 lib.spadot_colsum(_p(ws), ws.shape[0], ws.shape[1], _p(grads), _stream()), "spadot_colsum"))
@@ -1015,13 +1051,13 @@
     return bool(model_lib().spadot_mlp_chain_supported(len(stages), (ctypes.c_int * len(dims))(*dims)))
 
 
-def mlp_chain(x, stages, bf16_out=False, dx_add=None):
+def mlp_chain(x, stages, bf16_out=False, dx_add=None, slab_cell=None):
     params = [t_ for lin, ln, _ in stages for t_ in (lin.weight, lin.bias, ln.weight, ln.bias)]
-    CHAIN_BF16_OUT[0], CHAIN_DX_ADD[0] = bool(bf16_out), dx_add
+    CHAIN_BF16_OUT[0], CHAIN_DX_ADD[0], CHAIN_SLAB_CELL[0] = bool(bf16_out), dx_add, slab_cell
     try:
         out = _MLPChain.apply(x.contiguous(), [ln.eps for _, ln, _ in stages], [sl for _, _, sl in stages], *params)
     finally:
-        CHAIN_BF16_OUT[0], CHAIN_DX_ADD[0] = False, None
+        CHAIN_BF16_OUT[0], CHAIN_DX_ADD[0], CHAIN_SLAB_CELL[0] = False, None, None
     return (out, _LAST_CHAIN_BF16.pop()) if bf16_out else out
 
 
@@ -1492,7 +1528,7 @@
 class _ReconFB(torch.autograd.Function):
 
     @staticmethod
-    def forward(ctx, h, W, bias, y, inv_scale, hc, Wc, WcT, gw):
+    def forward(ctx, h, W, bias, y, inv_scale, hc, Wc, WcT, gw, slab_cell=None):
         lib = model_lib()
         b, K = h.shape
         G = W.shape[0]
@@ -1502,9 +1538,16 @@
         ws = torch.empty(nfl, dtype=torch.float32, device=dev)
         lossp = torch.empty(GB * RB, dtype=torch.float64, device=dev)
         gc = torch.empty((b, G), dtype=torch.bfloat16, device=dev)
-        dh = torch.empty((b, K), dtype=torch.float32, device=dev)
-        _check(lib.spadot_recon_fb(_p(hc), _p(Wc), _p(WcT), WcT.shape[1], _p(bias), _p(y), b, K, G, float(inv_scale), _p(gw), _p(gc), _p(ws),
-                                   _p(lossp), _p(dh), _stream()), "spadot_recon_fb")
+        ctx.slab_cell = slab_cell
+        if slab_cell is not None:
+            dh = ws[:b * K].view(b, K)
+            ctx.nslab = GB
+            _check(lib.spadot_recon_fb_slabs(_p(hc), _p(Wc), _p(WcT), WcT.shape[1], _p(bias), _p(y), b, K, G, float(inv_scale), _p(gw),
+                                             _p(gc), _p(ws), _p(lossp), _stream()), "spadot_recon_fb_slabs")
+        else:
+            dh = torch.empty((b, K), dtype=torch.float32, device=dev)
+            _check(lib.spadot_recon_fb(_p(hc), _p(Wc), _p(WcT), WcT.shape[1], _p(bias), _p(y), b, K, G, float(inv_scale), _p(gw), _p(gc),
+                                       _p(ws), _p(lossp), _p(dh), _stream()), "spadot_recon_fb")
         out = torch.empty(1, dtype=torch.float32, device=dev)
 
         def value(lossp=lossp, out=out):
@@ -1529,6 +1572,8 @@
         hc, gc, dh = ctx.saved_tensors
         lib = model_lib()
         dbp = ctx.dbp
+        if ctx.slab_cell is not None:
+            ctx.slab_cell["slabs"] = (dh, ctx.nslab)
         direct = _DIRECT_GRAD[0]
         db = ctx.bgrad if (direct and ctx.bgrad is not None) else torch.empty(dbp.shape[1], dtype=torch.float32, device=dh.device)
         dW = ctx.wgrad if (direct and ctx.wgrad is not None) else torch.empty((gc.shape[1], hc.shape[1]), dtype=torch.float32, device=dh.device)
@@ -1542,7 +1587,7 @@
         else:
             with torch.no_grad():
                 rest()
-        return dh, dW, db, None, None, None, None, None, None
+        return dh, dW, db, None, None, None, None, None, None, None
 
 
 def recon_fb_ok(h, W, bias, y, hc, Wc, WcT, gw):
@@ -1555,8 +1600,8 @@
                 and ok(hc, h) and ok(Wc, W) and model_lib().spadot_recon_fb_supported(h.shape[0], h.shape[1], W.shape[0]))
 
 
-def recon_sqerr_fb(h, W, bias, y, inv_scale, h_bf16, W_image, W_image_T, grad_weight):
-    return _ReconFB.apply(h, W, bias, y, inv_scale, h_bf16, W_image, W_image_T, grad_weight)
+def recon_sqerr_fb(h, W, bias, y, inv_scale, h_bf16, W_image, W_image_T, grad_weight, slab_cell=None):
+    return _ReconFB.apply(h, W, bias, y, inv_scale, h_bf16, W_image, W_image_T, grad_weight, slab_cell)
 
 
 def recon_sqerr_ok(h, W, bias, y):
@@ -1733,6 +1778,7 @@
         finally:
             _DIRECT_GRAD[0] = False
             POST_CHAIN[0] = None
+            PENDING_COLSUM[0] = None
         with torch.no_grad():
             for job in post:
                 job()
@@ -1753,6 +1799,7 @@
         finally:
             _DIRECT_GRAD[0] = False
             POST_CHAIN[0] = None
+            PENDING_COLSUM[0] = None
         with torch.no_grad():
             for job in post:
                 job()
@@ -1827,6 +1874,14 @@
     def step_head(self):
         assert self.head_count > 0 and self.count % 4 == 0
         self.t += 1
+        if FOLD_NORM[0]:
+            tab = ctypes.byref(self._images_struct()) if self._images else None
+            _check(model_lib().spadot_norm_adamw_head_dev(_p(self.flat_param), _p(self.flat_grad), _p(self.exp_avg), _p(self.exp_avg_sq),
+                                                          self.count, self.head_count, self.lr, self.betas[0], self.betas[1], self.eps,
+                                                          self.weight_decay, self.max_norm, _p(self.scratch), _p(self.sumsq),
+                                                          _p(self.step_dev), _p(self.grad_scale), tab, _stream()),
+                   "spadot_norm_adamw_head_dev")
+            return
         _check(model_lib().spadot_grad_norm_step_dev(_p(self.flat_grad), self.count, _p(self.scratch), _p(self.sumsq),
                                                      _p(self.step_dev), _stream()), "spadot_grad_norm_step_dev")
         self._update_range(0, self.head_count)
```
